# kaiidams/voice100

Hardware: AMD Instinct MI355X
Metric: audio frames/sec (fwd+bwd) asr_en_base, B=32x1024-frame mel (higher is better)
Workload: dtype bf16

## Files before the change

include/voice100_hip.h:

```cpp
#ifndef VOICE100_HIP_H
#define VOICE100_HIP_H

#ifdef __cplusplus
extern "C" {
#endif


int v100_dw_num_groups(int B, int C);
int v100_dwconv(const float* x, const float* x2, const float* w, const float* in_a, const float* in_b,
                const float* in_c, int in_mode, float* y, const float* aux, const float* out_a,
                const float* out_b, int out_mode, float* stats, int G, int B, int C, int Tin, int Tout,
                int K, int stride, int pad, int flip, int upsample, int force_generic, void* stream);

int v100_dwconv_wgrad(const float* g, const float* g2, const float* ga, const float* gb, const float* gc,
                      int g_mode, const float* x, const float* xa, const float* xb, int x_mode,
                      float* partial, float* dw, int G, int B, int C, int Tin, int Tout, int K, int stride,
                      int pad, int force_generic, void* stream);

int v100_dwconv_bwd(const float* g, const float* g2, const float* w, const float* ga, const float* gb,
                    const float* gc, const float* xpre, const float* xa, const float* xb, float* dxin,
                    float* stats, float* wpartial, float* dw, int G, int B, int C, int Tin, int Tout, int K,
                    int stride, int pad, int force_split, void* stream);

int v100_pw_num_parts(int B, int T);
int v100_pw_gemm(const float* A, const void* A_bf16, const float* X, const float* X2, const float* xa,
                 const float* xb, const float* xc, int x_mode, float* Y, const float* bias, const float* ea,
                 const float* eb, const float* R, int epi_mode, float* stats, int B, int M, int K, int T,
                 int use_bf16, void* stream);
int v100_pw_gemm_dropmask_supported(int B, int M, int K, int T, int use_bf16);
int v100_pw_gemm_dropmask(const float* A, const void* A_bf16, const float* X, float* Y, const void* keep, float p, int B, int M, int K,
                          int T, int use_bf16, void* stream);

int v100_pw_wgrad_splits(int B, int M, int K);
int v100_pw_wgrad(const float* G, const float* G2, const float* ga, const float* gb, const float* gc, int g_mode,
                  const float* X, const float* xa, const float* xb, int x_mode, float* partial, float* dW,
                  int S, int B, int M, int K, int T, int use_bf16, void* stream);

int v100_weight_prep(const float* w, int rows, int cols, void* w_bf16, float* wt, void* wt_bf16, void* stream);
int v100_weight_prep_f16(const float* w, int rows, int cols, void* w16, void* stream);

int v100_bn_finalize_train(const float* stats, int parts, long long count, const float* gamma, const float* beta,
                           float* running_mean, float* running_var, long long* num_batches_tracked, float momentum,
                           float eps, float* scale, float* shift, float* save_mean, float* save_rstd, int C, void* stream);
int v100_bn_eval_coeffs(const float* gamma, const float* beta, const float* running_mean, const float* running_var,
                        float eps, float* scale, float* shift, int C, void* stream);
int v100_bn_bwd_finalize(const float* partial, int parts, long long count, const float* gamma, const float* mean,
                         const float* rstd, float* p, float* q, float* r, float* dgamma, float* dbeta, int C, void* stream);
int v100_bn_frozen_coeffs(const float* gamma, const float* beta, const float* running_mean, const float* running_var,
                          float eps, float* scale, float* shift, float* mean, float* rstd, int C, void* stream);
int v100_bn_bwd_finalize_frozen(const float* partial, int parts, long long count, const float* gamma, const float* mean,
                                const float* rstd, float* p, float* q, float* r, float* dgamma, float* dbeta, int C, void* stream);

int v100_chan_reduce2(const float* u, const float* v, float* partial, int G, int B, int C, int T, void* stream);
int v100_slab_sum0(const float* partial, int parts, float* out, int C, void* stream);
int v100_chan_affine2(const float* u, const float* v, const float* A, const float* Bc, const float* Cc, float* out,
                      int B, int C, int T, void* stream);
int v100_mul_scale(const float* u, const float* m, float s, float* out, long long n, void* stream);
int v100_dropout_fwd(const float* x, long long seed, float p, float* y, void* mask, long long n, void* stream);
int v100_dropout_bwd(const float* dy, const void* mask, float p, float* dx, long long n, void* stream);
int v100_transpose_last2(const float* in, float* out, int B, int R, int Cc, void* stream);
int v100_embedding_bct(const long long* idx, const float* table, float* out, int B, int V, int C, int T, void* stream);
int v100_embedding_bwd(const long long* idx, const float* g, float* dtable, int B, int V, int C, int T, void* stream);


int v100_augment_fused(const float* x, const int* len, const float* uniform, float* y, int B, int Tin, int Tout,
                       int F, int stretch_rate, float pitch_rate, float amp, int n_tmask, const int* tm_s,
                       const int* tm_e, const float* tm_a, int fm_on, int fm_s, int fm_e, float fm_a, int noise_on,
                       float noise_low, float noise_high, float noise_std, int mix, float log_offset, void* stream);
int v100_augment_fused_len(const float* x, const int* len_raw, int* len_out, int* half_out, const float* uniform, float* y,
                           int B, int Tin, int Tout, int F, int stretch_rate, float pitch_rate, float amp, int n_tmask,
                           const int* tm_s, const int* tm_e, const float* tm_a, int fm_on, int fm_s, int fm_e, float fm_a,
                           int noise_on, float noise_low, float noise_high, float noise_std, int mix, float log_offset,
                           void* stream);
int v100_augment_fused_len_t(const float* x, const int* len_raw, int* len_out, int* half_out, const float* uniform, float* y,
                             float* yt, int B, int Tin, int Tout, int F, int stretch_rate, float pitch_rate, float amp, int n_tmask,
                             const int* tm_s, const int* tm_e, const float* tm_a, int fm_on, int fm_s, int fm_e, float fm_a,
                             int noise_on, float noise_low, float noise_high, float noise_std, int mix, float log_offset,
                             void* stream);

int v100_shift_copy(const float* in, float* out, const float* bias, int B, int C, int Tin, int Tout, int in_ctot,
                    int in_coff, int out_ctot, int out_coff, int in_mul, int in_add, int out_mul, int out_add, int n,
                    int accumulate, void* stream);
int v100_stft_frames(const float* x, float* frames, int B, int N, int T, int hop, int win, int n_fft, void* stream);
int v100_power_spectrum(const float* spec, float* pw, int B, int F, int T, void* stream);
int v100_log_transpose(const float* in, float* out, int B, int C, int T, float offset, void* stream);
int v100_log_mel_fused(const float* x, float* out, const float* window, const float* tw256, const float* tw512, const int* mel_start,
                       const int* mel_count, const float* mel_w, int B, int N, int T, int hop, int n_fft, int n_mels, float log_offset,
                       void* stream);
int v100_log_mel_fused_len(const float* x, const int* lengths, float* out, int* out_len, const float* window, const float* tw256,
                           const float* tw512, const int* mel_start, const int* mel_count, const float* mel_w, int B, int N, int T,
                           int hop, int n_fft, int n_mels, float log_offset, float fill, void* stream);
int v100_world_unnormalize(const float* x, float* f0, float* logspc, float* codeap, const float* f0_mean, const float* f0_std,
                           const float* ls_mean, const float* ls_std, const float* ca_mean, const float* ca_std,
                           int B, int T, int S, int Cap, void* stream);
int v100_world_loss_parts(int B, int Tp);
int v100_world_loss(const float* pred, const float* f0, const float* hasf0, const float* logspc, const float* codeap,
                    const int* length, const float* f0_mean, const float* f0_std, const float* ls_mean, const float* ls_std,
                    const float* ca_mean, const float* ca_std, const float* w, float* partial, float* loss, float* unit,
                    int B, int Tp, int Tt, int S, int Cap, int l1, void* stream);
int v100_world_loss_bwd(const float* unit, const float* gout, float* dpred, int B, int Tp, int S, int Cap, void* stream);
int v100_exp_clip(const float* x, float* y, float offset, long long n, void* stream);

int v100_bct_to_cm(const float* in, float* out, int B, int C, int T, void* stream);
int v100_cm_to_btc(const float* in, float* out, int B, int C, int T, void* stream);

int v100_world_randn_host(float* host_out, long long n);
int v100_world_decode_aperiodicity(const float* coded, float* ap, long long rows, int nb, int fs, int fft_size, void* stream);
long long v100_world_synth_workspace_bytes(int B, int T, int fs, double frame_period_ms, int fft_size, int max_pulses);
int v100_world_synthesize(const float* f0, const float* sp, const float* ap, const float* coded_ap, int nb, const int* frames, const float* randn_table,
                          long long table_len, const float* tw256, const float* tw512, const float* dc_remover, float* y,
                          int* n_pulses, void* workspace, int B, int T, int fs, double frame_period_ms, int fft_size,
                          int max_pulses, void* stream);

int v100_im2col(const float* x, float* cols, int B, int Cin, int Tin, int Tout, int k, int stride, int pad, void* stream);
int v100_col2im(const float* dcols, float* dx, int B, int Cin, int Tin, int Tout, int k, int stride, int pad, void* stream);
int v100_pad_copy(const float* src, float* dst, int B, int C, int Tsrc, int src_step, int src_off, int n, int Tx, int lpad, void* stream);
int v100_pw_taps_supported(int B, int M, int cx, int ntap, int T, int Tx, int use_bf16);
int v100_pw_gemm_taps(const float* A, const void* A_bf16, const float* Xp, float* Y, const float* bias, const float* R,
                      int B, int M, int cx, int T, int Tx, int ntap, const int* shifts, int use_bf16, void* stream);
int v100_pw_wgrad_taps(const float* G, int Tg, int g_off, const float* Xp, float* partial, float* dW, int S, int B, int M,
                       int cx, int T, int Tx, int ntap, const int* shifts, int use_bf16, void* stream);
int v100_ln_num_parts(int B, int T);
int v100_slab_sum2(const float* partial, int parts, float* out0, float* out1, int C, void* stream);
int v100_ln_gelu_fwd(const float* y, const float* gamma, const float* beta, float eps, float* out, float* mean,
                     float* rstd, int B, int C, int T, void* stream);
int v100_ln_gelu_bwd(const float* dout, const float* y, const float* gamma, const float* beta, const float* mean,
                     const float* rstd, float* dy, float* partial, int B, int C, int T, void* stream);

long long v100_launch_count(void);
int v100_copy_probe(const void* src, void* dst, long long nbytes, void* stream);
int v100_timing_enable(int tag_mask);
int v100_timing_read(int tag, double* ms, long long* count, double* bytes);
int v100_rows_copy_probe(const void* src, void* dst, int B, int C, int row_bytes, void* stream);

int v100_pw_gemm_io(const void* A_bf16, const void* X, const void* X2, const float* xa, const float* xb, const float* xc,
                    int x_mode, void* Y, const float* ea, const float* eb, const void* R, int epi_mode, float* stats,
                    int B, int M, int K, int T, int io16, void* stream);
int v100_pw_wgrad_io(const void* G, const void* G2, const float* ga, const float* gb, const float* gc, int g_mode,
                     const void* X, const float* xa, const float* xb, int x_mode, float* partial, float* dW, int S, int B,
                     int M, int K, int T, int io16, void* stream);
int v100_pw_wgrad_group_supported(int B, int M, int K, int T, int S, int g_mode, int x_mode, int io16);
int v100_pw_wgrad_group_tiles(int M, int K, int x_mode);
int v100_pw_wgrad_group(int n, const void* const* ptrs, const int* dims, void* stream);
int v100_dw_mfma_supported(int K, int stride);
int v100_row_pitch16(int T, int B);
int v100_dwconv_fwd_train_io(const void* a1, const float* w, const float* in_a, const float* in_b, void* a2, float* stats,
                             int G, int B, int C, int T, int K, int io16, void* stream);
int v100_dwconv_bwd_io(const void* g, const void* g2, const float* w, const float* ga, const float* gb, const float* gc,
                       const void* xpre, const float* xa, const float* xb, void* dxin, float* stats, float* wpartial,
                       float* dw, int G, int B, int C, int T, int K, int io16, void* stream);
int v100_dwconv_bwd_da1_io(const void* g, const void* g2, const float* w, const float* ga, const float* gb, const float* gc,
                           const void* xpre, const float* xa, const float* xb, void* da1_out, float* stats, float* dw,
                           const float* bn1_gamma, const float* bn1_mean, const float* bn1_rstd, float* pqr, float* dgamma,
                           float* dbeta, int B, int C, int T, int K, void* stream);
int v100_dwconv_fwd_eval_io(const void* h1, const float* w, const float* out_a, const float* out_b, void* h2, int B, int C, int T,
                            int K, int flags, void* stream);
int v100_chan_reduce2_io(const void* u, const void* v, float* partial, int G, int B, int C, int T, int io16, void* stream);
int v100_chan_affine2_shadow(const void* u, const float* v, const float* A, const float* Cc, float* out, void* shadow,
                             int B, int C, int T, int u_bf16, void* stream);
int v100_chan_affine2_io(const void* u, const void* v, const float* A, const float* Bc, const float* Cc, void* out,
                         int B, int C, int T, int io16, void* stream);
int v100_ir_act16_supported(const int* shape);

int v100_adam_chunk_elems(void);
int v100_adam_step(const void* chunks, int nchunks, const void* params, const void* grads, const void* exp_avg,
                   const void* exp_avg_sq, double lr, double beta1, double beta2, double eps, double weight_decay, int step,
                   void* stream);

int v100_grad_norm_partials(const void* chunks, int nchunks, const void* grads, void* partials, int norm_type, void* stream);
int v100_adam_step_clip(const void* chunks, int nchunks, const void* params, const void* grads, const void* exp_avg,
                        const void* exp_avg_sq, double lr, double beta1, double beta2, double eps, double weight_decay, int step,
                        int clip_mode, double clip, const void* partials, int npartials, int norm_type, void* total_norm, void* stream);
int v100_grad_clip(const void* chunks, int nchunks, const void* grads, int clip_mode, double clip, const void* partials, int npartials,
                   int norm_type, void* total_norm, void* stream);

int v100_ctc_workspace_floats(int B, int T, int Lmax);
int v100_ctc_loss_mean(const float* logits, const long long* targets, const int* in_len, const int* tgt_len, float* workspace,
                       float* nll, float* loss, float* grad, int B, int T, int V, int Lmax, int blank, void* stream);
int v100_ctc_loss(const float* logits, const long long* targets, const int* in_len, const int* tgt_len, float* workspace,
                  float* nll, float* grad, int B, int T, int V, int Lmax, int blank, void* stream);
int v100_ctc_loss_mean_t(const float* logits, const long long* targets, const int* in_len, const int* tgt_len, float* workspace,
                         float* nll, float* loss, float* grad, int grad_bvt, int B, int T, int V, int Lmax, int blank, void* stream);

long long v100_ir_prep_bytes(const int* shape);
long long v100_ir_fwd_workspace_bytes(const int* shape);
long long v100_ir_eval_cache_bytes(const int* shape);
int v100_ir_eval_prep(const int* shape, const void* const* ptrs, void* stream);
int v100_ir_fwd_eval(const int* shape, const void* const* ptrs, void* stream);
int v100_ir_stack_fwd_eval(int n, const int* shapes, const void* const* ptrs, void* stream);
int v100_ir_prep_batched(const int* shapes, const void* const* w1s, const void* const* w3s, void* const* preps, int n, void* stream);
int v100_ir_fwd_train(const int* shape, const void* const* ptrs, void* stream);
long long v100_ir_bwd_workspace_bytes(const int* shape);
int v100_ir_bwd(const int* shape, const void* const* ptrs, void* stream);

long long v100_ir_stack_plan(const int* desc, long long* plan);
int v100_ir_stack_fwd_train(const int* desc, const void* const* params, const void* x, const void* x16, void* blob, void* stream);
int v100_ir_stack_bwd(const int* desc, const void* const* params, const void* x, const void* x16, const void* blob, const void* dy,
                      void* dx, void* grads, void* ws, void* stream);
int v100_ir_stack_wgrad_plan(const int* desc, int have_x16, int min_problem_tiles, int min_flush_tiles, long long* out);
int v100_ir_stack_wgrad_group_thresholds(int min_problem_tiles, int min_flush_tiles);

int v100_ctc_greedy_decode(const float* logits, const int* lens, long long* out, int* out_len, int B, int T, int V, int blank, void* stream);
int v100_ctc_best_path(const float* logp, const long long* labels, const int* in_len, const int* lab_len, void* back_ws, int* path,
                       float* score, int B, int T, int V, int Lmax, int max_move, void* stream);
long long v100_ctc_align_workspace_bytes(int B, int T, int Lmax);
int v100_ctc_align_block(void);
int v100_ctc_align(const float* logp, const long long* labels, const int* in_len, const int* lab_len, void* moves_ws, int* path,
                   long long* best_labels, int* align, float* score, int B, int T, int V, int Lmax, int max_move, void* stream);
long long v100_edit_distance_workspace_bytes(int B, int Th, int Tr);
int v100_edit_distance(const long long* hyp, const int* hyp_len, const long long* ref, const int* ref_len, void* ws, int* dist,
                       int* hyp_n, int* ref_n, long long* totals, int B, int Th, int Tr, int levels, long long sep, void* stream);
long long v100_ctc_beam_workspace_bytes(int B, int T, int V, int W);
int v100_ctc_beam_search(const float* logits, const int* lens, void* ws, long long* ids, int* ids_len, float* scores, int B, int T, int V,
                         int W, int nbest, int blank, void* stream);
int v100_ctc_beam_search_lm(const float* logits, const int* lens, void* ws, long long* ids, int* ids_len, float* scores,
                            const float* lm_logp, const int* lm_next, const float* lm_final, int S, int start_state, float alpha,
                            float beta, int use_eos, float* ctc_scores, float* lm_scores, int B, int T, int V, int W, int nbest,
                            int blank, void* stream);
int v100_align_expand(const long long* text, const double* align, const int* text_len, long long* out, int* out_len, int B, int Lmax,
                      int Tmax, int head, int tail, void* stream);


int v100_world_randn_host_f64(double* host_out, long long n);
long long v100_world_randn_bound(int kind, int T, int fs, int fft_size);
int v100_world_frames(int fs, int length, double frame_period_ms);
int v100_world_dio_bands(int fs, double f0_floor, double f0_ceil, double channels_in_octave, int* half_lengths, int max_bands);
long long v100_world_dio_workspace_bytes(int B, int max_len, int fs, double f0_floor, double f0_ceil, double channels_in_octave,
                                         double frame_period_ms);
int v100_world_dio(const float* x, const int* lengths, int B, int max_len, int pitch, int fs, double f0_floor, double f0_ceil,
                   double channels_in_octave, double frame_period_ms, double allowed_range, const double* lowcut,
                   const double* nuttall, double* f0, void* workspace, void* stream);
int v100_world_cheaptrick(const float* x, const int* lengths, const double* f0, int B, int max_len, int pitch, int fs,
                          double frame_period_ms, double q1, int fft_size, const double* randn_table, long long table_len,
                          const double* twiddle, double* sp, float* logsp, double log_offset, long long* offsets, void* stream);
long long v100_world_d4c_workspace_bytes(int B, int max_len, int fs, double frame_period_ms);
int v100_world_d4c(const float* x, const int* lengths, const double* f0, int B, int max_len, int pitch, int fs, double frame_period_ms,
                   double threshold, int fft_size, const double* randn_table, long long table_len, const double* twiddle,
                   const double* nuttall, int window_length, double* ap, double* coded, float* coded32, void* workspace, void* stream);

long long v100_lstm_weight_bytes(int H, int ndir, int use_bf16, int backward);
int v100_lstm_geometry(int H, int use_bf16, int backward, int* out);
long long v100_lstm_ws_bytes(int B, int H, int ndir, int backward);
int v100_lstm_sync_words(int B, int ndir);
int v100_lstm_persistent_ok(int B, int H, int ndir, int use_bf16, int backward);
int v100_lstm_weight_prep(const float* w_hh0, const float* w_hh1, int H, int ndir, int use_bf16, int backward, void* out,
                          void* stream);
int v100_lstm_fwd(const float* xproj, const void* w_prep, const float* b_hh0, const float* b_hh1, const int* lens, float* y,
                  float* h_n, float* c_n, float* act, float* cs, float* hprev, void* ws, unsigned* sync, int B, int T, int H,
                  int ndir, int use_bf16, int persistent, void* stream);
int v100_lstm_bwd(const float* dy, const float* dh_n, const float* dc_n, const void* w_prep, const int* lens, const float* act,
                  const float* cs, float* dgates, void* ws, unsigned* sync, int B, int T, int H, int ndir, int use_bf16,
                  int persistent, void* stream);

int v100_world_loss_v2(const float* pred, const float* f0, const float* logspc, const float* codeap, const int* length,
                       const float* f0_mean, const float* f0_std, const float* ls_mean, const float* ls_std,
                       const float* ca_mean, const float* ca_std, float* partial, float* loss, float* unit,
                       int B, int Tp, int Tt, int S, int Cap, int l1, void* stream);
int v100_world_loss_v2_bwd(const float* unit, const float* gout, float* dpred, int B, int Tp, int S, int Cap, void* stream);
int v100_align_loss_parts(int B, int L);
int v100_align_loss(const float* pred, const long long* align, const int* text_len, float* partial, float* loss, float* unit,
                    int B, int L, int W, void* stream);
int v100_align_loss_bwd(const float* unit, const float* gout, float* dpred, int B, int L, void* stream);
int v100_align_expand_v2(const long long* text, const double* align, const int* text_len, long long* out, int* out_len, int B,
                         int Lmax, int Tmax, int head, int tail, void* stream);
int v100_world_unnormalize_v2(const float* x, float* f0, float* logspc, float* codeap, const float* f0_mean, const float* f0_std,
                              const float* ls_mean, const float* ls_std, const float* ca_mean, const float* ca_std,
                              int B, int T, int S, int Cap, void* stream);

int v100_masked_ce_parts(int B, int L);
int v100_masked_ce(const float* logits, const long long* target, const int* target_len, float* partial, float* loss, float* unit,
                   int B, int V, int L, void* stream);
int v100_masked_ce_bwd(const float* unit, const float* gout, float* dlogits, int B, int V, int L, void* stream);

long long v100_resample_out_len(long long len, int o, int n);
int v100_resample_tile(void);
int v100_resample_sinc(const float* x, const int* lens, const float* taps, const int* starts, float* y, int* out_lens, int B,
                       int Nmax, int Mmax, int o, int n, int width, int L, void* stream);

int v100_world_stat_parts(int B, int T, int S);
int v100_world_stat_accum(const float* f0, const int* f0_len, const float* logspc, const float* codeap, double* partial,
                          double* moments, int B, int T, int S, int A, void* stream);

#ifdef __cplusplus
}
#endif
#endif
```

voice100_amd/csrc/adam.hip:

```cpp
#include "common.h"
#include <math.h>

struct AdamChunk { int tensor; int count; long long offset; };

__device__ __forceinline__ void adam_update(float& pv, float gv, float& mv, float& vv, float lr_over_bc1, float omb1, float beta2,
                                            float omb2, float eps, float weight_decay, float inv_sqrt_bc2) {
    gv = fmaf(weight_decay, pv, gv);
    mv = fmaf(omb1, gv - mv, mv);
    vv = fmaf(omb2, gv * gv, beta2 * vv);
    pv -= lr_over_bc1 * mv / (sqrtf(vv) * inv_sqrt_bc2 + eps);
}

__global__ __launch_bounds__(256) void adam_step_kernel(const AdamChunk* __restrict__ chunks, float* const* __restrict__ params,
                                                        const float* const* __restrict__ grads, float* const* __restrict__ exp_avg,
                                                        float* const* __restrict__ exp_avg_sq, float lr_over_bc1, float omb1,
                                                        float beta2, float omb2, float eps, float weight_decay, float inv_sqrt_bc2) {
    const AdamChunk ch = chunks[blockIdx.x];
    float* __restrict__ p = params[ch.tensor] + ch.offset;
    const float* __restrict__ g = grads[ch.tensor] + ch.offset;
    float* __restrict__ m = exp_avg[ch.tensor] + ch.offset;
    float* __restrict__ v = exp_avg_sq[ch.tensor] + ch.offset;
    auto upd = [&](float& pv, float gv, float& mv, float& vv) {
        adam_update(pv, gv, mv, vv, lr_over_bc1, omb1, beta2, omb2, eps, weight_decay, inv_sqrt_bc2);
    };
    const bool vec = ((((size_t)p | (size_t)g | (size_t)m | (size_t)v) & 15) == 0);
    if (vec) {
        const int n4 = ch.count >> 2;
        for (int i = threadIdx.x; i < n4; i += 256) {
            f32x4 pv = reinterpret_cast<f32x4*>(p)[i], mv = reinterpret_cast<f32x4*>(m)[i], vv = reinterpret_cast<f32x4*>(v)[i];
            const f32x4 gv = reinterpret_cast<const f32x4*>(g)[i];
#pragma unroll
            for (int e = 0; e < 4; ++e) {
                float a = pv[e], b = mv[e], c = vv[e];
                upd(a, gv[e], b, c);
                pv[e] = a; mv[e] = b; vv[e] = c;
            }
            reinterpret_cast<f32x4*>(p)[i] = pv; reinterpret_cast<f32x4*>(m)[i] = mv; reinterpret_cast<f32x4*>(v)[i] = vv;
        }
        for (int i = (n4 << 2) + threadIdx.x; i < ch.count; i += 256) upd(p[i], g[i], m[i], v[i]);
    } else {
        for (int i = threadIdx.x; i < ch.count; i += 256) upd(p[i], g[i], m[i], v[i]);
    }
}

extern "C" int v100_adam_chunk_elems() { return 16384; }

extern "C" int v100_adam_step(const void* chunks, int nchunks, const void* params, const void* grads, const void* exp_avg,
                              const void* exp_avg_sq, double lr, double beta1, double beta2, double eps, double weight_decay, int step,
                              void* stream) {
    if (!chunks || !params || !grads || !exp_avg || !exp_avg_sq) return V100_ERR_NULL;
    if (nchunks <= 0 || step < 1) return V100_ERR_SHAPE;
    const double bc1 = 1.0 - pow(beta1, (double)step), bc2 = 1.0 - pow(beta2, (double)step);
    V100_GGL(adam_step_kernel, dim3((unsigned)nchunks), dim3(256), 0, (hipStream_t)stream, (const AdamChunk*)chunks,
                       (float* const*)params, (const float* const*)grads, (float* const*)exp_avg, (float* const*)exp_avg_sq,
                       (float)(lr / bc1), (float)(1.0 - beta1), (float)beta2, (float)(1.0 - beta2), (float)eps, (float)weight_decay,
                       (float)(1.0 / sqrt(bc2)));
    return v100_launch_status();
}

#define V100_NORM_L2 2
#define V100_NORM_INF (-1)
#define V100_CLIP_NORM 1
#define V100_CLIP_VALUE 2

__device__ __forceinline__ float nan_maxf(float a, float b) { return (a > b || a != a) ? a : b; }
__device__ __forceinline__ double nan_max(double a, double b) { return (a > b || a != a) ? a : b; }

template <bool MAX>
__device__ __forceinline__ double block_reduce256(double v, double* lds) {
#pragma unroll
    for (int off = 32; off > 0; off >>= 1) {
        const double o = __shfl_xor(v, off, 64);
        v = MAX ? nan_max(v, o) : v + o;
    }
    if ((threadIdx.x & 63) == 0) lds[threadIdx.x >> 6] = v;
    __syncthreads();
    double r = lds[0];
#pragma unroll
    for (int w = 1; w < 4; ++w) r = MAX ? nan_max(r, lds[w]) : r + lds[w];
    return r;
}

__device__ __forceinline__ float clip_coef(const double* __restrict__ partials, int npartials, bool inf, float max_norm,
                                           float* __restrict__ total_out, double* lds) {
    double a = 0.0;
    for (int i = threadIdx.x; i < npartials; i += 256) a = inf ? nan_max(a, partials[i]) : a + partials[i];
    a = inf ? block_reduce256<true>(a, lds) : block_reduce256<false>(a, lds);
    const float total = inf ? (float)a : (float)sqrt(a);
    if (total_out && blockIdx.x == 0 && threadIdx.x == 0) *total_out = total;
    const float coef = (1.0f / (total + 1e-6f)) * max_norm;
    return coef > 1.f ? 1.f : coef;
}

__device__ __forceinline__ float clamp_value(float x, float c) {
    x = x < -c ? -c : x;
    return x > c ? c : x;
}

template <bool INF>
__global__ __launch_bounds__(256) void grad_norm_partials_kernel(const AdamChunk* __restrict__ chunks, const float* const* __restrict__ grads,
                                                                 double* __restrict__ partials) {
    __shared__ double lds[4];
    const AdamChunk ch = chunks[blockIdx.x];
    const float* __restrict__ g = grads[ch.tensor] + ch.offset;
    float acc = 0.f;
    auto add = [&](float x) { acc = INF ? nan_maxf(acc, fabsf(x)) : fmaf(x, x, acc); };
    int i0 = 0;
    if (((size_t)g & 15) == 0) {
        const int n4 = ch.count >> 2;
        for (int i = threadIdx.x; i < n4; i += 256) {
            const f32x4 gv = reinterpret_cast<const f32x4*>(g)[i];
#pragma unroll
            for (int e = 0; e < 4; ++e) add(gv[e]);
        }
        i0 = n4 << 2;
    }
    for (int i = i0 + threadIdx.x; i < ch.count; i += 256) add(g[i]);
    const double r = block_reduce256<INF>((double)acc, lds);
    if (threadIdx.x == 0) partials[blockIdx.x] = r;
}

template <int MODE>
__global__ __launch_bounds__(256) void adam_step_clip_kernel(const AdamChunk* __restrict__ chunks, float* const* __restrict__ params,
                                                             float* const* __restrict__ grads, float* const* __restrict__ exp_avg,
                                                             float* const* __restrict__ exp_avg_sq, float lr_over_bc1, float omb1,
                                                             float beta2, float omb2, float eps, float weight_decay, float inv_sqrt_bc2,
                                                             float clip, const double* __restrict__ partials, int npartials, int inf,
                                                             float* __restrict__ total_out) {
    __shared__ double lds[4];
    const float coef = MODE == V100_CLIP_NORM ? clip_coef(partials, npartials, inf != 0, clip, total_out, lds) : 1.f;
    const bool write_g = MODE == V100_CLIP_VALUE || coef != 1.f;
    const AdamChunk ch = chunks[blockIdx.x];
    float* __restrict__ p = params[ch.tensor] + ch.offset;
    float* __restrict__ g = grads[ch.tensor] + ch.offset;
    float* __restrict__ m = exp_avg[ch.tensor] + ch.offset;
    float* __restrict__ v = exp_avg_sq[ch.tensor] + ch.offset;
    auto cl = [&](float x) { return MODE == V100_CLIP_NORM ? x * coef : clamp_value(x, clip); };
    auto upd = [&](float& pv, float gv, float& mv, float& vv) {
        adam_update(pv, gv, mv, vv, lr_over_bc1, omb1, beta2, omb2, eps, weight_decay, inv_sqrt_bc2);
    };
    int i0 = 0;
    if (((((size_t)p | (size_t)g | (size_t)m | (size_t)v) & 15) == 0)) {
        const int n4 = ch.count >> 2;
        for (int i = threadIdx.x; i < n4; i += 256) {
            f32x4 pv = reinterpret_cast<f32x4*>(p)[i], mv = reinterpret_cast<f32x4*>(m)[i], vv = reinterpret_cast<f32x4*>(v)[i];
            f32x4 gv = reinterpret_cast<const f32x4*>(g)[i];
#pragma unroll
            for (int e = 0; e < 4; ++e) {
                gv[e] = cl(gv[e]);
                float a = pv[e], b = mv[e], c = vv[e];
                upd(a, gv[e], b, c);
                pv[e] = a; mv[e] = b; vv[e] = c;
            }
            if (write_g) reinterpret_cast<f32x4*>(g)[i] = gv;
            reinterpret_cast<f32x4*>(p)[i] = pv; reinterpret_cast<f32x4*>(m)[i] = mv; reinterpret_cast<f32x4*>(v)[i] = vv;
        }
        i0 = n4 << 2;
    }
    for (int i = i0 + threadIdx.x; i < ch.count; i += 256) {
        const float gv = cl(g[i]);
        if (write_g) g[i] = gv;
        upd(p[i], gv, m[i], v[i]);
    }
}

template <int MODE>
__global__ __launch_bounds__(256) void grad_clip_kernel(const AdamChunk* __restrict__ chunks, float* const* __restrict__ grads, float clip,
                                                        const double* __restrict__ partials, int npartials, int inf,
                                                        float* __restrict__ total_out) {
    __shared__ double lds[4];
    const float coef = MODE == V100_CLIP_NORM ? clip_coef(partials, npartials, inf != 0, clip, total_out, lds) : 1.f;
    if (MODE == V100_CLIP_NORM && coef == 1.f) return;
    const AdamChunk ch = chunks[blockIdx.x];
    float* __restrict__ g = grads[ch.tensor] + ch.offset;
    auto cl = [&](float x) { return MODE == V100_CLIP_NORM ? x * coef : clamp_value(x, clip); };
    int i0 = 0;
    if (((size_t)g & 15) == 0) {
        const int n4 = ch.count >> 2;
        for (int i = threadIdx.x; i < n4; i += 256) {
            f32x4 gv = reinterpret_cast<f32x4*>(g)[i];
#pragma unroll
            for (int e = 0; e < 4; ++e) gv[e] = cl(gv[e]);
            reinterpret_cast<f32x4*>(g)[i] = gv;
        }
        i0 = n4 << 2;
    }
    for (int i = i0 + threadIdx.x; i < ch.count; i += 256) g[i] = cl(g[i]);
}

extern "C" int v100_grad_norm_partials(const void* chunks, int nchunks, const void* grads, void* partials, int norm_type, void* stream) {
    if (!chunks || !grads || !partials) return V100_ERR_NULL;
    if (nchunks <= 0 || (norm_type != V100_NORM_L2 && norm_type != V100_NORM_INF)) return V100_ERR_SHAPE;
    if (norm_type == V100_NORM_INF)
        V100_GGL(grad_norm_partials_kernel<true>, dim3((unsigned)nchunks), dim3(256), 0, (hipStream_t)stream, (const AdamChunk*)chunks,
                 (const float* const*)grads, (double*)partials);
    else
        V100_GGL(grad_norm_partials_kernel<false>, dim3((unsigned)nchunks), dim3(256), 0, (hipStream_t)stream, (const AdamChunk*)chunks,
                 (const float* const*)grads, (double*)partials);
    return v100_launch_status();
}

static int check_clip(int clip_mode, double clip, const void* partials, int npartials, int norm_type) {
    if (clip_mode == V100_CLIP_NORM) {
        if (!partials) return V100_ERR_NULL;
        if (npartials <= 0 || (norm_type != V100_NORM_L2 && norm_type != V100_NORM_INF)) return V100_ERR_SHAPE;
        return V100_OK;
    }
    return clip_mode == V100_CLIP_VALUE ? V100_OK : V100_ERR_SHAPE;
}

extern "C" int v100_adam_step_clip(const void* chunks, int nchunks, const void* params, const void* grads, const void* exp_avg,
                                   const void* exp_avg_sq, double lr, double beta1, double beta2, double eps, double weight_decay, int step,
                                   int clip_mode, double clip, const void* partials, int npartials, int norm_type, void* total_norm,
                                   void* stream) {
    if (!chunks || !params || !grads || !exp_avg || !exp_avg_sq) return V100_ERR_NULL;
    if (nchunks <= 0 || step < 1) return V100_ERR_SHAPE;
    if (int rc = check_clip(clip_mode, clip, partials, npartials, norm_type)) return rc;
    const double bc1 = 1.0 - pow(beta1, (double)step), bc2 = 1.0 - pow(beta2, (double)step);
    const int inf = norm_type == V100_NORM_INF;
#define V100_ADAM_CLIP_LAUNCH(MODE)                                                                                                       \
    V100_GGL(adam_step_clip_kernel<MODE>, dim3((unsigned)nchunks), dim3(256), 0, (hipStream_t)stream, (const AdamChunk*)chunks,         \
             (float* const*)params, (float* const*)grads, (float* const*)exp_avg, (float* const*)exp_avg_sq, (float)(lr / bc1),           \
             (float)(1.0 - beta1), (float)beta2, (float)(1.0 - beta2), (float)eps, (float)weight_decay, (float)(1.0 / sqrt(bc2)),         \
             (float)clip, (const double*)partials, npartials, inf, (float*)total_norm)
    if (clip_mode == V100_CLIP_NORM) V100_ADAM_CLIP_LAUNCH(V100_CLIP_NORM);
    else V100_ADAM_CLIP_LAUNCH(V100_CLIP_VALUE);
#undef V100_ADAM_CLIP_LAUNCH
    return v100_launch_status();
}

extern "C" int v100_grad_clip(const void* chunks, int nchunks, const void* grads, int clip_mode, double clip, const void* partials,
                              int npartials, int norm_type, void* total_norm, void* stream) {
    if (!chunks || !grads) return V100_ERR_NULL;
    if (nchunks <= 0) return V100_ERR_SHAPE;
    if (int rc = check_clip(clip_mode, clip, partials, npartials, norm_type)) return rc;
    const int inf = norm_type == V100_NORM_INF;
    if (clip_mode == V100_CLIP_NORM)
        V100_GGL(grad_clip_kernel<V100_CLIP_NORM>, dim3((unsigned)nchunks), dim3(256), 0, (hipStream_t)stream, (const AdamChunk*)chunks,
                 (float* const*)grads, (float)clip, (const double*)partials, npartials, inf, (float*)total_norm);
    else
        V100_GGL(grad_clip_kernel<V100_CLIP_VALUE>, dim3((unsigned)nchunks), dim3(256), 0, (hipStream_t)stream, (const AdamChunk*)chunks,
                 (float* const*)grads, (float)clip, (const double*)partials, npartials, inf, (float*)total_norm);
    return v100_launch_status();
}
```

voice100_amd/csrc/block.hip:

```cpp
#include "common.h"
#include "../../include/voice100_hip.h"
#include "depthwise_common.h"

namespace {
struct Carver {
    char* p; size_t used;
    explicit Carver(void* base) : p((char*)base), used(0) {}
    template <class T> T* take(size_t n) {
        used = (used + 255) & ~size_t(255);
        T* r = p ? (T*)(p + used) : nullptr;
        used += n * sizeof(T);
        return r;
    }
};
inline int conv_out(int t, int k, int s) { return (t + 2 * ((k - 1) / 2) - k) / s + 1; }
const float kMom = 0.1f, kEps = 1e-5f;
}
#define CK(call) do { rc = (call); if (rc) return rc; } while (0)

enum { IR_B, IR_CIN, IR_HID, IR_COUT, IR_T, IR_K, IR_STRIDE, IR_RES, IR_BF16, IR_PREPPED, IR_ACT16, IR_NSHAPE };
static inline int pitch16(int T, int B) { return v100_pitch16(T, B); }
extern "C" int v100_row_pitch16(int T, int B) { return v100_pitch16(T, B); }
enum { PW_IO_X = 1, PW_IO_X2 = 2, PW_IO_Y = 4, PW_IO_R = 8, PW_IO_F16 = 16, WG_IO_G = 1, WG_IO_G2 = 2, WG_IO_X = 4 };

extern "C" int v100_ir_act16_supported(const int* sh) {
    if (!sh || sh[IR_BF16] != 1 || sh[IR_STRIDE] != 1) return 0;
    if (!v100_dw_mfma_supported(sh[IR_K], sh[IR_STRIDE])) return 0;
    const long B = sh[IR_B], hid = sh[IR_HID], cin = sh[IR_CIN], cout = sh[IR_COUT], P = pitch16(sh[IR_T], sh[IR_B]);
    if (hid % 2 || cin % 2 || cout % 2) return 0;
    if (B * hid * P * 4 >= 0x7fffff00L || (hid + 128) * P * 4 >= 0x7fffff00L || (hid + 128) * (cin > cout ? cin : cout) * 2 >= 0x7fffff00L) return 0;
    return 1;
}

struct IrPrep { void *w1bf, *w1tbf, *w3bf, *w3tbf; float *w1t, *w3t; };
static size_t ir_prep_carve(const int* sh, void* base, IrPrep& w) {
    const int cin = sh[IR_CIN], hid = sh[IR_HID], cout = sh[IR_COUT];
    Carver c(base);
    if (sh[IR_BF16]) {
        w.w1bf = c.take<u16>((size_t)hid * cin); w.w1tbf = c.take<u16>((size_t)hid * cin);
        w.w3bf = c.take<u16>((size_t)cout * hid); w.w3tbf = c.take<u16>((size_t)cout * hid);
        w.w1t = nullptr; w.w3t = nullptr;
    } else {
        w.w1bf = w.w1tbf = w.w3bf = w.w3tbf = nullptr;
        w.w1t = c.take<float>((size_t)hid * cin); w.w3t = c.take<float>((size_t)cout * hid);
    }
    return c.used + 256;
}
extern "C" long long v100_ir_prep_bytes(const int* shape) {
    IrPrep w;
    return (long long)ir_prep_carve(shape, nullptr, w);
}

static size_t ir_fwd_carve(const int* sh, void* base, float** stats) {
    const int B = sh[IR_B], hid = sh[IR_HID], cout = sh[IR_COUT], T = sh[IR_T];
    const int T2 = conv_out(T, sh[IR_K], sh[IR_STRIDE]);
    Carver c(base);
    size_t n = (size_t)v100_pw_num_parts(B, T) * hid * 2;
    const size_t n2 = (size_t)v100_dw_num_groups(B, hid) * hid * 2;
    const size_t n3 = (size_t)v100_pw_num_parts(B, T2) * cout * 2;
    if (n2 > n) n = n2;
    if (n3 > n) n = n3;
    *stats = c.take<float>(n);
    return c.used + 256;
}

extern "C" long long v100_ir_fwd_workspace_bytes(const int* shape) {
    float* s;
    return (long long)ir_fwd_carve(shape, nullptr, &s);
}

extern "C" int v100_ir_fwd_train(const int* sh, const void* const* P, void* stream) {
    if (!sh || !P) return V100_ERR_NULL;
    const int B = sh[IR_B], cin = sh[IR_CIN], hid = sh[IR_HID], cout = sh[IR_COUT], T = sh[IR_T], K = sh[IR_K], S = sh[IR_STRIDE];
    const int res = sh[IR_RES], bf = sh[IR_BF16];
    if (bf != 0 && bf != 1) return V100_ERR_SHAPE;
    const int pad = (K - 1) / 2, T2 = conv_out(T, K, S);
    const float* x = (const float*)P[0];
    const float* w1 = (const float*)P[1]; const float* wd = (const float*)P[7]; const float* w3 = (const float*)P[13];
    float* a1 = (float*)P[19]; float* a2 = (float*)P[20]; float* a3 = (float*)P[21]; float* y = (float*)P[22];
    float* coef = (float*)P[23];
    const int mc = hid > cout ? hid : cout;
    float *s1 = coef, *t1 = coef + mc, *m1 = coef + 2 * mc, *r1 = coef + 3 * mc, *s2 = coef + 4 * mc, *t2 = coef + 5 * mc,
          *m2 = coef + 6 * mc, *r2 = coef + 7 * mc, *s3 = coef + 8 * mc, *t3 = coef + 9 * mc, *m3 = coef + 10 * mc, *r3 = coef + 11 * mc;
    float* st;
    ir_fwd_carve(sh, const_cast<void*>(P[24]), &st);
    IrPrep pw;
    ir_prep_carve(sh, const_cast<void*>(P[25]), pw);
    void *w1bf = pw.w1bf, *w3bf = pw.w3bf;
    int rc;
    if (!(sh[IR_PREPPED] & 1)) {
        CK(v100_weight_prep(w1, hid, cin, pw.w1bf, pw.w1t, pw.w1tbf, stream));
        CK(v100_weight_prep(w3, cout, hid, pw.w3bf, pw.w3t, pw.w3tbf, stream));
    }
    const int parts1 = v100_pw_num_parts(B, T), parts3 = v100_pw_num_parts(B, T2), G = v100_dw_num_groups(B, hid);
    const bool frozen = (sh[IR_PREPPED] & 8) != 0;
    if (frozen && sh[IR_ACT16]) return V100_ERR_SHAPE;
    auto finalize = [&](const float* stats, int parts, long long count, int j, float* s_, float* t_, float* m_, float* r_, int C) -> int {
        if (frozen)
            return v100_bn_frozen_coeffs((const float*)P[j], (const float*)P[j + 1], (const float*)P[j + 2], (const float*)P[j + 3], kEps, s_, t_, m_, r_, C, stream);
        return v100_bn_finalize_train(stats, parts, count, (const float*)P[j], (const float*)P[j + 1], (float*)P[j + 2], (float*)P[j + 3],
                                      (long long*)P[j + 4], kMom, kEps, s_, t_, m_, r_, C, stream);
    };
    if (sh[IR_ACT16]) {
        if (!v100_ir_act16_supported(sh)) return V100_ERR_SHAPE;
        const void* x16 = (sh[IR_ACT16] >= 4 && (sh[IR_PREPPED] & 2)) ? P[26] : nullptr;
        void* y16 = (sh[IR_ACT16] >= 4 && (sh[IR_PREPPED] & 2)) ? const_cast<void*>(P[27]) : nullptr;
        if (x16) CK(v100_pw_gemm_io(w1bf, x16, nullptr, nullptr, nullptr, nullptr, 0, a1, nullptr, nullptr, nullptr, 1, st, B, hid, cin, T, PW_IO_X | PW_IO_Y, stream));
        else CK(v100_pw_gemm_io(w1bf, x, nullptr, nullptr, nullptr, nullptr, 0, a1, nullptr, nullptr, nullptr, 1, st, B, hid, cin, T, PW_IO_Y, stream));
        if (G == 1) {
            const DwFin fin{1, (double)B * T2, (const float*)P[8], (const float*)P[9], nullptr, s2, t2, nullptr, m2, r2,
                            (float*)P[10], (float*)P[11], (long long*)P[12], kMom, kEps};
            const DwPre pre{{1, (double)B * T, (const float*)P[2], (const float*)P[3], nullptr, s1, t1, nullptr, m1, r1,
                             (float*)P[4], (float*)P[5], (long long*)P[6], kMom, kEps}, st, parts1};
            CK(dw_fwd_train_io_fin(a1, wd, s1, t1, a2, st, G, B, hid, T, K, DW_IO_X | DW_IO_Y, fin, pre, stream));
        } else {
            CK(v100_bn_finalize_train(st, parts1, (long long)B * T, (const float*)P[2], (const float*)P[3], (float*)P[4], (float*)P[5], (long long*)P[6],
                                      kMom, kEps, s1, t1, m1, r1, hid, stream));
            CK(v100_dwconv_fwd_train_io(a1, wd, s1, t1, a2, st, G, B, hid, T, K, DW_IO_X | DW_IO_Y, stream));
            CK(v100_bn_finalize_train(st, G, (long long)B * T2, (const float*)P[8], (const float*)P[9], (float*)P[10], (float*)P[11], (long long*)P[12],
                                      kMom, kEps, s2, t2, m2, r2, hid, stream));
        }
        const bool a316 = sh[IR_ACT16] >= 3;
        CK(v100_pw_gemm_io(w3bf, a2, nullptr, s2, t2, nullptr, 1, a3, nullptr, nullptr, nullptr, 1, st, B, cout, hid, T2, PW_IO_X | (a316 ? PW_IO_Y : 0), stream));
        const DwPre pre{{1, (double)B * T2, (const float*)P[14], (const float*)P[15], nullptr, s3, t3, nullptr, m3, r3,
                         (float*)P[16], (float*)P[17], (long long*)P[18], kMom, kEps}, st, parts3};
        const bool r16 = sh[IR_ACT16] >= 5 && x16 && a316;
        const bool noy = sh[IR_ACT16] >= 5 && y16 && a316 && (sh[IR_PREPPED] & 4);
        CK(chan_affine2_fin(a3, res ? (r16 ? x16 : (const void*)x) : nullptr, noy ? nullptr : y, y16, B, cout, T2, a316 ? 1 : 0, pre, stream, r16 ? 1 : 0));
        return V100_OK;
    }
    CK(v100_pw_gemm(w1, w1bf, x, nullptr, nullptr, nullptr, nullptr, 0, a1, nullptr, nullptr, nullptr, nullptr, 1, st, B, hid, cin, T, bf, stream));
    CK(finalize(st, parts1, (long long)B * T, 2, s1, t1, m1, r1, hid));
    CK(v100_dwconv(a1, nullptr, wd, s1, t1, nullptr, 1, a2, nullptr, nullptr, nullptr, 0, st, G, B, hid, T, T2, K, S, pad, 0, 1, 0, stream));
    CK(finalize(st, G, (long long)B * T2, 8, s2, t2, m2, r2, hid));
    CK(v100_pw_gemm(w3, w3bf, a2, nullptr, s2, t2, nullptr, 1, a3, nullptr, nullptr, nullptr, nullptr, 1, st, B, cout, hid, T2, bf, stream));
    if (!frozen && bf == 1 && (sh[IR_PREPPED] & 2) && P[27]) {
        const DwPre pre{{1, (double)B * T2, (const float*)P[14], (const float*)P[15], nullptr, s3, t3, nullptr, m3, r3,
                         (float*)P[16], (float*)P[17], (long long*)P[18], kMom, kEps}, st, parts3};
        CK(chan_affine2_fin(a3, res ? x : nullptr, y, const_cast<void*>(P[27]), B, cout, T2, 0, pre, stream, 0));
        return V100_OK;
    }
    CK(finalize(st, parts3, (long long)B * T2, 14, s3, t3, m3, r3, cout));
    if (bf == 1 && (sh[IR_PREPPED] & 2) && P[27]) CK(v100_chan_affine2_shadow(a3, res ? x : nullptr, s3, t3, y, const_cast<void*>(P[27]), B, cout, T2, 0, stream));
    else CK(v100_chan_affine2(a3, res ? x : nullptr, s3, nullptr, t3, y, B, cout, T2, stream));
    return V100_OK;
}

struct IrBwdWs {
    float *part, *da3, *dz2, *dz1, *slab, *pqr;
};
static size_t ir_bwd_carve(const int* sh, void* base, IrBwdWs& w) {
    const int B = sh[IR_B], cin = sh[IR_CIN], hid = sh[IR_HID], cout = sh[IR_COUT], T = sh[IR_T], K = sh[IR_K];
    const int T2 = conv_out(T, K, sh[IR_STRIDE]);
    Carver c(base);
    size_t n = (size_t)v100_dw_num_groups(B, cout) * cout * 2;
    size_t m = (size_t)v100_pw_num_parts(B, T2) * hid * 2; if (m > n) n = m;
    m = (size_t)v100_dw_num_groups(B, hid) * hid * 2; if (m > n) n = m;
    w.part = c.take<float>(n);
    w.da3 = sh[IR_ACT16] >= 3 ? (float*)c.take<u16>((size_t)B * cout * pitch16(T2, B)) : c.take<float>((size_t)B * cout * T2);
    if (sh[IR_ACT16] >= 2) {
        w.dz2 = (float*)c.take<u16>((size_t)B * hid * pitch16(T2, B));
        w.dz1 = (float*)c.take<u16>((size_t)B * hid * pitch16(T, B));
    } else {
        w.dz2 = c.take<float>((size_t)B * hid * T2);
        w.dz1 = c.take<float>((size_t)B * hid * T);
    }
    n = (size_t)v100_pw_wgrad_splits(B, cout, hid) * cout * hid;
    m = (size_t)v100_pw_wgrad_splits(B, hid, cin) * hid * cin; if (m > n) n = m;
    m = (size_t)v100_dw_num_groups(B, hid) * hid * K; if (m > n) n = m;
    w.slab = c.take<float>(n);
    w.pqr = c.take<float>((size_t)6 * (hid > cout ? hid : cout));
    return c.used + 256;
}

static size_t ir_defer_da3_bytes(const int* sh) {
    const size_t n = (size_t)sh[IR_B] * sh[IR_COUT] * pitch16(conv_out(sh[IR_T], sh[IR_K], sh[IR_STRIDE]), sh[IR_B]) * 2;
    return (n + 255) & ~size_t(255);
}
static size_t ir_defer_bytes(const int* sh) {
    const size_t n = (size_t)sh[IR_B] * sh[IR_HID] * pitch16(sh[IR_T], sh[IR_B]) * 2;
    return ir_defer_da3_bytes(sh) + ((n + 255) & ~size_t(255));
}
static int ir_wgrad_defer_tiles(const int* sh) {
    return v100_pw_wgrad_group_tiles(sh[IR_COUT], sh[IR_HID], 1) + v100_pw_wgrad_group_tiles(sh[IR_HID], sh[IR_CIN], 0);
}
static bool ir_wgrad_defer_ok(const int* sh, bool have_x16, int min_tiles) {
    const int B = sh[IR_B], cin = sh[IR_CIN], hid = sh[IR_HID], cout = sh[IR_COUT], T = sh[IR_T], K = sh[IR_K];
    if (sh[IR_ACT16] < 4 || !(sh[IR_PREPPED] & 2) || (sh[IR_PREPPED] & 8) || !have_x16 || sh[IR_STRIDE] != 1) return false;
    if (!v100_ir_act16_supported(sh) || v100_dw_num_groups(B, hid) != 1 || !dw_bwd_da1_supported(B, hid, T, K, 1)) return false;
    const int io = WG_IO_G | WG_IO_X;
    return v100_pw_wgrad_group_supported(B, cout, hid, T, v100_pw_wgrad_splits(B, cout, hid), 0, 1, io) &&
           v100_pw_wgrad_group_supported(B, hid, cin, T, v100_pw_wgrad_splits(B, hid, cin), 0, 0, io) &&
           v100_pw_wgrad_group_tiles(cout, hid, 1) >= min_tiles && v100_pw_wgrad_group_tiles(hid, cin, 0) >= min_tiles;
}

extern "C" long long v100_ir_bwd_workspace_bytes(const int* shape) {
    IrBwdWs w;
    return (long long)ir_bwd_carve(shape, nullptr, w);
}

extern "C" int v100_ir_bwd(const int* sh, const void* const* P, void* stream) {
    if (!sh || !P) return V100_ERR_NULL;
    const int B = sh[IR_B], cin = sh[IR_CIN], hid = sh[IR_HID], cout = sh[IR_COUT], T = sh[IR_T], K = sh[IR_K], S = sh[IR_STRIDE];
    const int res = sh[IR_RES], bf = sh[IR_BF16];
    const int pad = (K - 1) / 2, T2 = conv_out(T, K, S);
    const float *x = (const float*)P[0], *a1 = (const float*)P[1], *a2 = (const float*)P[2], *a3 = (const float*)P[3];
    const float *w1 = (const float*)P[4], *wd = (const float*)P[5], *w3 = (const float*)P[6];
    const float *g1 = (const float*)P[7], *g2 = (const float*)P[8], *g3 = (const float*)P[9];
    const float* coef = (const float*)P[10];
    const int mc = hid > cout ? hid : cout;
    const float *s1 = coef, *t1 = coef + mc, *m1 = coef + 2 * mc, *r1 = coef + 3 * mc, *s2 = coef + 4 * mc, *t2 = coef + 5 * mc,
                *m2 = coef + 6 * mc, *r2 = coef + 7 * mc, *m3 = coef + 10 * mc, *r3 = coef + 11 * mc;
    const float* dy = (const float*)P[11];
    float* dx = (float*)P[12];
    const int dy16 = (sh[IR_PREPPED] & 16) ? 1 : 0, dx16 = (sh[IR_PREPPED] & 32) ? 1 : 0;
    IrBwdWs w;
    ir_bwd_carve(sh, const_cast<void*>(P[22]), w);
    const bool defer = (sh[IR_PREPPED] & 64) != 0;
    if (defer) {
        if (!P[25]) return V100_ERR_NULL;
        if (sh[IR_ACT16] < 4) return V100_ERR_SHAPE;
        w.da3 = (float*)P[25];
        w.dz1 = (float*)((char*)const_cast<void*>(P[25]) + ir_defer_da3_bytes(sh));
    }
    float *pp = w.pqr, *qq = w.pqr + mc, *rr = w.pqr + 2 * mc;
    int rc;
    IrPrep pw;
    ir_prep_carve(sh, const_cast<void*>(P[23]), pw);
    (void)w1; (void)w3;
    const bool frozen = (sh[IR_PREPPED] & 8) != 0;
    if (frozen && sh[IR_ACT16]) return V100_ERR_SHAPE;
    auto bwd_finalize = frozen ? v100_bn_bwd_finalize_frozen : v100_bn_bwd_finalize;
    const int Gr = v100_dw_num_groups(B, cout);
    const bool a316 = sh[IR_ACT16] >= 3;
    bool da3_done = false;
    if (a316) {
        const DwFin fin{2, (double)B * T2, g3, m3, r3, pp, qq, rr, (float*)P[20], (float*)P[21], nullptr, nullptr, nullptr, 0.f, 0.f};
        if (chan_bn3_bwd(dy, a3, w.part, w.da3, B, cout, T2, fin, stream, dy16)) {
            if ((rc = v100_launch_status()) != V100_OK) return rc;
            da3_done = true;
        } else if (dy16) return V100_ERR_SHAPE;
        else CK(chan_reduce2_io_fin(dy, a3, w.part, B, cout, T2, fin, stream));
    } else {
        if (dy16) return V100_ERR_SHAPE;
        CK(v100_chan_reduce2(dy, a3, w.part, Gr, B, cout, T2, stream));
        CK(bwd_finalize(w.part, Gr, (long long)B * T2, g3, m3, r3, pp, qq, rr, (float*)P[20], (float*)P[21], cout, stream));
    }
    if (da3_done) {}
    else if (a316) CK(v100_chan_affine2_io(dy, a3, pp, qq, rr, w.da3, B, cout, T2, 6, stream));
    else CK(v100_chan_affine2(dy, a3, pp, qq, rr, w.da3, B, cout, T2, stream));
    if (sh[IR_ACT16]) {
        if (!v100_ir_act16_supported(sh)) return V100_ERR_SHAPE;
        const bool g16 = sh[IR_ACT16] >= 2;
        if (!defer)
            CK(v100_pw_wgrad_io(w.da3, nullptr, nullptr, nullptr, nullptr, 0, a2, s2, t2, 1, w.slab, (float*)P[19], v100_pw_wgrad_splits(B, cout, hid),
                                B, cout, hid, T2, WG_IO_X | (a316 ? WG_IO_G : 0), stream));
        const int parts16 = v100_pw_num_parts(B, T2);
        CK(v100_pw_gemm_io(pw.w3tbf, w.da3, nullptr, nullptr, nullptr, nullptr, 0, w.dz2, s2, t2, a2, 4, w.part, B, hid, cout, T2,
                           PW_IO_R | (g16 ? PW_IO_Y : 0) | (a316 ? PW_IO_X : 0), stream));
        const int G16 = v100_dw_num_groups(B, hid);
        bool da1 = false;
        if (G16 == 1) {
            float *pp2 = w.pqr + 3 * mc, *qq2 = w.pqr + 4 * mc, *rr2 = w.pqr + 5 * mc;
            const DwFin fin{2, (double)B * T, g1, m1, r1, pp2, qq2, rr2, (float*)P[14], (float*)P[15], nullptr, nullptr, nullptr, 0.f, 0.f};
            const DwPre pre{{2, (double)B * T2, g2, m2, r2, pp, qq, rr, (float*)P[17], (float*)P[18], nullptr, nullptr, nullptr, 0.f, 0.f},
                            w.part, parts16};
            da1 = g16 && !frozen && dw_bwd_da1_supported(B, hid, T, K, G16);
            CK(dw_bwd_io_fin(w.dz2, a2, wd, pp, qq, rr, a1, s1, t1, w.dz1, w.part, w.slab, (float*)P[16], G16, B, hid, T, K,
                             g16 ? (DW_IO_X | DW_IO_X2 | DW_IO_AUX | DW_IO_Y) : (DW_IO_X2 | DW_IO_AUX), fin, pre, stream, da1 ? 1 : 0));
            pp = pp2; qq = qq2; rr = rr2;
        } else {
            CK(v100_bn_bwd_finalize(w.part, parts16, (long long)B * T2, g2, m2, r2, pp, qq, rr, (float*)P[17], (float*)P[18], hid, stream));
            CK(v100_dwconv_bwd_io(w.dz2, a2, wd, pp, qq, rr, a1, s1, t1, w.dz1, w.part, w.slab, (float*)P[16], G16, B, hid, T, K,
                                  g16 ? (DW_IO_X | DW_IO_X2 | DW_IO_AUX | DW_IO_Y) : (DW_IO_X2 | DW_IO_AUX), stream));
            CK(v100_bn_bwd_finalize(w.part, G16, (long long)B * T, g1, m1, r1, pp, qq, rr, (float*)P[14], (float*)P[15], hid, stream));
        }
        const void* x16 = (sh[IR_ACT16] >= 4 && (sh[IR_PREPPED] & 2)) ? P[24] : nullptr;
        if (defer && !(da1 && x16)) return V100_ERR_SHAPE;
        if (da1) {
            if (!defer)
                CK(v100_pw_wgrad_io(w.dz1, nullptr, nullptr, nullptr, nullptr, 0, x16 ? x16 : (const void*)x, nullptr, nullptr, 0, w.slab, (float*)P[13],
                                    v100_pw_wgrad_splits(B, hid, cin), B, hid, cin, T, WG_IO_G | (x16 ? WG_IO_X : 0), stream));
            if (dx)
                CK(v100_pw_gemm_io(pw.w1tbf, w.dz1, nullptr, nullptr, nullptr, nullptr, 0, dx, nullptr, nullptr, res ? dy : nullptr, res ? 5 : 0, nullptr,
                                   B, cin, hid, T, PW_IO_X | ((dy16 && res) ? PW_IO_R : 0) | (dx16 ? PW_IO_Y : 0), stream));
            return V100_OK;
        }
        if (dy16 || dx16) return V100_ERR_SHAPE;
        CK(v100_pw_wgrad_io(w.dz1, a1, pp, qq, rr, 2, x16 ? x16 : (const void*)x, nullptr, nullptr, 0, w.slab, (float*)P[13], v100_pw_wgrad_splits(B, hid, cin),
                            B, hid, cin, T, WG_IO_G2 | (g16 ? WG_IO_G : 0) | (x16 ? WG_IO_X : 0), stream));
        if (dx)
            CK(v100_pw_gemm_io(pw.w1tbf, w.dz1, a1, pp, qq, rr, 2, dx, nullptr, nullptr, res ? dy : nullptr, res ? 5 : 0, nullptr,
                               B, cin, hid, T, PW_IO_X2 | (g16 ? PW_IO_X : 0), stream));
        return V100_OK;
    }
    if (dy16 || dx16) return V100_ERR_SHAPE;
    CK(v100_pw_wgrad(w.da3, nullptr, nullptr, nullptr, nullptr, 0, a2, s2, t2, 1, w.slab, (float*)P[19], v100_pw_wgrad_splits(B, cout, hid),
                     B, cout, hid, T2, bf, stream));
    const int parts = v100_pw_num_parts(B, T2);
    CK(v100_pw_gemm(pw.w3t, pw.w3tbf, w.da3, nullptr, nullptr, nullptr, nullptr, 0, w.dz2, nullptr, s2, t2, a2, 4, w.part, B, hid, cout, T2, bf, stream));
    CK(bwd_finalize(w.part, parts, (long long)B * T2, g2, m2, r2, pp, qq, rr, (float*)P[17], (float*)P[18], hid, stream));
    const int G = v100_dw_num_groups(B, hid);
    CK(v100_dwconv_bwd(w.dz2, a2, wd, pp, qq, rr, a1, s1, t1, w.dz1, w.part, w.slab, (float*)P[16], G, B, hid, T, T2, K, S, pad, 0, stream));
    CK(bwd_finalize(w.part, G, (long long)B * T, g1, m1, r1, pp, qq, rr, (float*)P[14], (float*)P[15], hid, stream));
    CK(v100_pw_wgrad(w.dz1, a1, pp, qq, rr, 2, x, nullptr, nullptr, 0, w.slab, (float*)P[13], v100_pw_wgrad_splits(B, hid, cin),
                     B, hid, cin, T, bf, stream));
    if (dx)
        CK(v100_pw_gemm(pw.w1t, pw.w1tbf, w.dz1, a1, pp, qq, rr, 2, dx, nullptr, nullptr, nullptr, res ? dy : nullptr, res ? 5 : 0, nullptr,
                        B, cin, hid, T, bf, stream));
    return V100_OK;
}

struct IrEvalCache { void *w1bf, *w3bf; float *s1, *t1, *s2, *t2, *s3, *t3; };
static size_t ir_eval_carve(const int* sh, void* base, IrEvalCache& w) {
    const int cin = sh[IR_CIN], hid = sh[IR_HID], cout = sh[IR_COUT];
    Carver c(base);
    w.w1bf = w.w3bf = nullptr;
    if (sh[IR_BF16]) { w.w1bf = c.take<u16>((size_t)hid * cin); w.w3bf = c.take<u16>((size_t)cout * hid); }
    w.s1 = c.take<float>(hid); w.t1 = c.take<float>(hid); w.s2 = c.take<float>(hid); w.t2 = c.take<float>(hid);
    w.s3 = c.take<float>(cout); w.t3 = c.take<float>(cout);
    return c.used + 256;
}
extern "C" long long v100_ir_eval_cache_bytes(const int* shape) {
    IrEvalCache w;
    return (long long)ir_eval_carve(shape, nullptr, w);
}
extern "C" int v100_ir_eval_prep(const int* sh, const void* const* P, void* stream) {
    if (!sh || !P) return V100_ERR_NULL;
    const int cin = sh[IR_CIN], hid = sh[IR_HID], cout = sh[IR_COUT];
    IrEvalCache c;
    ir_eval_carve(sh, const_cast<void*>(P[14]), c);
    int rc;
    if (sh[IR_BF16] == 2) {
        CK(v100_weight_prep_f16((const float*)P[0], hid, cin, c.w1bf, stream));
        CK(v100_weight_prep_f16((const float*)P[9], cout, hid, c.w3bf, stream));
    } else if (sh[IR_BF16]) {
        CK(v100_weight_prep((const float*)P[0], hid, cin, c.w1bf, nullptr, nullptr, stream));
        CK(v100_weight_prep((const float*)P[9], cout, hid, c.w3bf, nullptr, nullptr, stream));
    }
    CK(v100_bn_eval_coeffs((const float*)P[1], (const float*)P[2], (const float*)P[3], (const float*)P[4], kEps, c.s1, c.t1, hid, stream));
    CK(v100_bn_eval_coeffs((const float*)P[5], (const float*)P[6], (const float*)P[7], (const float*)P[8], kEps, c.s2, c.t2, hid, stream));
    CK(v100_bn_eval_coeffs((const float*)P[10], (const float*)P[11], (const float*)P[12], (const float*)P[13], kEps, c.s3, c.t3, cout, stream));
    return V100_OK;
}
extern "C" int v100_ir_fwd_eval(const int* sh, const void* const* P, void* stream) {
    if (!sh || !P) return V100_ERR_NULL;
    const int B = sh[IR_B], cin = sh[IR_CIN], hid = sh[IR_HID], cout = sh[IR_COUT], T = sh[IR_T], K = sh[IR_K], S = sh[IR_STRIDE];
    const int res = sh[IR_RES], bf = sh[IR_BF16];
    const int pad = (K - 1) / 2, T2 = conv_out(T, K, S);
    const float* x = (const float*)P[0];
    IrEvalCache c;
    ir_eval_carve(sh, const_cast<void*>(P[4]), c);
    float *h1 = (float*)P[5], *h2 = (float*)P[6], *y = (float*)P[7];
    int rc;
    if (sh[IR_ACT16] == 2) {
        int shb[IR_NSHAPE];
        for (int i = 0; i < IR_NSHAPE; ++i) shb[i] = sh[i];
        shb[IR_BF16] = 1;
        if ((bf != 1 && bf != 2) || S != 1 || T > 768 || !v100_ir_act16_supported(shb)) return V100_ERR_SHAPE;
        const long long N = (long long)B * pitch16(T, B);
        if (N > 0x7fffff00LL) return V100_ERR_SHAPE;
        const int f16 = bf == 2 ? PW_IO_F16 : 0;
        CK(v100_pw_gemm_io(c.w1bf, x, nullptr, nullptr, nullptr, nullptr, 0, h1, c.s1, c.t1, nullptr, 2, nullptr, 1, hid, cin, (int)N, PW_IO_Y | f16, stream));
        CK(dw_fwd_eval_io(h1, (const float*)P[2], c.s2, c.t2, h2, B, hid, T, K, stream, 1, bf == 2));
        CK(v100_pw_gemm_io(c.w3bf, h2, nullptr, nullptr, nullptr, nullptr, 0, y, c.s3, c.t3, res ? x : nullptr, 3, nullptr, 1, cout, hid, (int)N, PW_IO_X | f16, stream));
        return V100_OK;
    }
    if (sh[IR_ACT16]) {
        if (bf != 1 || !v100_ir_act16_supported(sh)) return V100_ERR_SHAPE;
        CK(v100_pw_gemm_io(c.w1bf, x, nullptr, nullptr, nullptr, nullptr, 0, h1, c.s1, c.t1, nullptr, 2, nullptr, B, hid, cin, T, PW_IO_Y, stream));
        CK(dw_fwd_eval_io(h1, (const float*)P[2], c.s2, c.t2, h2, B, hid, T, K, stream));
        CK(v100_pw_gemm_io(c.w3bf, h2, nullptr, nullptr, nullptr, nullptr, 0, y, c.s3, c.t3, res ? x : nullptr, 3, nullptr, B, cout, hid, T2, PW_IO_X, stream));
        return V100_OK;
    }
    CK(v100_pw_gemm((const float*)P[1], c.w1bf, x, nullptr, nullptr, nullptr, nullptr, 0, h1, nullptr, c.s1, c.t1, nullptr, 2, nullptr, B, hid, cin, T, bf, stream));
    CK(v100_dwconv(h1, nullptr, (const float*)P[2], nullptr, nullptr, nullptr, 0, h2, nullptr, c.s2, c.t2, 1, nullptr, v100_dw_num_groups(B, hid),
                   B, hid, T, T2, K, S, pad, 0, 1, 0, stream));
    CK(v100_pw_gemm((const float*)P[3], c.w3bf, h2, nullptr, nullptr, nullptr, nullptr, 0, y, nullptr, c.s3, c.t3, res ? x : nullptr, 3, nullptr, B, cout, hid, T2, bf, stream));
    return V100_OK;
}

extern "C" int v100_ir_stack_fwd_eval(int n, const int* shapes, const void* const* ptrs, void* stream) {
    if (!shapes || !ptrs) return V100_ERR_NULL;
    if (n < 0) return V100_ERR_SHAPE;
    for (int i = 0; i < n; ++i) {
        const int rc = v100_ir_fwd_eval(shapes + (size_t)i * IR_NSHAPE, ptrs + (size_t)i * 8, stream);
        if (rc != V100_OK) return rc;
    }
    return V100_OK;
}

struct PrepBatch {
    enum { MAXN = 32 };
    const float* w[2 * MAXN]; u16* wbf[2 * MAXN]; float* wt[2 * MAXN]; u16* wtbf[2 * MAXN];
    int rows[2 * MAXN], cols[2 * MAXN];
};
__global__ __launch_bounds__(256) void weight_prep_batched_kernel(PrepBatch t) {
    __shared__ float tile[64][65];
    const int e = blockIdx.y;
    const float* __restrict__ w = t.w[e];
    const int rows = t.rows[e], cols = t.cols[e];
    const int tr = (rows + 63) >> 6, tc = (cols + 63) >> 6;
    const int tx = threadIdx.x & 63, ty = threadIdx.x >> 6;
    const bool fast = !(rows & 63) && !(cols & 63) && t.wt[e] == nullptr && t.wbf[e] != nullptr && t.wtbf[e] != nullptr;
    for (int tl = blockIdx.x; fast && tl < tr * tc; tl += gridDim.x) {
        const int r0 = (tl / tc) << 6, c0 = (tl % tc) << 6;
        __syncthreads();
#pragma unroll
        for (int q = 0; q < 4; ++q) {
            const int id = threadIdx.x + 256 * q;
            const int i = id >> 4, c4 = (id & 15) << 2;
            const f32x4 v = *reinterpret_cast<const f32x4*>(w + (size_t)(r0 + i) * cols + c0 + c4);
            uint2 o; o.x = pack_bf16(v[0], v[1]); o.y = pack_bf16(v[2], v[3]);
            *reinterpret_cast<uint2*>(t.wbf[e] + (size_t)(r0 + i) * cols + c0 + c4) = o;
            tile[i][c4] = v[0]; tile[i][c4 + 1] = v[1]; tile[i][c4 + 2] = v[2]; tile[i][c4 + 3] = v[3];
        }
        __syncthreads();
#pragma unroll
        for (int q = 0; q < 4; ++q) {
            const int id = threadIdx.x + 256 * q;
            const int c = id >> 4, r4 = (id & 15) << 2;
            uint2 o; o.x = pack_bf16(tile[r4][c], tile[r4 + 1][c]); o.y = pack_bf16(tile[r4 + 2][c], tile[r4 + 3][c]);
            *reinterpret_cast<uint2*>(t.wtbf[e] + (size_t)(c0 + c) * rows + r0 + r4) = o;
        }
    }
    for (int tl = blockIdx.x; !fast && tl < tr * tc; tl += gridDim.x) {
        const int r0 = (tl / tc) << 6, c0 = (tl % tc) << 6;
        __syncthreads();
#pragma unroll 4
        for (int i = ty; i < 64; i += 4) {
            const int r = r0 + i, c = c0 + tx;
            float v = 0.f;
            if (r < rows && c < cols) {
                v = w[(size_t)r * cols + c];
                if (t.wbf[e]) t.wbf[e][(size_t)r * cols + c] = f2bf(v);
            }
            tile[i][tx] = v;
        }
        __syncthreads();
#pragma unroll 4
        for (int i = ty; i < 64; i += 4) {
            const int c = c0 + i, r = r0 + tx;
            if (c < cols && r < rows) {
                const float v = tile[tx][i];
                if (t.wt[e]) t.wt[e][(size_t)c * rows + r] = v;
                if (t.wtbf[e]) t.wtbf[e][(size_t)c * rows + r] = f2bf(v);
            }
        }
    }
}
extern "C" int v100_ir_prep_batched(const int* shapes, const void* const* w1s, const void* const* w3s, void* const* preps, int n,
                                    void* stream) {
    if (!shapes || !w1s || !w3s || !preps) return V100_ERR_NULL;
    if (n <= 0 || n > PrepBatch::MAXN) return V100_ERR_SHAPE;
    PrepBatch t;
    long maxn = 0;
    for (int i = 0; i < n; ++i) {
        const int* sh = shapes + (size_t)i * IR_NSHAPE;
        if (!w1s[i] || !w3s[i] || !preps[i]) return V100_ERR_NULL;
        IrPrep pw;
        ir_prep_carve(sh, preps[i], pw);
        t.w[2 * i] = (const float*)w1s[i]; t.rows[2 * i] = sh[IR_HID]; t.cols[2 * i] = sh[IR_CIN];
        t.wbf[2 * i] = (u16*)pw.w1bf; t.wt[2 * i] = pw.w1t; t.wtbf[2 * i] = (u16*)pw.w1tbf;
        t.w[2 * i + 1] = (const float*)w3s[i]; t.rows[2 * i + 1] = sh[IR_COUT]; t.cols[2 * i + 1] = sh[IR_HID];
        t.wbf[2 * i + 1] = (u16*)pw.w3bf; t.wt[2 * i + 1] = pw.w3t; t.wtbf[2 * i + 1] = (u16*)pw.w3tbf;
        const long a = (long)sh[IR_HID] * sh[IR_CIN], b = (long)sh[IR_COUT] * sh[IR_HID];
        if (a > maxn) maxn = a;
        if (b > maxn) maxn = b;
        if (a <= 0 || b <= 0) return V100_ERR_SHAPE;
    }
    long gx = (maxn + 4095) / 4096;
    if (gx > 256) gx = 256;
    if (gx < 1) gx = 1;
    V100_GGL(weight_prep_batched_kernel, dim3((unsigned)gx, 2 * n), dim3(256), 0, (hipStream_t)stream, t);
    return v100_launch_status();
}

enum { ST_N, ST_B, ST_T, ST_BF16, ST_LEVEL, ST_SHADOW, ST_HDR };
namespace {
struct StackBlock { int sh[IR_NSHAPE]; long long a1, a2, a3, y, y16, coef, prep; int Tout; size_t grad_floats; long long defer_off; };
inline size_t al256(size_t v) { return (v + 255) & ~size_t(255); }
int wg_min_problem_tiles = 32, wg_min_flush_tiles = 192;
int stack_layout(const int* desc, StackBlock* blk, size_t& blob_bytes, size_t& bwd_ws, size_t& grad_floats, size_t& fwd_ws_off,
                 int min_tiles = wg_min_problem_tiles) {
    const int n = desc[ST_N], B = desc[ST_B], bf = desc[ST_BF16], level = desc[ST_LEVEL];
    if (n <= 0 || n > 32 || B <= 0 || desc[ST_T] <= 0 || (bf != 0 && bf != 1)) return 0;
    int T = desc[ST_T];
    size_t off = 0, fwd_ws = 0, bws = 0, dxmax = 0;
    grad_floats = 0;
    const bool shadows = bf == 1 && level >= 4;
    for (int i = 0; i < n; ++i) {
        const int* d = desc + ST_HDR + 6 * i;
        StackBlock& b = blk[i];
        const int cin = d[0], hid = d[1], cout = d[2], k = d[3], s = d[4], res = d[5];
        if (cin <= 0 || hid <= 0 || cout <= 0 || k <= 0 || s <= 0) return 0;
        int* sh = b.sh;
        sh[IR_B] = B; sh[IR_CIN] = cin; sh[IR_HID] = hid; sh[IR_COUT] = cout; sh[IR_T] = T; sh[IR_K] = k; sh[IR_STRIDE] = s;
        sh[IR_RES] = res; sh[IR_BF16] = bf; sh[IR_PREPPED] = 1 | (shadows ? 2 : 0); sh[IR_ACT16] = 0;
        if (bf == 1 && level && v100_ir_act16_supported(sh)) sh[IR_ACT16] = level;
        const int T2 = conv_out(T, k, s);
        if (T2 <= 0) return 0;
        b.Tout = T2;
        const int lv = sh[IR_ACT16];
        const size_t P = pitch16(T, B), P2 = pitch16(T2, B);
        b.a1 = (long long)off; off = al256(off + (lv ? (size_t)B * hid * P * 2 : (size_t)B * hid * T * 4));
        b.a2 = (long long)off; off = al256(off + (lv ? (size_t)B * hid * P * 2 : (size_t)B * hid * T2 * 4));
        b.a3 = (long long)off; off = al256(off + (lv >= 3 ? (size_t)B * cout * P * 2 : (size_t)B * cout * T2 * 4));
        b.y = (long long)off; off = al256(off + (size_t)B * cout * T2 * 4);
        b.y16 = -1;
        if (shadows && (i + 1 < n || desc[ST_SHADOW])) { b.y16 = (long long)off; off = al256(off + (size_t)B * cout * P2 * 2); }
        if (i > 0 && lv >= 5 && shadows && blk[i - 1].y16 >= 0 && blk[i - 1].sh[IR_ACT16] >= 5) blk[i - 1].sh[IR_PREPPED] |= 4;
        b.coef = (long long)off; off = al256(off + (size_t)12 * (hid > cout ? hid : cout) * 4);
        b.prep = (long long)off; off = al256(off + (size_t)v100_ir_prep_bytes(sh));
        const size_t fw = (size_t)v100_ir_fwd_workspace_bytes(sh), bw = (size_t)v100_ir_bwd_workspace_bytes(sh);
        if (fw > fwd_ws) fwd_ws = fw;
        if (bw > bws) bws = bw;
        const size_t dxb = (size_t)B * cin * T * 4;
        if (dxb > dxmax) dxmax = dxb;
        b.grad_floats = (size_t)hid * cin + 2 * (size_t)hid + (size_t)hid * k + 2 * (size_t)hid + (size_t)cout * hid + 2 * (size_t)cout;
        grad_floats += b.grad_floats;
        T = T2;
    }
    fwd_ws_off = off;
    blob_bytes = al256(off + fwd_ws) + 256;
    bwd_ws = al256(bws) + 2 * al256(dxmax) + 256;
    for (int i = 0; i < n; ++i) {
        blk[i].defer_off = -1;
        if (ir_wgrad_defer_ok(blk[i].sh, i == 0 || blk[i - 1].y16 >= 0, min_tiles)) {
            blk[i].defer_off = (long long)bwd_ws;
            bwd_ws += ir_defer_bytes(blk[i].sh);
        }
    }
    return 1;
}

void stack_flush_plan(const StackBlock* blk, int n, bool have_x16, int min_flush, bool* defer, int* flush) {
    int tiles = 0, count = 0;
    for (int i = n - 1; i >= 0; --i) {
        defer[i] = blk[i].defer_off >= 0 && (i > 0 || have_x16);
        flush[i] = 0;
        if (defer[i]) { tiles += ir_wgrad_defer_tiles(blk[i].sh); count += 2; }
        if (!count) continue;
        const bool next = i > 0 && blk[i - 1].defer_off >= 0 && (i > 1 || have_x16);
        const bool fits = next && count + 2 <= 16 && tiles + ir_wgrad_defer_tiles(blk[i - 1].sh) <= 256;
        if (i == 0 || count + 2 > 16 || (tiles >= min_flush && !fits)) {
            flush[i] = tiles >= min_flush ? tiles : -tiles;
            tiles = count = 0;
        }
    }
}
}

extern "C" int v100_ir_stack_wgrad_group_thresholds(int min_problem_tiles, int min_flush_tiles) {
    if (min_problem_tiles < 1 || min_flush_tiles < 1) return V100_ERR_SHAPE;
    wg_min_problem_tiles = min_problem_tiles;
    wg_min_flush_tiles = min_flush_tiles;
    return V100_OK;
}

extern "C" int v100_ir_stack_wgrad_plan(const int* desc, int have_x16, int min_problem_tiles, int min_flush_tiles, long long* out) {
    if (!desc || !out) return V100_ERR_NULL;
    if (min_problem_tiles < 1 || min_flush_tiles < 1) return V100_ERR_SHAPE;
    StackBlock blk[32];
    size_t blob, bws, gf, fwo;
    if (!stack_layout(desc, blk, blob, bws, gf, fwo, min_problem_tiles)) return V100_ERR_SHAPE;
    const int n = desc[ST_N];
    bool defer[32]; int flush[32];
    stack_flush_plan(blk, n, have_x16 != 0, min_flush_tiles, defer, flush);
    size_t shared = bws;
    for (int i = 0; i < n; ++i) {
        out[3 * i] = defer[i]; out[3 * i + 1] = blk[i].defer_off; out[3 * i + 2] = flush[i];
        if (blk[i].defer_off >= 0 && (size_t)blk[i].defer_off < shared) shared = (size_t)blk[i].defer_off;
    }
    out[3 * n] = (long long)bws; out[3 * n + 1] = (long long)shared;
    return V100_OK;
}

extern "C" long long v100_ir_stack_plan(const int* desc, long long* plan) {
    if (!desc || !plan) return -1;
    StackBlock blk[32];
    size_t blob, bws, gf, fwo;
    if (!stack_layout(desc, blk, blob, bws, gf, fwo)) return -1;
    const int n = desc[ST_N];
    for (int i = 0; i < n; ++i) {
        long long* o = plan + 8 * i;
        o[0] = blk[i].a1; o[1] = blk[i].a2; o[2] = blk[i].a3; o[3] = blk[i].y; o[4] = blk[i].y16; o[5] = blk[i].coef; o[6] = blk[i].prep;
        o[7] = blk[i].Tout;
    }
    long long* t = plan + 8 * n;
    t[0] = (long long)blob; t[1] = (long long)bws; t[2] = (long long)gf; t[3] = (long long)fwo; t[4] = 0; t[5] = 0;
    return (long long)blob;
}

extern "C" int v100_ir_stack_fwd_train(const int* desc, const void* const* params, const void* x, const void* x16, void* blob,
                                       void* stream) {
    if (!desc || !params || !x || !blob) return V100_ERR_NULL;
    StackBlock blk[32];
    size_t blob_bytes, bws, gf, fwo;
    if (!stack_layout(desc, blk, blob_bytes, bws, gf, fwo)) return V100_ERR_SHAPE;
    const int n = desc[ST_N];
    char* base = (char*)blob;
    int rc;
    {
        int shapes[32 * IR_NSHAPE];
        const void* w1s[32]; const void* w3s[32]; void* preps[32];
        for (int i = 0; i < n; ++i) {
            for (int j = 0; j < IR_NSHAPE; ++j) shapes[i * IR_NSHAPE + j] = blk[i].sh[j];
            w1s[i] = params[18 * i + 0]; w3s[i] = params[18 * i + 12]; preps[i] = base + blk[i].prep;
        }
        CK(v100_ir_prep_batched(shapes, w1s, w3s, preps, n, stream));
    }
    const void* xin = x;
    const void* xin16 = x16;
    for (int i = 0; i < n; ++i) {
        const StackBlock& b = blk[i];
        const void* P[28];
        P[0] = xin;
        for (int j = 0; j < 18; ++j) P[1 + j] = params[18 * i + j];
        P[19] = base + b.a1; P[20] = base + b.a2; P[21] = base + b.a3; P[22] = base + b.y; P[23] = base + b.coef;
        P[24] = base + fwo; P[25] = base + b.prep;
        P[26] = xin16; P[27] = b.y16 >= 0 ? base + b.y16 : nullptr;
        CK(v100_ir_fwd_train(b.sh, P, stream));
        xin = base + b.y;
        xin16 = b.y16 >= 0 ? base + b.y16 : nullptr;
    }
    return V100_OK;
}

extern "C" int v100_ir_stack_bwd(const int* desc, const void* const* params, const void* x, const void* x16, const void* blob,
                                 const void* dy, void* dx, void* grads, void* ws, void* stream) {
    if (!desc || !params || !x || !blob || !dy || !grads || !ws) return V100_ERR_NULL;
    StackBlock blk[32];
    size_t blob_bytes, bws, gf, fwo;
    if (!stack_layout(desc, blk, blob_bytes, bws, gf, fwo)) return V100_ERR_SHAPE;
    const int n = desc[ST_N];
    const char* base = (const char*)blob;
    size_t wsmax = 0, dxmax = 0;
    for (int i = 0; i < n; ++i) {
        const size_t bw = (size_t)v100_ir_bwd_workspace_bytes(blk[i].sh);
        if (bw > wsmax) wsmax = bw;
        const size_t dxb = (size_t)blk[i].sh[IR_B] * blk[i].sh[IR_CIN] * blk[i].sh[IR_T] * 4;
        if (dxb > dxmax) dxmax = dxb;
    }
    char* w0 = (char*)ws;
    char* pp[2] = {w0 + al256(wsmax), w0 + al256(wsmax) + al256(dxmax)};
    size_t goff = gf;
    const void* dyi = dy;
    int rc;
    static const bool grad16_on = [] { const char* e = getenv("V100_IR_GRAD16"); return !(e && e[0] == '0'); }();
    auto grad16_ok = [&](int i) {
        const int* sh = blk[i].sh;
        return grad16_on && desc[ST_LEVEL] >= 5 && sh[IR_ACT16] >= 3 && sh[IR_STRIDE] == 1 && sh[IR_T] >= 8 &&
               chan_bn3_bwd_fits(sh[IR_B], sh[IR_T]) && v100_ir_act16_supported(sh) &&
               dw_bwd_da1_supported(sh[IR_B], sh[IR_HID], sh[IR_T], sh[IR_K], v100_dw_num_groups(sh[IR_B], sh[IR_HID])) && sh[IR_ACT16] >= 2;
    };
    bool defer[32]; int flush[32];
    stack_flush_plan(blk, n, x16 != nullptr, wg_min_flush_tiles, defer, flush);
    const void* gp[5 * 16]; int gd[8 * 16]; int gblk[16]; int ng = 0;
    auto flush_pending = [&](bool grouped) -> int {
        int rc = V100_OK;
        if (grouped) rc = v100_pw_wgrad_group(ng, gp, gd, stream);
        else
            for (int j = 0; j < ng && rc == V100_OK; ++j) {
                IrBwdWs w;
                ir_bwd_carve(blk[gblk[j]].sh, w0, w);
                const int* d = gd + 8 * j;
                rc = v100_pw_wgrad_io(gp[5 * j], nullptr, nullptr, nullptr, nullptr, d[5], gp[5 * j + 1], (const float*)gp[5 * j + 2],
                                      (const float*)gp[5 * j + 3], d[6], w.slab, (float*)const_cast<void*>(gp[5 * j + 4]), d[4], d[0], d[1], d[2], d[3],
                                      d[7], stream);
            }
        ng = 0;
        return rc;
    };
    bool dy_is16 = false;
    for (int i = n - 1; i >= 0; --i) {
        StackBlock b = blk[i];
        if (defer[i]) b.sh[IR_PREPPED] |= 64;
        const bool dx_is16 = i > 0 && grad16_ok(i) && grad16_ok(i - 1);
        if (dy_is16 && !grad16_ok(i)) return V100_ERR_SHAPE;
        b.sh[IR_PREPPED] |= (dy_is16 ? 16 : 0) | (dx_is16 ? 32 : 0);
        goff -= b.grad_floats;
        float* g = (float*)grads + goff;
        const int cin = b.sh[IR_CIN], hid = b.sh[IR_HID], cout = b.sh[IR_COUT], k = b.sh[IR_K];
        void* dxi = i > 0 ? (void*)pp[i & 1] : dx;
        const void* P[26];
        P[25] = defer[i] ? w0 + b.defer_off : nullptr;
        P[0] = i > 0 ? (const void*)(base + blk[i - 1].y) : x;
        P[1] = base + b.a1; P[2] = base + b.a2; P[3] = base + b.a3;
        P[4] = params[18 * i + 0]; P[5] = params[18 * i + 6]; P[6] = params[18 * i + 12];
        P[7] = params[18 * i + 1]; P[8] = params[18 * i + 7]; P[9] = params[18 * i + 13];
        P[10] = base + b.coef; P[11] = dyi; P[12] = dxi;
        float* q = g;
        P[13] = q; q += (size_t)hid * cin; P[14] = q; q += hid; P[15] = q; q += hid;
        P[16] = q; q += (size_t)hid * k; P[17] = q; q += hid; P[18] = q; q += hid;
        P[19] = q; q += (size_t)cout * hid; P[20] = q; q += cout; P[21] = q;
        P[22] = w0; P[23] = base + b.prep;
        P[24] = i > 0 ? (blk[i - 1].y16 >= 0 ? (const void*)(base + blk[i - 1].y16) : nullptr) : x16;
        CK(v100_ir_bwd(b.sh, P, stream));
        if (defer[i]) {
            const int B = b.sh[IR_B], T = b.sh[IR_T], mc = hid > cout ? hid : cout;
            const float* coef = (const float*)(base + b.coef);
            const char* own = w0 + b.defer_off;
            const void* pr[2][5] = {{own, P[2], coef + 4 * mc, coef + 5 * mc, P[19]}, {own + ir_defer_da3_bytes(b.sh), P[24], nullptr, nullptr, P[13]}};
            const int dm[2][8] = {{B, cout, hid, T, v100_pw_wgrad_splits(B, cout, hid), 0, 1, WG_IO_G | WG_IO_X},
                                  {B, hid, cin, T, v100_pw_wgrad_splits(B, hid, cin), 0, 0, WG_IO_G | WG_IO_X}};
            for (int j = 0; j < 2; ++j, ++ng) {
                for (int e = 0; e < 5; ++e) gp[5 * ng + e] = pr[j][e];
                for (int e = 0; e < 8; ++e) gd[8 * ng + e] = dm[j][e];
                gblk[ng] = i;
            }
        }
        if (flush[i]) CK(flush_pending(flush[i] > 0));
        dyi = dxi;
        dy_is16 = dx_is16;
    }
    return V100_OK;
}
```

voice100_amd/functional.py:

```python
import ctypes
import functools
import weakref
import os
from typing import Optional

import torch

from . import _native as N


@functools.lru_cache(maxsize=None)
def pitch16(T: int, B: int) -> int:
    return int(N.helper("v100_row_pitch16", int(T), int(B)))

CHECK_IDS = os.environ.get("VOICE100_CHECK_IDS", "0") not in ("", "0")


def _check_ids(idx: torch.Tensor, n: int, what: str) -> None:
    if CHECK_IDS and idx.numel():
        lo, hi = int(idx.min()), int(idx.max())
        if lo < 0 or hi >= n:
            raise IndexError(f"{what}: index out of range [0, {n}) (min {lo}, max {hi})")

BN_EPS = 1e-5
BN_MOMENTUM = 0.1

_PRECISION = "fp32"
_ACT16 = int(os.environ.get("VOICE100_ACT16", "5"))


def set_activation_storage(level: int) -> None:
    global _ACT16
    if level not in (0, 1, 2, 3, 4, 5):
        raise ValueError("activation storage level must be 0 ... 5")
    _ACT16 = level


def get_activation_storage() -> int:
    return _ACT16


def set_matmul_precision(p: str) -> None:
    global _PRECISION
    if p not in ("fp32", "bf16", "fp16"):
        raise ValueError("precision must be 'fp32', 'bf16' or 'fp16'")
    _PRECISION = p


def _fmt(precision: Optional[str]) -> int:
    precision = precision or _PRECISION
    try:
        return {"fp32": 0, "bf16": 1, "fp16": 2}[precision]
    except KeyError:
        raise ValueError(f"unknown precision {precision!r}") from None


def _no_fp16_training(fmt: int, what: str):
    if fmt == 2:
        raise RuntimeError(f"{what}: 'fp16' is an inference precision (no gradient kernels); train with 'bf16' or 'fp32'")


def get_matmul_precision() -> str:
    return _PRECISION


def _f32(*shape, like):
    return torch.empty(shape, dtype=torch.float32, device=like.device)


def _check(x: torch.Tensor, name: str):
    if not x.is_cuda:
        raise RuntimeError(f"{name}: voice100_amd runs on the GPU only (got a {x.device} tensor); "
                           "there is no CPU fallback -- see oracle/ for the CPU checker")
    if x.dtype != torch.float32:
        raise RuntimeError(f"{name}: expected float32, got {x.dtype}")


def conv_out_len(t: int, k: int, stride: int) -> int:
    pad = (k - 1) // 2
    return (t + 2 * pad - k) // stride + 1


class _Weights:

    def __init__(self, w2d: torch.Tensor, fmt, transposed: bool):
        fmt = int(fmt)
        self.w = w2d
        m, k = w2d.shape
        self.w_bf = self.wt = self.wt_bf = None
        if fmt == 2:
            _no_fp16_training(2 if transposed else 0, "backward GEMM")
            self.w_bf = torch.empty((m, k), dtype=torch.float16, device=w2d.device)
            N.call("v100_weight_prep_f16", w2d, m, k, self.w_bf)
            return
        if fmt:
            self.w_bf = torch.empty((m, k), dtype=torch.bfloat16, device=w2d.device)
        if transposed:
            if fmt:
                self.wt_bf = torch.empty((k, m), dtype=torch.bfloat16, device=w2d.device)
            else:
                self.wt = _f32(k, m, like=w2d)
        if self.w_bf is not None or self.wt is not None or self.wt_bf is not None:
            N.call("v100_weight_prep", w2d, m, k, self.w_bf, self.wt, self.wt_bf)


_DERIVED = {}


def _derived(w: torch.Tensor, tag, build):
    key = (id(w), tag)
    ent = _DERIVED.get(key)
    if ent is not None and ent[0]() is w and ent[1] == w._version and ent[2] == w.data_ptr():
        return ent[3]
    val = build()
    try:
        ref = weakref.ref(w, lambda _r, k=key: _DERIVED.pop(k, None))
    except TypeError:
        return val
    _DERIVED[key] = (ref, w._version, w.data_ptr(), val)
    return val


def clear_derived_cache() -> None:
    _DERIVED.clear()


def _weights_of(w: torch.Tensor, rows: int, cols: int, fmt, transposed: bool) -> "_Weights":
    return _derived(w, ("w", rows, cols, int(fmt), bool(transposed)), lambda: _Weights(w.detach().reshape(rows, cols), fmt, transposed))


def _touched(tensors) -> None:
    torch.autograd.graph.increment_version(tensors)


def _pw_gemm(a_f32, a_bf, x, y, m, k, t, b, bf16, x2=None, xa=None, xb=None, xc=None, x_mode=0, bias=None,
             ea=None, eb=None, r=None, epi=0, stats=None):
    N.call("v100_pw_gemm", a_f32, a_bf, x, x2, xa, xb, xc, x_mode, y, bias, ea, eb, r, epi, stats, b, m, k, t, int(bf16))


def _bn_train(stats, parts, count, bn_w, bn_b, rm, rv, nbt, c, like):
    scale, shift, mean, rstd = (_f32(c, like=like) for _ in range(4))
    N.call("v100_bn_finalize_train", stats, parts, count, bn_w, bn_b, rm, rv, nbt, BN_MOMENTUM, BN_EPS, scale, shift, mean, rstd, c)
    _touched((rm, rv, nbt))
    return scale, shift, mean, rstd


def _bn_eval(bn_w, bn_b, rm, rv, c, like):
    scale, shift = _f32(c, like=like), _f32(c, like=like)
    N.call("v100_bn_eval_coeffs", bn_w, bn_b, rm, rv, BN_EPS, scale, shift, c)
    return scale, shift


def _bn_bwd(partial, parts, count, gamma, mean, rstd, c, like):
    p, q, r, dg, db = (_f32(c, like=like) for _ in range(5))
    N.call("v100_bn_bwd_finalize", partial, parts, count, gamma, mean, rstd, p, q, r, dg, db, c)
    return p, q, r, dg, db


def _ptr_table(items):
    arr = (ctypes.c_void_p * len(items))()
    for i, t in enumerate(items):
        arr[i] = None if t is None else t.data_ptr()
    return arr


class InvertedResidualTrainFn(torch.autograd.Function):

    @staticmethod
    def forward(ctx, x, w1, g1, b1, wd, g2, b2, w3, g3, b3, rm1, rv1, nbt1, rm2, rv2, nbt2, rm3, rv3, nbt3,
                kernel_size, stride, use_residual, precision, prep=None, x16=None, want_shadow=False, frozen=False):
        _check(x, "InvertedResidual")
        x = x.contiguous()
        B, cin, T = x.shape
        hid, cout = w1.shape[0], w3.shape[0]
        k = int(kernel_size)
        T2 = conv_out_len(T, k, stride)
        bf16 = _fmt(precision)
        _no_fp16_training(bf16, "InvertedResidual (training mode)")
        shadows = bf16 == 1 and _ACT16 >= 4 and not frozen
        shape = (ctypes.c_int * 11)(B, cin, hid, cout, T, k, int(stride), int(bool(use_residual)), int(bf16),
                                    int(prep is not None) | (2 if shadows else 0) | (8 if frozen else 0), 0)
        if bf16 == 1 and _ACT16 and not frozen and N.helper("v100_ir_act16_supported", shape):
            shape[10] = _ACT16
            pitch = pitch16(T, B)
            a1 = torch.empty((B, hid, pitch), dtype=torch.bfloat16, device=x.device)
            a2 = torch.empty((B, hid, pitch), dtype=torch.bfloat16, device=x.device)
            a3 = torch.empty((B, cout, pitch), dtype=torch.bfloat16, device=x.device) if _ACT16 >= 3 else _f32(B, cout, T2, like=x)
        else:
            a1 = _f32(B, hid, T, like=x)
            a2 = _f32(B, hid, T2, like=x)
            a3 = _f32(B, cout, T2, like=x)
        y = _f32(B, cout, T2, like=x)
        y16 = torch.empty((B, cout, pitch16(T2, B)), dtype=torch.bfloat16, device=x.device) if (shadows and want_shadow) else None
        if not (shadows and shape[10] >= 4):
            x16 = None
        coef = _f32(12, max(hid, cout), like=x)
        ws = torch.empty(N.helper("v100_ir_fwd_workspace_bytes", shape), dtype=torch.uint8, device=x.device)
        if prep is None:
            prep = torch.empty(N.helper("v100_ir_prep_bytes", shape), dtype=torch.uint8, device=x.device)
        tensors = (x, w1, g1, b1, rm1, rv1, nbt1, wd, g2, b2, rm2, rv2, nbt2, w3, g3, b3, rm3, rv3, nbt3, a1, a2, a3, y, coef, ws, prep)
        if shadows:
            tensors = tensors + (x16, y16)
        for t in tensors[:19]:
            if not t.is_contiguous() or not t.is_cuda:
                raise RuntimeError("InvertedResidual: parameters and buffers must be contiguous CUDA tensors")
        N.call("v100_ir_fwd_train", shape, _ptr_table(tensors))
        if not frozen:
            _touched((rm1, rv1, nbt1, rm2, rv2, nbt2, rm3, rv3, nbt3))
        ctx.save_for_backward(x, a1, a2, a3, w1, wd, w3, g1, g2, g3, coef, prep, x16 if x16 is not None else coef)
        ctx.has_x16 = x16 is not None
        ctx.shape = shape
        if y16 is not None:
            ctx.mark_non_differentiable(y16)
        ctx.set_materialize_grads(False)
        ctx.y_shape = y.shape
        return y, y16

    @staticmethod
    def backward(ctx, dy, _dy16=None):
        x, a1, a2, a3, w1, wd, w3, g1, g2, g3, coef, prep, x16 = ctx.saved_tensors
        if not ctx.has_x16:
            x16 = None
        shape = ctx.shape
        if dy is None:
            dy = torch.zeros(ctx.y_shape, dtype=torch.float32, device=x.device)
        dy = dy.contiguous()
        hid, cin = w1.shape[0], w1.shape[1]
        cout, k = w3.shape[0], wd.shape[2]
        sizes = (hid * cin, hid, hid, hid * k, hid, hid, cout * hid, cout, cout)
        flat = _f32(sum(sizes), like=x)
        parts, off = [], 0
        for n in sizes:
            parts.append(flat[off:off + n])
            off += n
        dx = torch.empty_like(x) if ctx.needs_input_grad[0] else None
        ws = torch.empty(N.helper("v100_ir_bwd_workspace_bytes", shape), dtype=torch.uint8, device=x.device)
        extra = (x16,) if (shape[9] & 2) else ()
        N.call("v100_ir_bwd", shape, _ptr_table((x, a1, a2, a3, w1, wd, w3, g1, g2, g3, coef, dy, dx) + tuple(parts) + (ws, prep) + extra))
        dW1, dg1, db1, dWd, dg2, db2, dW3, dg3, db3 = parts
        return (dx, dW1.view_as(w1), dg1, db1, dWd.view_as(wd), dg2, db2, dW3.view_as(w3), dg3, db3) + (None,) * 17


def _block_tensors(blk):
    mods = blk.__dict__["_modules"]["conv"].__dict__["_modules"]
    pw, dw, pl, bn3 = mods["0"].__dict__["_modules"], mods["1"].__dict__["_modules"], mods["2"], mods["3"]
    c1, bn1, cd, bn2 = pw["0"], pw["1"], dw["0"], dw["1"]
    p1, b1, p2, b2, p3, b3 = bn1._parameters, bn1._buffers, bn2._parameters, bn2._buffers, bn3._parameters, bn3._buffers
    return (c1._parameters["weight"], p1["weight"], p1["bias"], b1["running_mean"], b1["running_var"], b1["num_batches_tracked"],
            cd._parameters["weight"], p2["weight"], p2["bias"], b2["running_mean"], b2["running_var"], b2["num_batches_tracked"],
            pl._parameters["weight"], p3["weight"], p3["bias"], b3["running_mean"], b3["running_var"], b3["num_batches_tracked"])


_STACK_PLANS = {}
_GRAD_ARENAS = []


def register_grad_arena(a) -> None:
    import weakref
    unregister_grad_arena(a)
    _GRAD_ARENAS.insert(0, weakref.ref(a))


def unregister_grad_arena(a) -> None:
    _GRAD_ARENAS[:] = [r for r in _GRAD_ARENAS if r() is not None and r() is not a]


def _grad_arena_for(weights, numel):
    if any(w.grad is not None for w in weights):
        return None
    for r in _GRAD_ARENAS:
        a = r()
        if a is None or not a._hooks:
            continue
        if weights[0] not in a._view:
            continue
        buf = a.grad_arena(weights)
        if buf is not None and buf.numel() != numel:
            a._claimed.discard(a._view[weights[0]][0])
            buf = None
        return buf
    return None
_STACK_SEGMENT = None


def set_stack_segment(n: Optional[int]) -> None:
    global _STACK_SEGMENT
    if n is not None and n < 1:
        raise ValueError("segment must be >= 1 or None")
    _STACK_SEGMENT = n


def set_wgrad_group_thresholds(min_problem_tiles: int = 32, min_flush_tiles: int = 192) -> None:
    N.call("v100_ir_stack_wgrad_group_thresholds", int(min_problem_tiles), int(min_flush_tiles))
    _STACK_PLANS.clear()


def _stack_plan(cfgs, B, T, bf16, level, last_shadow):
    key = (cfgs, B, T, bf16, level, last_shadow)
    ent = _STACK_PLANS.get(key)
    if ent is None:
        n = len(cfgs)
        desc = (ctypes.c_int * (6 + 6 * n))(n, B, T, bf16, level, int(last_shadow), *[v for c in cfgs for v in c])
        plan = (ctypes.c_longlong * (8 * n + 6))()
        if N.helper("v100_ir_stack_plan", desc, plan) < 0:
            raise RuntimeError("InvertedResidual stack: invalid shape")
        if len(_STACK_PLANS) > 256:
            _STACK_PLANS.clear()
        ent = _STACK_PLANS[key] = (desc, [tuple(plan[8 * i:8 * i + 8]) for i in range(n)], tuple(plan[8 * n:8 * n + 6]))
    return ent


class IRStackTrainFn(torch.autograd.Function):

    @staticmethod
    def forward(ctx, x, x16, meta, *weights):
        cfgs, precision, last_shadow, params = meta
        _check(x, "InvertedResidual stack")
        x = x.contiguous()
        B, cin, T = x.shape
        n = len(cfgs)
        if len(params) != 18 * n or len(weights) != 9 * n or cfgs[0][0] != cin:
            raise RuntimeError("InvertedResidual stack: parameter list / input width do not match the block configuration")
        bf16 = _fmt(precision)
        _no_fp16_training(bf16, "InvertedResidual (training mode)")
        level = _ACT16 if bf16 == 1 else 0
        desc, blocks, totals = _stack_plan(cfgs, B, T, bf16, level, bool(last_shadow))
        if not (bf16 == 1 and level >= 4):
            x16 = None
        blob = torch.empty(totals[0], dtype=torch.uint8, device=x.device)
        ptab = (ctypes.c_void_p * (18 * n))(*[t.data_ptr() for t in params])
        N.call("v100_ir_stack_fwd_train", desc, ptab, x, x16, blob)
        _touched([params[18 * i + j] for i in range(n) for j in (3, 4, 5, 9, 10, 11, 15, 16, 17)])
        o = blocks[-1]
        cout, T2 = cfgs[-1][2], o[7]
        y = blob[o[3]:o[3] + 4 * B * cout * T2].view(torch.float32).view(B, cout, T2)
        y16 = None
        if o[4] >= 0:
            P2 = pitch16(T2, B)
            y16 = blob[o[4]:o[4] + 2 * B * cout * P2].view(torch.bfloat16).view(B, cout, P2)
            ctx.mark_non_differentiable(y16)
        ctx.set_materialize_grads(False)
        ctx.blob, ctx.x, ctx.x16, ctx.params, ctx.desc, ctx.totals, ctx.cfgs = blob, x, x16, params, desc, totals, cfgs
        ctx.ptab = ptab
        ctx.y_shape = y.shape
        return y, y16

    @staticmethod
    def backward(ctx, dy, _dy16=None):
        x, params, cfgs, totals = ctx.x, ctx.params, ctx.cfgs, ctx.totals
        if ctx.blob is None:
            raise RuntimeError("InvertedResidual stack: backward ran already for this forward (its activations are freed as soon as "
                               "they are consumed; retain_graph / a second backward needs a second forward)")
        n = len(cfgs)
        if dy is None:
            dy = torch.zeros(ctx.y_shape, dtype=torch.float32, device=x.device)
        dy = dy.contiguous()
        weights = [params[18 * b + j] for b in range(n) for j in (0, 1, 2, 6, 7, 8, 12, 13, 14)]
        grads = _grad_arena_for(weights, totals[2]) if _GRAD_ARENAS else None
        if grads is None:
            grads = _f32(totals[2], like=x)
        ws = torch.empty(totals[1], dtype=torch.uint8, device=x.device)
        dx = torch.empty_like(x) if ctx.needs_input_grad[0] else None
        N.call("v100_ir_stack_bwd", ctx.desc, ctx.ptab, x, ctx.x16, ctx.blob, dy, dx, grads, ws)
        ctx.blob = None
        out, off = [], 0
        for i, (cin, hid, cout, k, _, _) in enumerate(cfgs):
            p = params[18 * i:18 * i + 18]
            for j, numel in ((0, hid * cin), (1, hid), (2, hid), (6, hid * k), (7, hid), (8, hid), (12, cout * hid), (13, cout), (14, cout)):
                out.append(grads[off:off + numel].view_as(p[j]))
                off += numel
        return (dx, None, None) + tuple(out)


def _stack_segments(blocks, segment):
    ent = blocks[0].__dict__.get("_v100_stack_meta")
    if ent is None or len(ent[0]) != len(blocks) or any(a is not b for a, b in zip(ent[0], blocks)):
        ent = blocks[0].__dict__["_v100_stack_meta"] = (tuple(blocks), {})
    segs = ent[1].get(segment)
    if segs is None:
        segs = []
        for s in range(0, len(blocks), segment):
            seg = blocks[s:s + segment]
            cfgs = tuple((b.conv[0][0].in_channels, b.conv[0][0].out_channels, b.conv[2].out_channels, int(b.kernel_size), int(b.stride),
                          int(bool(b.use_residual))) for b in seg)
            params = tuple(t for b in seg for t in _block_tensors(b))
            for t in params:
                if not t.is_cuda or not t.is_contiguous():
                    raise RuntimeError("InvertedResidual: parameters and buffers must be contiguous CUDA tensors (no CPU fallback)")
            segs.append((cfgs, params, seg))
        ent[1][segment] = segs
    return segs


def _stack_eligible(blocks) -> bool:
    import torch.nn.modules.module as _m
    if _m._global_forward_hooks or _m._global_forward_pre_hooks:
        return False
    for b in blocks:
        if not b.training or b._forward_hooks or b._forward_pre_hooks:
            return False
    return True


def ir_stack_train(blocks, x, precision: Optional[str] = None, segment: Optional[int] = None):
    blocks = list(blocks)
    if not _stack_eligible(blocks):
        for b in blocks:
            x = b(x)
        return x
    if segment is None:
        segment = _STACK_SEGMENT
    if segment is None:
        import torch.distributed as dist
        segment = 3 if (dist.is_available() and dist.is_initialized() and dist.get_world_size() > 1) else len(blocks)
    precision = precision or _PRECISION
    segs = _stack_segments(blocks, segment)
    for i, (cfgs, params, seg) in enumerate(segs):
        current = tuple(t for b in seg for t in _block_tensors(b))
        if any(a is not c for a, c in zip(params, current)):
            for t in current:
                if not t.is_cuda or not t.is_contiguous():
                    raise RuntimeError("InvertedResidual: parameters and buffers must be contiguous CUDA tensors (no CPU fallback)")
            params = current
            segs[i] = (cfgs, params, seg)
        sh = getattr(x, "_v100_shadow", None)
        x16 = sh[0] if (sh is not None and sh[1] == x._version and sh[0].shape[:2] == x.shape[:2]
                        and sh[0].shape[2] == pitch16(x.shape[2], x.shape[0])) else None
        last = i + 1 == len(segs)
        weights = [params[18 * b + j] for b in range(len(cfgs)) for j in (0, 1, 2, 6, 7, 8, 12, 13, 14)]
        y, y16 = IRStackTrainFn.apply(x, x16, (cfgs, precision, not last, params), *weights)
        if y16 is not None:
            y._v100_shadow = (y16, y._version)
        x = y
    return x


def prepare_block_weights(blocks, precision: Optional[str] = None) -> None:
    bf16 = _fmt(precision)
    _no_fp16_training(bf16, "InvertedResidual (training mode)")
    todo, total = [], 0
    for blk in blocks:
        w1, w3 = blk.conv[0][0].weight, blk.conv[2].weight
        if not w1.is_cuda:
            raise RuntimeError("InvertedResidual: parameters must be CUDA tensors (no CPU fallback)")
        hid, cin = w1.shape[0], w1.shape[1]
        cout = w3.shape[0]
        shape = (0, cin, hid, cout, 0, 0, 1, 0, int(bf16), 1, 0)
        nbytes = N.helper("v100_ir_prep_bytes", (ctypes.c_int * 11)(*shape))
        todo.append((blk, shape, w1, w3, total, nbytes))
        total += (nbytes + 255) // 256 * 256
    if not todo:
        return
    pool = torch.empty(total, dtype=torch.uint8, device=todo[0][2].device)
    bufs = [pool[off:off + nbytes] for _, _, _, _, off, nbytes in todo]
    for i in range(0, len(todo), 32):
        chunk = todo[i:i + 32]
        shapes = (ctypes.c_int * (11 * len(chunk)))(*[v for c in chunk for v in c[1]])
        N.call("v100_ir_prep_batched", shapes, _ptr_table([c[2] for c in chunk]), _ptr_table([c[3] for c in chunk]),
               _ptr_table(bufs[i:i + 32]), len(chunk))
    for (blk, _, _, _, _, _), buf in zip(todo, bufs):
        blk._prep_buf = buf
        blk._prep_fresh = bf16


def prepared_weights_of(blk, precision: Optional[str] = None):
    bf16 = _fmt(precision)
    fresh = getattr(blk, "_prep_fresh", None)
    if fresh is not None and fresh == bf16:
        buf, blk._prep_fresh, blk._prep_buf = blk._prep_buf, None, None
        return buf
    return None


def inverted_residual_eval_cached(blk, x, precision: Optional[str] = None):
    _check(x, "InvertedResidual")
    x = x.contiguous()
    pw, dw, pl, bn3 = blk.conv[0], blk.conv[1], blk.conv[2], blk.conv[3]
    bn1, bn2 = pw[1], dw[1]
    w1, wd, w3 = pw[0].weight, dw[0].weight, pl.weight
    bf16 = _fmt(precision)
    B, cin, T = x.shape
    hid, cout, k = w1.shape[0], w3.shape[0], int(blk.kernel_size)
    T2 = conv_out_len(T, k, blk.stride)
    shape = (ctypes.c_int * 11)(B, cin, hid, cout, T, k, int(blk.stride), int(bool(blk.use_residual)), int(bf16), 0, 0)
    params = (w1, bn1.weight, bn1.bias, bn1.running_mean, bn1.running_var, bn2.weight, bn2.bias, bn2.running_mean, bn2.running_var,
              w3, bn3.weight, bn3.bias, bn3.running_mean, bn3.running_var)
    key = (bf16,) + tuple((t.data_ptr(), t._version) for t in params) + (wd.data_ptr(), wd._version)
    if getattr(blk, "_eval_key", None) != key:
        for t in params + (wd,):
            if not t.is_cuda or not t.is_contiguous():
                raise RuntimeError("InvertedResidual: parameters and buffers must be contiguous CUDA tensors (no CPU fallback)")
        cache = torch.empty(N.helper("v100_ir_eval_cache_bytes", shape), dtype=torch.uint8, device=x.device)
        N.call("v100_ir_eval_prep", shape, _ptr_table(tuple(t.detach() for t in params) + (cache,)))
        blk._eval_cache, blk._eval_key = cache, key
    y = _f32(B, cout, T2, like=x)
    if bf16 == 1 and _ACT16 and N.helper("v100_ir_act16_supported", shape):
        shape[10] = 1
        pitch = pitch16(T, B)
        h1 = torch.empty((B, hid, pitch), dtype=torch.bfloat16, device=x.device)
        h2 = torch.empty((B, hid, pitch), dtype=torch.bfloat16, device=x.device)
    else:
        h1, h2 = _f32(B, hid, T, like=x), _f32(B, hid, T2, like=x)
    N.call("v100_ir_fwd_eval", shape, _ptr_table((x, w1.detach(), wd.detach(), w3.detach(), blk._eval_cache, h1, h2, y)))
    return y


EVAL_CM = os.environ.get("VOICE100_EVAL_CM", "1") not in ("", "0")


def eval_cm_supported(blocks, T: int, precision: Optional[str] = None, batch: int = 1) -> bool:
    import torch.nn.modules.module as _m
    if not EVAL_CM or _fmt(precision) == 0 or T > 768 or T < 1:
        return False
    if batch > 65535 or batch * pitch16(T, batch) > 0x7fffff00:
        return False
    if _m._global_forward_hooks or _m._global_forward_pre_hooks:
        return False
    for b in blocks:
        if b.training or b.stride != 1 or b._forward_hooks or b._forward_pre_hooks:
            return False
        if not N.helper("v100_dw_mfma_supported", int(b.kernel_size), 1):
            return False
        w1 = b.conv[0][0].weight
        if not w1.is_cuda or (w1.shape[0] % 2) or (w1.shape[1] % 2) or (b.conv[2].weight.shape[0] % 2):
            return False
    return True


def bct_to_cm(x: torch.Tensor) -> torch.Tensor:
    _check(x, "bct_to_cm")
    x = x.contiguous()
    B, C, T = x.shape
    P = pitch16(T, B)
    y = _f32(C, B * P, like=x)
    N.call("v100_bct_to_cm", x, y, B, C, T)
    return y


def cm_to_btc(x: torch.Tensor, B: int, T: int) -> torch.Tensor:
    C = x.shape[0]
    y = _f32(B, T, C, like=x)
    N.call("v100_cm_to_btc", x, y, B, C, T)
    return y


def inverted_residual_eval_cm(blk, x: torch.Tensor, B: int, T: int, precision: Optional[str] = None) -> torch.Tensor:
    pw, dw, pl, bn3 = blk.conv[0], blk.conv[1], blk.conv[2], blk.conv[3]
    bn1, bn2 = pw[1], dw[1]
    w1, wd, w3 = pw[0].weight, dw[0].weight, pl.weight
    fmt = _fmt(precision)
    hid, cin, cout, k = w1.shape[0], w1.shape[1], w3.shape[0], int(blk.kernel_size)
    P = pitch16(T, B)
    if x.shape != (cin, B * P):
        raise RuntimeError("inverted_residual_eval_cm: x must be [cin, B * pitch(T)]")
    shape = (ctypes.c_int * 11)(B, cin, hid, cout, T, k, 1, int(bool(blk.use_residual)), int(fmt), 0, 0)
    params = (w1, bn1.weight, bn1.bias, bn1.running_mean, bn1.running_var, bn2.weight, bn2.bias, bn2.running_mean, bn2.running_var,
              w3, bn3.weight, bn3.bias, bn3.running_mean, bn3.running_var)
    key = (fmt,) + tuple((t.data_ptr(), t._version) for t in params) + (wd.data_ptr(), wd._version)
    if getattr(blk, "_eval_key", None) != key:
        for t in params + (wd,):
            if not t.is_cuda or not t.is_contiguous():
                raise RuntimeError("InvertedResidual: parameters and buffers must be contiguous CUDA tensors (no CPU fallback)")
        cache = torch.empty(N.helper("v100_ir_eval_cache_bytes", shape), dtype=torch.uint8, device=x.device)
        N.call("v100_ir_eval_prep", shape, _ptr_table(tuple(t.detach() for t in params) + (cache,)))
        blk._eval_cache, blk._eval_key = cache, key
    shape[10] = 2
    h = torch.empty((2, hid, B * P), dtype=torch.float16 if fmt == 2 else torch.bfloat16, device=x.device)
    y = _f32(cout, B * P, like=x)
    N.call("v100_ir_fwd_eval", shape, _ptr_table((x, w1.detach(), wd.detach(), w3.detach(), blk._eval_cache, h[0], h[1], y)))
    return y


class _EvalStackPlan:
    __slots__ = ("key", "n", "shapes", "ptrs", "caches", "hid_max", "cout_max", "cout_last", "keep")


_EVAL_STACK_PLANS: "weakref.WeakKeyDictionary" = weakref.WeakKeyDictionary()


def ir_stack_eval_cm(blocks, x: torch.Tensor, B: int, T: int, precision: Optional[str] = None) -> torch.Tensor:
    fmt = _fmt(precision)
    n = len(blocks)
    P = pitch16(T, B)
    tens = [_block_tensors(b) for b in blocks]
    key = (fmt, B, T, x.device.index, n) + tuple((id(t), t.data_ptr(), t._version) for bt in tens for t in bt)
    plan = _EVAL_STACK_PLANS.get(blocks[0])
    if plan is None or plan.key != key:
        plan = _EvalStackPlan()
        plan.key, plan.n = key, n
        plan.shapes = (ctypes.c_int * (11 * n))()
        plan.ptrs = (ctypes.c_void_p * (8 * n))()
        plan.caches, plan.keep = [], []
        plan.hid_max = plan.cout_max = 0
        cin_prev = x.shape[0]
        for i, (blk, bt) in enumerate(zip(blocks, tens)):
            (w1, g1, b1, rm1, rv1, _n1, wd, g2, b2, rm2, rv2, _n2, w3, g3, b3, rm3, rv3, _n3) = bt
            hid, cin, cout, k = w1.shape[0], w1.shape[1], w3.shape[0], int(blk.kernel_size)
            if cin != cin_prev or int(blk.stride) != 1:
                raise RuntimeError("ir_stack_eval_cm: blocks must chain (cin == previous cout) at stride 1")
            cin_prev = cout
            params = (w1, g1, b1, rm1, rv1, g2, b2, rm2, rv2, w3, g3, b3, rm3, rv3)
            for t in params + (wd,):
                if not t.is_cuda or not t.is_contiguous():
                    raise RuntimeError("InvertedResidual: parameters and buffers must be contiguous CUDA tensors (no CPU fallback)")
            shape = (ctypes.c_int * 11)(B, cin, hid, cout, T, k, 1, int(bool(blk.use_residual)), int(fmt), 0, 0)
            cache = torch.empty(N.helper("v100_ir_eval_cache_bytes", shape), dtype=torch.uint8, device=x.device)
            N.call("v100_ir_eval_prep", shape, _ptr_table(tuple(t.detach() for t in params) + (cache,)))
            shape[10] = 2
            for j in range(11):
                plan.shapes[11 * i + j] = shape[j]
            plan.ptrs[8 * i + 1], plan.ptrs[8 * i + 2], plan.ptrs[8 * i + 3] = w1.data_ptr(), wd.data_ptr(), w3.data_ptr()
            plan.ptrs[8 * i + 4] = cache.data_ptr()
            plan.caches.append(cache)
            plan.keep.append(bt)
            plan.hid_max, plan.cout_max = max(plan.hid_max, hid), max(plan.cout_max, cout)
            plan.cout_last = cout
        _EVAL_STACK_PLANS[blocks[0]] = plan
    if x.shape != (plan.shapes[1], B * P):
        raise RuntimeError("ir_stack_eval_cm: x must be [cin, B * pitch(T)]")
    cols = B * P
    h = torch.empty((2, plan.hid_max, cols), dtype=torch.float16 if fmt == 2 else torch.bfloat16, device=x.device)
    out = _f32(plan.cout_last, cols, like=x)
    tmp = _f32(2, plan.cout_max, cols, like=x) if n > 1 else None
    h0, h1 = h.data_ptr(), h[1].data_ptr()
    cur = x.data_ptr()
    ptrs = plan.ptrs
    for i in range(n):
        y = out.data_ptr() if i == n - 1 else tmp[i & 1].data_ptr()
        ptrs[8 * i], ptrs[8 * i + 5], ptrs[8 * i + 6], ptrs[8 * i + 7] = cur, h0, h1, y
        cur = y
    N.call("v100_ir_stack_fwd_eval", n, plan.shapes, ptrs)
    return out


def pointwise_conv1d_cm(x: torch.Tensor, w: torch.Tensor, bias, precision: Optional[str] = None) -> torch.Tensor:
    cout, cin = w.shape[0], w.shape[1]
    n = x.shape[1]
    fmt = _fmt(precision)
    W = _weights_of(w, cout, cin, fmt, False)
    y = _f32(cout, n, like=x)
    _pw_gemm(W.w, W.w_bf, x, y, cout, cin, n, 1, fmt, bias=bias.detach() if bias is not None else None, epi=0)
    return y


def inverted_residual_eval(x, w1, g1, b1, rm1, rv1, wd, g2, b2, rm2, rv2, w3, g3, b3, rm3, rv3,
                           kernel_size, stride, use_residual, precision):
    _check(x, "InvertedResidual")
    x = x.contiguous()
    B, cin, T = x.shape
    hid, cout = w1.shape[0], w3.shape[0]
    k = int(kernel_size)
    pad = (k - 1) // 2
    T2 = conv_out_len(T, k, stride)
    bf16 = _fmt(precision)
    W1 = _Weights(w1.detach().reshape(hid, cin), bf16, False)
    W3 = _Weights(w3.detach().reshape(cout, hid), bf16, False)
    s1, t1 = _bn_eval(g1, b1, rm1, rv1, hid, x)
    s2, t2 = _bn_eval(g2, b2, rm2, rv2, hid, x)
    s3, t3 = _bn_eval(g3, b3, rm3, rv3, cout, x)
    h1 = _f32(B, hid, T, like=x)
    _pw_gemm(W1.w, W1.w_bf, x, h1, hid, cin, T, B, bf16, ea=s1, eb=t1, epi=2)
    h2 = _f32(B, hid, T2, like=x)
    G = N.helper("v100_dw_num_groups", B, hid)
    N.call("v100_dwconv", h1, None, wd.detach().reshape(hid, k).contiguous(), None, None, None, 0, h2, None, s2, t2, 1, None, G,
           B, hid, T, T2, k, stride, pad, 0, 1, 0)
    y = _f32(B, cout, T2, like=x)
    _pw_gemm(W3.w, W3.w_bf, h2, y, cout, hid, T2, B, bf16, ea=s3, eb=t3, r=x if use_residual else None, epi=3)
    return y


class PointwiseConvFn(torch.autograd.Function):

    @staticmethod
    def forward(ctx, x, w, bias, precision):
        _check(x, "pointwise_conv1d")
        x = x.contiguous()
        B, cin, T = x.shape
        cout = w.shape[0]
        bf16 = _fmt(precision)
        W = _weights_of(w, cout, cin, bf16, False)
        y = _f32(B, cout, T, like=x)
        _pw_gemm(W.w, W.w_bf, x, y, cout, cin, T, B, bf16, bias=bias.detach() if bias is not None else None, epi=0)
        ctx.save_for_backward(x, w)
        ctx.has_bias = bias is not None
        ctx.bf16 = bf16
        return y

    @staticmethod
    def backward(ctx, dy):
        x, w = ctx.saved_tensors
        dy = dy.contiguous()
        B, cin, T = x.shape
        cout = w.shape[0]
        bf16 = ctx.bf16
        _no_fp16_training(bf16, "backward")
        W = _weights_of(w, cout, cin, bf16, True)
        S = N.helper("v100_pw_wgrad_splits", B, cout, cin)
        partial = _f32(S, cout, cin, like=x)
        dW = _f32(cout, cin, like=x)
        N.call("v100_pw_wgrad", dy, None, None, None, None, 0, x, None, None, 0, partial, dW, S, B, cout, cin, T, int(bf16))
        db = None
        if ctx.has_bias:
            G = N.helper("v100_dw_num_groups", B, cout)
            part = _f32(G, cout, 2, like=x)
            N.call("v100_chan_reduce2", dy, None, part, G, B, cout, T)
            db = _f32(cout, like=x)
            N.call("v100_slab_sum0", part, G, db, cout)
        dx = None
        if ctx.needs_input_grad[0]:
            dx = _f32(B, cin, T, like=x)
            _pw_gemm(W.wt, W.wt_bf, dy, dx, cin, cout, T, B, bf16, epi=0)
        return dx, dW.view_as(w), db, None


def pointwise_conv1d(x, w, bias=None, precision: Optional[str] = None):
    return PointwiseConvFn.apply(x, w, bias, precision or _PRECISION)


class TransposeLast2Fn(torch.autograd.Function):

    @staticmethod
    def forward(ctx, x):
        _check(x, "transpose_last2")
        x = x.contiguous()
        B, R, C = x.shape
        y = _f32(B, C, R, like=x)
        N.call("v100_transpose_last2", x, y, B, R, C)
        return y

    @staticmethod
    def backward(ctx, dy):
        if not dy.is_contiguous() and dy.transpose(1, 2).is_contiguous():
            return dy.transpose(1, 2)
        dy = dy.contiguous()
        B, C, R = dy.shape
        dx = _f32(B, R, C, like=dy)
        N.call("v100_transpose_last2", dy, dx, B, C, R)
        return dx


def tag_transposed(x: torch.Tensor, xt: torch.Tensor):
    x._v100_T = (xt, x._version)


def transpose_last2(x):
    tag = getattr(x, "_v100_T", None)
    if tag is not None and tag[1] == x._version and not x.requires_grad and tag[0].device == x.device \
            and tag[0].shape == (x.shape[0], x.shape[2], x.shape[1]):
        return tag[0]
    y = TransposeLast2Fn.apply(x)
    if y.requires_grad:
        y._v100_grad_T = True
    return y


class DropoutMaskFn(torch.autograd.Function):

    @staticmethod
    def forward(ctx, x, keep, scale):
        x = x.contiguous()
        y = torch.empty_like(x)
        N.call("v100_mul_scale", x, keep, float(scale), y, x.numel())
        ctx.save_for_backward(keep)
        ctx.scale = float(scale)
        return y

    @staticmethod
    def backward(ctx, dy):
        (keep,) = ctx.saved_tensors
        dy = dy.contiguous()
        dx = torch.empty_like(dy)
        N.call("v100_mul_scale", dy, keep, ctx.scale, dx, dy.numel())
        return dx, None, None


class DropoutFn(torch.autograd.Function):

    @staticmethod
    def forward(ctx, x, p, seed):
        _check(x, "dropout")
        x = x.contiguous()
        y = torch.empty_like(x)
        mask = torch.empty(x.numel(), dtype=torch.uint8, device=x.device)
        N.call("v100_dropout_fwd", x, int(seed), float(p), y, mask, x.numel())
        ctx.save_for_backward(mask)
        ctx.p = float(p)
        return y

    @staticmethod
    def backward(ctx, dy):
        (mask,) = ctx.saved_tensors
        dy = dy.contiguous()
        dx = torch.empty_like(dy)
        N.call("v100_dropout_bwd", dy, mask, ctx.p, dx, dy.numel())
        return dx, None, None


class DropoutPointwiseFn(torch.autograd.Function):

    @staticmethod
    def forward(ctx, x, w, bias, p, seed, precision):
        _check(x, "dropout_pointwise_conv1d")
        x = x.contiguous()
        B, cin, T = x.shape
        cout = w.shape[0]
        bf16 = _fmt(precision)
        xd = torch.empty_like(x)
        mask = torch.empty(x.numel(), dtype=torch.uint8, device=x.device)
        N.call("v100_dropout_fwd", x, int(seed), float(p), xd, mask, x.numel())
        W = _weights_of(w, cout, cin, bf16, False)
        y = _f32(B, cout, T, like=x)
        _pw_gemm(W.w, W.w_bf, xd, y, cout, cin, T, B, bf16, bias=bias.detach() if bias is not None else None, epi=0)
        ctx.save_for_backward(xd, w, mask)
        ctx.has_bias = bias is not None
        ctx.bf16 = bf16
        ctx.p = float(p)
        return y

    @staticmethod
    def backward(ctx, dy):
        xd, w, mask = ctx.saved_tensors
        dy = dy.contiguous()
        B, cin, T = xd.shape
        cout = w.shape[0]
        bf16 = ctx.bf16
        _no_fp16_training(bf16, "backward")
        W = _weights_of(w, cout, cin, bf16, True)
        S = N.helper("v100_pw_wgrad_splits", B, cout, cin)
        partial = _f32(S, cout, cin, like=xd)
        dW = _f32(cout, cin, like=xd)
        N.call("v100_pw_wgrad", dy, None, None, None, None, 0, xd, None, None, 0, partial, dW, S, B, cout, cin, T, int(bf16))
        db = None
        if ctx.has_bias:
            G = N.helper("v100_dw_num_groups", B, cout)
            part = _f32(G, cout, 2, like=xd)
            N.call("v100_chan_reduce2", dy, None, part, G, B, cout, T)
            db = _f32(cout, like=xd)
            N.call("v100_slab_sum0", part, G, db, cout)
        dx = None
        if ctx.needs_input_grad[0]:
            dx = _f32(B, cin, T, like=xd)
            if N.helper("v100_pw_gemm_dropmask_supported", B, cin, cout, T, int(bf16)):
                N.call("v100_pw_gemm_dropmask", W.wt, W.wt_bf, dy, dx, mask, ctx.p, B, cin, cout, T, int(bf16))
            else:
                dz = _f32(B, cin, T, like=xd)
                _pw_gemm(W.wt, W.wt_bf, dy, dz, cin, cout, T, B, bf16, epi=0)
                N.call("v100_dropout_bwd", dz, mask, ctx.p, dx, dx.numel())
        return dx, dW.view_as(w), db, None, None, None


def dropout_pointwise_conv1d(x, w, bias, p: float, precision: Optional[str] = None):
    seed = int(torch.randint(0, 2 ** 62, (1,), dtype=torch.int64).item())
    return DropoutPointwiseFn.apply(x, w, bias, float(p), seed, precision or _PRECISION)


def dropout(x, p: float, training: bool, keep: Optional[torch.Tensor] = None):
    if not training or p == 0.0:
        return x
    if p >= 1.0:
        return x * 0.0
    if keep is not None:
        return DropoutMaskFn.apply(x, keep, 1.0 / (1.0 - p))
    seed = int(torch.randint(0, 2 ** 62, (1,), dtype=torch.int64).item())
    return DropoutFn.apply(x, p, seed)


class EmbeddingBCTFn(torch.autograd.Function):

    @staticmethod
    def forward(ctx, idx, table):
        if not idx.is_cuda:
            raise RuntimeError("embedding: voice100_amd runs on the GPU only")
        idx = idx.contiguous().to(torch.int64)
        B, T = idx.shape
        V, C = table.shape
        _check_ids(idx, V, "embedding")
        out = _f32(B, C, T, like=table)
        N.call("v100_embedding_bct", idx, table.detach().contiguous(), out, B, V, C, T)
        ctx.save_for_backward(idx)
        ctx.vc = (V, C)
        return out

    @staticmethod
    def backward(ctx, dy):
        (idx,) = ctx.saved_tensors
        V, C = ctx.vc
        dy = dy.contiguous()
        B, _, T = dy.shape
        dtable = _f32(V, C, like=dy)
        N.call("v100_embedding_bwd", idx, dy, dtable, B, V, C, T)
        return None, dtable


def embedding_bct(idx, table):
    return EmbeddingBCTFn.apply(idx, table)


def _pad_rows(x, lpad: int, tx: int, step: int = 1, off: int = 0, n: Optional[int] = None):
    B, C, T = x.shape
    n = T if n is None else n
    flat = torch.empty(B * C * tx + 64, dtype=torch.float32, device=x.device)
    xp = flat[:B * C * tx].view(B, C, tx)
    N.call("v100_pad_copy", x, xp, B, C, T, step, off, n, tx, lpad)
    return xp


USE_TAP_GEMM = True


def _taps_ok(b, m, cx, ntap, t, tx, fmt) -> bool:
    return USE_TAP_GEMM and bool(N.helper("v100_pw_taps_supported", b, m, cx, ntap, t, tx, int(fmt)))


def _gemm_taps(W, xp, y, bias, r, m, cx, t, shifts, fmt):
    B, _, tx = xp.shape
    N.call("v100_pw_gemm_taps", W.w, W.w_bf, xp, y, bias, r, B, m, cx, t, tx, len(shifts), (ctypes.c_int * len(shifts))(*shifts), int(fmt))


def _wgrad_taps(g, tg, g_off, xp, m, cx, t, shifts, fmt):
    B, _, tx = xp.shape
    kk = len(shifts) * cx
    S = N.helper("v100_pw_wgrad_splits", B, m, kk)
    partial, dW = _f32(S, m, kk, like=xp), _f32(m, kk, like=xp)
    N.call("v100_pw_wgrad_taps", g, tg, g_off, xp, partial, dW, S, B, m, cx, t, tx, len(shifts), (ctypes.c_int * len(shifts))(*shifts), int(fmt))
    return dW


class ConvTranspose1dK5S2Fn(torch.autograd.Function):

    @staticmethod
    def _stack(x):
        B, cin, L = x.shape
        xe = _f32(B, 3 * cin, L, like=x)
        xo = _f32(B, 2 * cin, L, like=x)
        for tap, d in enumerate((1, 0, -1)):
            N.call("v100_shift_copy", x, xe, None, B, cin, L, L, cin, 0, 3 * cin, tap * cin, 1, d, 1, 0, L, 0)
        for tap, d in enumerate((1, 0)):
            N.call("v100_shift_copy", x, xo, None, B, cin, L, L, cin, 0, 2 * cin, tap * cin, 1, d, 1, 0, L, 0)
        return xe, xo

    @staticmethod
    def _mats(w):
        wt = w.detach().permute(1, 2, 0)
        ae = wt[:, [0, 2, 4], :].reshape(w.shape[1], -1).contiguous()
        ao = wt[:, [1, 3], :].reshape(w.shape[1], -1).contiguous()
        return ae, ao

    @staticmethod
    def forward(ctx, x, w, bias, precision):
        _check(x, "conv_transpose1d")
        if w.shape[2] != 5:
            raise RuntimeError("conv_transpose1d: only kernel_size=5, stride=2, padding=2 is built (tts.py:22)")
        x = x.contiguous()
        B, cin, L = x.shape
        cout = w.shape[1]
        bf16 = _fmt(precision)
        def _phase_weights():
            ae, ao = ConvTranspose1dK5S2Fn._mats(w)
            return _Weights(ae, bf16, False), _Weights(ao, bf16, False)
        We, Wo = _derived(w, ("convt_fwd", int(bf16)), _phase_weights)
        ye, yo = _f32(B, cout, L, like=x), _f32(B, cout, L, like=x)
        tx = (L + 2 + 3) // 4 * 4
        ctx.taps = _taps_ok(B, cout, cin, 3, L, tx, bf16) and (bf16 == 2 or _taps_ok(B, cin, cout, 3, L, tx, bf16))
        if ctx.taps:
            xp = _pad_rows(x, 1, tx)
            _gemm_taps(We, xp, ye, None, None, cout, cin, L, (2, 1, 0), bf16)
            _gemm_taps(Wo, xp, yo, None, None, cout, cin, L, (2, 1), bf16)
        else:
            xe, xo = ConvTranspose1dK5S2Fn._stack(x)
            _pw_gemm(We.w, We.w_bf, xe, ye, cout, 3 * cin, L, B, bf16)
            _pw_gemm(Wo.w, Wo.w_bf, xo, yo, cout, 2 * cin, L, B, bf16)
        T = 2 * L - 1
        y = _f32(B, cout, T, like=x)
        b = bias.detach() if bias is not None else None
        N.call("v100_shift_copy", ye, y, b, B, cout, L, T, cout, 0, cout, 0, 1, 0, 2, 0, L, 0)
        if L > 1:
            N.call("v100_shift_copy", yo, y, b, B, cout, L, T, cout, 0, cout, 0, 1, 0, 2, 1, L - 1, 0)
        ctx.save_for_backward(x, w)
        ctx.has_bias = bias is not None
        ctx.bf16 = bf16
        return y

    @staticmethod
    def backward(ctx, dy):
        x, w = ctx.saved_tensors
        dy = dy.contiguous()
        B, cin, L = x.shape
        cout = w.shape[1]
        T = 2 * L - 1
        bf16 = ctx.bf16
        _no_fp16_training(bf16, "backward")
        if ctx.taps:
            return ConvTranspose1dK5S2Fn._backward_taps(ctx, x, w, dy)
        dye, dyo = _f32(B, cout, L, like=x), torch.zeros((B, cout, L), dtype=torch.float32, device=x.device)
        N.call("v100_shift_copy", dy, dye, None, B, cout, T, L, cout, 0, cout, 0, 2, 0, 1, 0, L, 0)
        if L > 1:
            N.call("v100_shift_copy", dy, dyo, None, B, cout, T, L, cout, 0, cout, 0, 2, 1, 1, 0, L - 1, 0)
        xe, xo = ConvTranspose1dK5S2Fn._stack(x)
        ae, ao = ConvTranspose1dK5S2Fn._mats(w)
        We, Wo = _Weights(ae, bf16, True), _Weights(ao, bf16, True)
        dae, dao = _f32(cout, 3 * cin, like=x), _f32(cout, 2 * cin, like=x)
        for g, xs, out, kk in ((dye, xe, dae, 3 * cin), (dyo, xo, dao, 2 * cin)):
            S = N.helper("v100_pw_wgrad_splits", B, cout, kk)
            partial = _f32(S, cout, kk, like=x)
            N.call("v100_pw_wgrad", g, None, None, None, None, 0, xs, None, None, 0, partial, out, S, B, cout, kk, L, int(bf16))
        dw = torch.empty_like(w)
        dw[:, :, [0, 2, 4]] = dae.view(cout, 3, cin).permute(2, 0, 1)
        dw[:, :, [1, 3]] = dao.view(cout, 2, cin).permute(2, 0, 1)
        db = None
        if ctx.has_bias:
            G = N.helper("v100_dw_num_groups", B, cout)
            part = _f32(G, cout, 2, like=x)
            N.call("v100_chan_reduce2", dy, None, part, G, B, cout, T)
            db = _f32(cout, like=x)
            N.call("v100_slab_sum0", part, G, db, cout)
        dx = None
        if ctx.needs_input_grad[0]:
            dxe, dxo = _f32(B, 3 * cin, L, like=x), _f32(B, 2 * cin, L, like=x)
            _pw_gemm(We.wt, We.wt_bf, dye, dxe, 3 * cin, cout, L, B, bf16)
            _pw_gemm(Wo.wt, Wo.wt_bf, dyo, dxo, 2 * cin, cout, L, B, bf16)
            dx = torch.zeros_like(x)
            for tap, d in enumerate((1, 0, -1)):
                N.call("v100_shift_copy", dxe, dx, None, B, cin, L, L, 3 * cin, tap * cin, cin, 0, 1, -d, 1, 0, L, 1)
            for tap, d in enumerate((1, 0)):
                N.call("v100_shift_copy", dxo, dx, None, B, cin, L, L, 2 * cin, tap * cin, cin, 0, 1, -d, 1, 0, L, 1)
        return dx, dw, db, None


def _convt_backward_taps(ctx, x, w, dy):
    B, cin, L = x.shape
    cout = w.shape[1]
    T = 2 * L - 1
    bf16 = ctx.bf16
    tx = (L + 2 + 3) // 4 * 4
    xp = _pad_rows(x, 1, tx)
    dyep = _pad_rows(dy, 1, tx, step=2, off=0, n=L)
    dyop = _pad_rows(dy, 1, tx, step=2, off=1 if L > 1 else 0, n=L - 1)
    dae = _wgrad_taps(dyep, tx, 1, xp, cout, cin, L, (2, 1, 0), bf16)
    dao = _wgrad_taps(dyop, tx, 1, xp, cout, cin, L, (2, 1), bf16)
    dw = torch.empty_like(w)
    dw[:, :, [0, 2, 4]] = dae.view(cout, 3, cin).permute(2, 0, 1)
    dw[:, :, [1, 3]] = dao.view(cout, 2, cin).permute(2, 0, 1)
    db = None
    if ctx.has_bias:
        G = N.helper("v100_dw_num_groups", B, cout)
        part = _f32(G, cout, 2, like=x)
        N.call("v100_chan_reduce2", dy, None, part, G, B, cout, T)
        db = _f32(cout, like=x)
        N.call("v100_slab_sum0", part, G, db, cout)
    dx = None
    if ctx.needs_input_grad[0]:
        wd = w.detach()
        a1 = wd[:, :, [0, 2, 4]].permute(0, 2, 1).reshape(cin, 3 * cout).contiguous()
        a2 = wd[:, :, [1, 3]].permute(0, 2, 1).reshape(cin, 2 * cout).contiguous()
        W1, W2 = _Weights(a1, bf16, False), _Weights(a2, bf16, False)
        dx1, dx = _f32(B, cin, L, like=x), _f32(B, cin, L, like=x)
        _gemm_taps(W1, dyep, dx1, None, None, cin, cout, L, (0, 1, 2), bf16)
        _gemm_taps(W2, dyop, dx, None, dx1, cin, cout, L, (0, 1), bf16)
    return dx, dw, db, None


ConvTranspose1dK5S2Fn._backward_taps = staticmethod(_convt_backward_taps)


def conv_transpose1d_k5s2(x, w, bias=None, precision: Optional[str] = None):
    return ConvTranspose1dK5S2Fn.apply(x, w, bias, precision or _PRECISION)


class Conv1dDenseFn(torch.autograd.Function):

    @staticmethod
    def forward(ctx, x, w, bias, stride, padding, precision):
        _check(x, "conv1d_dense")
        x = x.contiguous()
        B, cin, T = x.shape
        cout, cin_w, k = w.shape
        if cin_w != cin:
            raise RuntimeError(f"conv1d_dense: weight expects {cin_w} input channels, got {cin}")
        tout = (T + 2 * padding - k) // stride + 1
        if tout <= 0:
            raise RuntimeError("conv1d_dense: input shorter than the kernel")
        bf16 = _fmt(precision)
        W = _derived(w, ("dense_fwd", int(bf16)),
                     lambda: _Weights(w.detach().permute(0, 2, 1).reshape(cout, k * cin).contiguous(), bf16, False))
        y = _f32(B, cout, tout, like=x)
        bias_d = bias.detach() if bias is not None else None
        tx = (T + k - 1 + 3) // 4 * 4
        taps = (stride == 1 and 2 * padding == k - 1 and k <= 8 and _taps_ok(B, cout, cin, k, T, tx, bf16)
                and (bf16 == 2 or _taps_ok(B, cin, cout, k, T, tx, bf16)))
        if taps:
            _gemm_taps(W, _pad_rows(x, padding, tx), y, bias_d, None, cout, cin, T, tuple(range(k)), bf16)
        else:
            cols = _f32(B, k * cin, tout, like=x)
            N.call("v100_im2col", x, cols, B, cin, T, tout, k, stride, padding)
            _pw_gemm(W.w, W.w_bf, cols, y, cout, k * cin, tout, B, bf16, bias=bias_d, epi=0)
        ctx.save_for_backward(x, w)
        ctx.cfg = (stride, padding, bias is not None, bf16, tout, taps)
        return y

    @staticmethod
    def backward(ctx, dy):
        x, w = ctx.saved_tensors
        stride, padding, has_bias, bf16, tout, taps = ctx.cfg
        _no_fp16_training(bf16, "backward")
        dy = dy.contiguous()
        B, cin, T = x.shape
        cout, _, k = w.shape
        kk = k * cin
        tx = (T + k - 1 + 3) // 4 * 4
        if taps:
            dW = _wgrad_taps(dy, T, 0, _pad_rows(x, padding, tx), cout, cin, T, tuple(range(k)), bf16)
        else:
            cols = _f32(B, kk, tout, like=x)
            N.call("v100_im2col", x, cols, B, cin, T, tout, k, stride, padding)
            S = N.helper("v100_pw_wgrad_splits", B, cout, kk)
            partial = _f32(S, cout, kk, like=x)
            dW = _f32(cout, kk, like=x)
            N.call("v100_pw_wgrad", dy, None, None, None, None, 0, cols, None, None, 0, partial, dW, S, B, cout, kk, tout, int(bf16))
        dw = dW.view(cout, k, cin).permute(0, 2, 1).contiguous()
        db = None
        if has_bias:
            G = N.helper("v100_dw_num_groups", B, cout)
            part = _f32(G, cout, 2, like=x)
            N.call("v100_chan_reduce2", dy, None, part, G, B, cout, tout)
            db = _f32(cout, like=x)
            N.call("v100_slab_sum0", part, G, db, cout)
        dx = None
        if ctx.needs_input_grad[0] and taps:
            a = w.detach().flip(2).permute(1, 2, 0).reshape(cin, k * cout).contiguous()
            dx = _f32(B, cin, T, like=x)
            _gemm_taps(_Weights(a, bf16, False), _pad_rows(dy, padding, tx), dx, None, None, cin, cout, T, tuple(range(k)), bf16)
        elif ctx.needs_input_grad[0]:
            w2d = w.detach().permute(0, 2, 1).reshape(cout, kk).contiguous()
            W = _Weights(w2d, bf16, True)
            dcols = cols
            _pw_gemm(W.wt, W.wt_bf, dy, dcols, kk, cout, tout, B, bf16, epi=0)
            dx = _f32(B, cin, T, like=x)
            N.call("v100_col2im", dcols, dx, B, cin, T, tout, k, stride, padding)
        return dx, dw, db, None, None, None


def conv1d_dense(x, w, bias=None, stride: int = 1, padding: int = 0, precision: Optional[str] = None):
    return Conv1dDenseFn.apply(x, w, bias, int(stride), int(padding), precision or _PRECISION)


class LayerNormGeluFn(torch.autograd.Function):

    @staticmethod
    def forward(ctx, y, gamma, beta, eps):
        _check(y, "layer_norm_gelu")
        y = y.contiguous()
        B, C, T = y.shape
        out = _f32(B, C, T, like=y)
        mean, rstd = _f32(B, T, like=y), _f32(B, T, like=y)
        g, b = gamma.detach().contiguous(), beta.detach().contiguous()
        N.call("v100_ln_gelu_fwd", y, g, b, float(eps), out, mean, rstd, B, C, T)
        ctx.save_for_backward(y, g, b, mean, rstd)
        return out

    @staticmethod
    def backward(ctx, dout):
        y, g, b, mean, rstd = ctx.saved_tensors
        dout = dout.contiguous()
        B, C, T = y.shape
        parts = N.helper("v100_ln_num_parts", B, T)
        partial = _f32(parts, C, 2, like=y)
        dy = _f32(B, C, T, like=y)
        N.call("v100_ln_gelu_bwd", dout, y, g, b, mean, rstd, dy, partial, B, C, T)
        dg, db = _f32(C, like=y), _f32(C, like=y)
        N.call("v100_slab_sum2", partial, parts, dg, db, C)
        return dy, dg, db, None


def layer_norm_gelu(y, gamma, beta, eps: float = 1e-5):
    return LayerNormGeluFn.apply(y, gamma, beta, eps)


def world_unnormalize_gate(x_bta, f0_mean, f0_std, ls_mean, ls_std, ca_mean, ca_std):
    _check(x_bta, "world_unnormalize")
    x_bta = x_bta.contiguous()
    B, T, A = x_bta.shape
    S, cap = ls_mean.shape[0], ca_mean.shape[0]
    assert A == 2 + S + cap
    f0 = _f32(B, T, like=x_bta)
    logspc = _f32(B, T, S, like=x_bta)
    codeap = _f32(B, T, cap, like=x_bta)
    N.call("v100_world_unnormalize", x_bta, f0, logspc, codeap, f0_mean, f0_std, ls_mean, ls_std, ca_mean, ca_std, B, T, S, cap)
    return f0, logspc, codeap



class WorldLossFn(torch.autograd.Function):

    @staticmethod
    def forward(ctx, pred, length, hasf0, f0, logspc, codeap, norm, weights, l1):
        _check(pred, "world_loss")
        pred = pred.contiguous()
        B, Tp, A = pred.shape
        S, cap = logspc.shape[2], codeap.shape[2]
        if A != 2 + S + cap:
            raise RuntimeError(f"world_loss: pred has {A} features, targets imply {2 + S + cap}")
        Tt = f0.shape[1]
        dev = pred.device
        f0, logspc, codeap = (t.to(device=dev, dtype=torch.float32).contiguous() for t in (f0, logspc, codeap))
        if logspc.shape[1] != Tt or codeap.shape[1] != Tt:
            raise RuntimeError("world_loss: targets must share one time axis")
        hasf0 = None if hasf0 is None else hasf0.to(device=dev, dtype=torch.float32).contiguous()
        length = length.to(device=dev, dtype=torch.int32).contiguous()
        nrm = [None] * 6 if norm is None else [t.detach().to(device=dev, dtype=torch.float32).contiguous() for t in norm]
        w = None if weights is None else weights.detach().to(device=dev, dtype=torch.float32).contiguous()
        partial = _f32(N.helper("v100_world_loss_parts", B, Tp), 4, like=pred)
        loss = _f32(4, like=pred)
        unit = torch.empty_like(pred)
        N.call("v100_world_loss", pred, f0, hasf0, logspc, codeap, length, *nrm, w, partial, loss, unit, B, Tp, Tt, S, cap, int(l1))
        ctx.save_for_backward(unit)
        ctx.dims = (B, Tp, S, cap)
        return loss

    @staticmethod
    def backward(ctx, gout):
        (unit,) = ctx.saved_tensors
        B, Tp, S, cap = ctx.dims
        dpred = torch.empty_like(unit)
        N.call("v100_world_loss_bwd", unit, gout.to(torch.float32).contiguous(), dpred, B, Tp, S, cap)
        return (dpred,) + (None,) * 8


def world_loss(pred_bta, length, hasf0, f0, logspc, codeap, norm=None, weights=None, loss: str = "mse"):
    if loss not in ("l1", "mse"):
        raise ValueError("Unknown loss type")
    return WorldLossFn.apply(pred_bta, length, hasf0, f0, logspc, codeap, norm, weights, loss == "l1")


def world_unnormalize_gate_v2(x_bta, f0_mean, f0_std, ls_mean, ls_std, ca_mean, ca_std):
    if x_bta.is_cuda and x_bta.dtype in (torch.float16, torch.bfloat16):
        x_bta = x_bta.float()
    _check(x_bta, "world_unnormalize_v2")
    x_bta = x_bta.contiguous()
    B, T, A = x_bta.shape
    S, cap = ls_mean.shape[0], ca_mean.shape[0]
    if A != 2 + S + 2 * cap:
        raise RuntimeError(f"world_unnormalize_v2: x has {A} features, the norm implies {2 + S + 2 * cap}")
    f0 = _f32(B, T, like=x_bta)
    logspc = _f32(B, T, S, like=x_bta)
    codeap = _f32(B, T, cap, like=x_bta)
    nv = [t.detach().float().contiguous() for t in (f0_mean, f0_std, ls_mean, ls_std, ca_mean, ca_std)]
    N.call("v100_world_unnormalize_v2", x_bta, f0, logspc, codeap, *nv, B, T, S, cap)
    return f0, logspc, codeap


class WorldLossV2Fn(torch.autograd.Function):

    @staticmethod
    def forward(ctx, pred, length, f0, logspc, codeap, norm, l1):
        _check(pred, "world_loss_v2")
        pred = pred.contiguous()
        B, Tp, A = pred.shape
        S, cap = logspc.shape[2], codeap.shape[2]
        if A != 2 + S + 2 * cap:
            raise RuntimeError(f"world_loss_v2: pred has {A} features, targets imply {2 + S + 2 * cap}")
        Tt = f0.shape[1]
        dev = pred.device
        f0, logspc, codeap = (t.to(device=dev, dtype=torch.float32).contiguous() for t in (f0, logspc, codeap))
        if logspc.shape[1] != Tt or codeap.shape[1] != Tt or f0.shape[0] != B or logspc.shape[0] != B or codeap.shape[0] != B:
            raise RuntimeError("world_loss_v2: targets must be [B, Tt(, C)] with one time axis")
        length = length.to(device=dev, dtype=torch.int32).contiguous()
        if length.shape != (B,):
            raise RuntimeError("world_loss_v2: length must be [B]")
        nrm = [t.detach().to(device=dev, dtype=torch.float32).contiguous() for t in norm]
        partial = _f32(N.helper("v100_world_loss_parts", B, Tp), 5, like=pred)
        loss = _f32(5, like=pred)
        unit = torch.empty_like(pred)
        N.call("v100_world_loss_v2", pred, f0, logspc, codeap, length, *nrm, partial, loss, unit, B, Tp, Tt, S, cap, int(l1))
        ctx.save_for_backward(unit)
        ctx.dims = (B, Tp, S, cap)
        return loss

    @staticmethod
    def backward(ctx, gout):
        (unit,) = ctx.saved_tensors
        B, Tp, S, cap = ctx.dims
        dpred = torch.empty_like(unit)
        N.call("v100_world_loss_v2_bwd", unit, gout.to(torch.float32).contiguous(), dpred, B, Tp, S, cap)
        return (dpred,) + (None,) * 6


def world_loss_v2(pred_bta, length, f0, logspc, codeap, norm, loss: str = "mse"):
    if loss not in ("l1", "mse"):
        raise ValueError("Unknown loss type")
    return WorldLossV2Fn.apply(pred_bta, length, f0, logspc, codeap, tuple(norm), loss == "l1")


class AlignLossFn(torch.autograd.Function):

    @staticmethod
    def forward(ctx, pred, align, text_len):
        _check(pred, "align_loss")
        pred = pred.contiguous()
        B, L, two = pred.shape
        if two != 2:
            raise RuntimeError("align_loss: pred must be [B, L, 2]")
        dev = pred.device
        align = align.to(device=dev, dtype=torch.int64).contiguous()
        W = align.shape[1]
        if align.shape[0] != B or W - 1 != 2 * L:
            raise RuntimeError(f"align_loss: align [B, 2L+1] = [{B}, {2 * L + 1}] expected, got {list(align.shape)}")
        text_len = text_len.to(device=dev, dtype=torch.int32).contiguous()
        partial = _f32(N.helper("v100_align_loss_parts", B, L), like=pred)
        loss = _f32(1, like=pred)
        unit = torch.empty_like(pred)
        N.call("v100_align_loss", pred, align, text_len, partial, loss, unit, B, L, W)
        ctx.save_for_backward(unit)
        return loss[0]

    @staticmethod
    def backward(ctx, gout):
        (unit,) = ctx.saved_tensors
        B, L, _ = unit.shape
        dpred = torch.empty_like(unit)
        N.call("v100_align_loss_bwd", unit, gout.to(torch.float32).reshape(1).contiguous(), dpred, B, L)
        return dpred, None, None


def align_loss(pred_bl2, align, text_len):
    return AlignLossFn.apply(pred_bl2, align, text_len)


class MaskedCrossEntropyFn(torch.autograd.Function):

    @staticmethod
    def forward(ctx, logits, target, target_len):
        _check(logits, "masked_cross_entropy")
        logits = logits.contiguous()
        B, V, L = logits.shape
        dev = logits.device
        target = target.to(device=dev, dtype=torch.int64).contiguous()
        target_len = target_len.to(device=dev, dtype=torch.int32).contiguous()
        if CHECK_IDS and target.numel():
            _check_ids(torch.where(target == -100, torch.zeros_like(target), target), V, "masked_cross_entropy targets")
        parts = N.helper("v100_masked_ce_parts", B, L)
        if parts < 0:
            raise RuntimeError(f"masked_cross_entropy: invalid shape {list(logits.shape)}")
        partial = _f32(parts, like=logits)
        loss = _f32(1, like=logits)
        unit = torch.empty_like(logits)
        N.call("v100_masked_ce", logits, target, target_len, partial, loss, unit, B, V, L)
        ctx.save_for_backward(unit)
        return loss[0]

    @staticmethod
    def backward(ctx, gout):
        (unit,) = ctx.saved_tensors
        B, V, L = unit.shape
        dlogits = torch.empty_like(unit)
        N.call("v100_masked_ce_bwd", unit, gout.to(torch.float32).reshape(1).contiguous(), dlogits, B, V, L)
        return dlogits, None, None


def _masked_cross_entropy_stock(logits_bvl, target, target_len):
    ce = torch.nn.functional.cross_entropy(logits_bvl, target, reduction="none")
    mask = (torch.arange(target.shape[1], device=target.device)[None, :] < target_len.to(target.device)[:, None]).to(ce.dtype)
    return torch.sum(ce * mask) / torch.sum(mask)


def masked_cross_entropy(logits_bvl, target, target_len):
    if logits_bvl.dim() != 3 or target.dim() != 2 or target_len.dim() != 1:
        raise RuntimeError("masked_cross_entropy: logits [B, V, L], target [B, L], target_len [B] expected")
    B, V, L = logits_bvl.shape
    if target.shape[0] != B or target.shape[1] != L or target_len.shape[0] != B:
        raise RuntimeError(f"masked_cross_entropy: logits {list(logits_bvl.shape)} need target [{B}, {L}] and target_len [{B}], got "
                           f"{list(target.shape)} and {list(target_len.shape)}")
    from ._base import tracing
    if not logits_bvl.is_cuda or tracing():
        return _masked_cross_entropy_stock(logits_bvl, target, target_len)
    return MaskedCrossEntropyFn.apply(logits_bvl, target, target_len)


class CTCLossFn(torch.autograd.Function):

    @staticmethod
    def forward(ctx, logits, targets, input_lengths, target_lengths, blank, grad_bvt=False):
        _check(logits, "ctc_loss")
        logits = logits.contiguous()
        B, T, V = logits.shape
        targets = targets.to(device=logits.device, dtype=torch.int64).contiguous()
        lmax = targets.shape[1]
        if lmax > 2047:
            raise RuntimeError(f"ctc_loss: padded target width {lmax} exceeds the kernel's 2047-token limit")
        _check_ids(targets, V, "ctc_loss targets")
        il = input_lengths.to(device=logits.device, dtype=torch.int32).contiguous()
        tl = target_lengths.to(device=logits.device, dtype=torch.int32).contiguous()
        nws = N.helper("v100_ctc_workspace_floats", B, T, lmax)
        if nws < 0:
            raise RuntimeError("ctc_loss: workspace too large")
        ws = _f32(nws, like=logits)
        nll = _f32(B, like=logits)
        loss = _f32(1, like=logits)
        grad = _f32(B, V, T, like=logits) if grad_bvt else torch.empty_like(logits)
        N.call("v100_ctc_loss_mean_t", logits, targets, il, tl, ws, nll, loss, grad, int(bool(grad_bvt)), B, T, V, lmax, int(blank))
        ctx.save_for_backward(grad)
        ctx.handed_out = False
        ctx.grad_bvt = bool(grad_bvt)
        return loss[0]

    @staticmethod
    def backward(ctx, gout):
        (grad,) = ctx.saved_tensors
        if ctx.handed_out:
            raise RuntimeError("ctc_loss: second backward after the unit-root-gradient shortcut handed out the saved gradient; "
                               "call backward() with an explicit gradient tensor (not functional.unit_grad) when retaining the graph")
        if ctx.grad_bvt:
            grad = grad.transpose(1, 2)
        if is_unit_grad(gout):
            ctx.handed_out = True
            return grad, None, None, None, None, None
        return grad * gout, None, None, None, None, None


_UNIT_GRADS = {}


def unit_grad(like: torch.Tensor) -> torch.Tensor:
    key = (like.device, like.dtype)
    one = _UNIT_GRADS.get(key)
    if one is None:
        one = _UNIT_GRADS[key] = torch.ones((), device=like.device, dtype=like.dtype)
    return one


def is_unit_grad(g: torch.Tensor) -> bool:
    one = _UNIT_GRADS.get((g.device, g.dtype))
    return one is not None and g.dim() == 0 and g.data_ptr() == one.data_ptr()


def tag_half_length(lengths: torch.Tensor, half: torch.Tensor) -> None:
    lengths._v100_half = (half, lengths._version)


def half_length(lengths: torch.Tensor):
    tag = getattr(lengths, "_v100_half", None)
    if tag is not None and tag[1] == lengths._version and tag[0].device == lengths.device:
        return tag[0] if tag[0].dtype == lengths.dtype else tag[0].to(lengths.dtype)
    return None


def ctc_loss(logits_btv, targets, input_lengths, target_lengths, blank: int = 0):
    grad_bvt = bool(getattr(logits_btv, "_v100_grad_T", False)) and logits_btv.requires_grad
    return CTCLossFn.apply(logits_btv, targets, input_lengths, target_lengths, blank, grad_bvt)


LSTM_PERSISTENT = os.environ.get("V100_LSTM_PERSISTENT", "1") not in ("", "0")


def _lstm_sync(sync: torch.Tensor, layer, what: str) -> None:
    code = int(sync[0].item())
    if code:
        raise RuntimeError(f"lstm layer {layer}: the {what} recurrence gave up waiting for a hand-off at step {code - 1} "
                           "(the outputs of this call are invalid)")


def _lstm_prep(w0, w1, H, ndir, fmt, backward, like):
    buf = torch.empty(int(N.helper("v100_lstm_weight_bytes", H, ndir, fmt, backward)), dtype=torch.uint8, device=like.device)
    N.call("v100_lstm_weight_prep", w0.detach(), None if w1 is None else w1.detach(), H, ndir, fmt, backward, buf)
    return buf


def _lstm_scratch(B, H, ndir, backward, like):
    ws = torch.empty(int(N.helper("v100_lstm_ws_bytes", B, H, ndir, backward)), dtype=torch.uint8, device=like.device)
    sync = torch.empty(int(N.helper("v100_lstm_sync_words", B, ndir)), dtype=torch.int32, device=like.device)
    return ws, sync


class LSTMLayerFn(torch.autograd.Function):

    @staticmethod
    def forward(ctx, x, lens, precision, persistent, layer, train, w_ih0, w_hh0, b_ih0, b_hh0, w_ih1, w_hh1, b_ih1, b_hh1):
        _check(x, "lstm")
        x = x.contiguous()
        B, C, T = x.shape
        H = w_hh0.shape[1]
        ndir = 1 if w_ih1 is None else 2
        fmt = _fmt(precision)
        if train:
            _no_fp16_training(fmt, "lstm")
        xproj = _f32(ndir, B, 4 * H, T, like=x)
        for d, (w_ih, b_ih) in enumerate(((w_ih0, b_ih0), (w_ih1, b_ih1))[:ndir]):
            W = _weights_of(w_ih, 4 * H, C, fmt, False)
            _pw_gemm(W.w, W.w_bf, x, xproj[d], 4 * H, C, T, B, fmt, bias=None if b_ih is None else b_ih.detach())
        wp = _lstm_prep(w_hh0, w_hh1, H, ndir, fmt, 0, x)
        ws, sync = _lstm_scratch(B, H, ndir, 0, x)
        y = _f32(B, ndir * H, T, like=x)
        hn = torch.zeros((ndir, B, H), dtype=torch.float32, device=x.device)
        cn = torch.zeros((ndir, B, H), dtype=torch.float32, device=x.device)
        act = cs = hprev = None
        if train:
            act, cs, hprev = _f32(ndir, T, B, 4 * H, like=x), _f32(ndir, T, B, H, like=x), _f32(ndir, B, H, T, like=x)
        bh = [None if b is None else b.detach() for b in (b_hh0, b_hh1)]
        N.call("v100_lstm_fwd", xproj, wp, bh[0], bh[1], lens, y, hn, cn, act, cs, hprev, ws, sync, B, T, H, ndir, fmt,
               int(bool(persistent)))
        _lstm_sync(sync, layer, "forward")
        if train:
            ctx.save_for_backward(x, lens, act, cs, hprev, w_ih0, w_hh0, w_ih1, w_hh1)
        ctx.meta = (fmt, bool(persistent), layer, b_ih0 is not None, ndir, H)
        return y, hn, cn

    @staticmethod
    def backward(ctx, dy, dhn, dcn):
        x, lens, act, cs, hprev, w_ih0, w_hh0, w_ih1, w_hh1 = ctx.saved_tensors
        fmt, persistent, layer, has_bias, ndir, H = ctx.meta
        B, C, T = x.shape
        H4 = 4 * H
        dy = dy.contiguous()
        dhn = None if dhn is None else dhn.contiguous()
        dcn = None if dcn is None else dcn.contiguous()
        wp = _lstm_prep(w_hh0, w_hh1, H, ndir, fmt, 1, x)
        ws, sync = _lstm_scratch(B, H, ndir, 1, x)
        dg = _f32(ndir, B, H4, T, like=x)
        N.call("v100_lstm_bwd", dy, dhn, dcn, wp, lens, act, cs, dg, ws, sync, B, T, H, ndir, fmt, int(persistent))
        _lstm_sync(sync, layer, "backward")
        grads = []
        for d, (w_ih, w_hh) in enumerate(((w_ih0, w_hh0), (w_ih1, w_hh1))[:ndir]):
            out = []
            for w, xin, cin in ((w_ih, x, C), (w_hh, hprev[d], H)):
                S = N.helper("v100_pw_wgrad_splits", B, H4, cin)
                partial = _f32(S, H4, cin, like=x)
                dW = _f32(H4, cin, like=x)
                N.call("v100_pw_wgrad", dg[d], None, None, None, None, 0, xin, None, None, 0, partial, dW, S, B, H4, cin, T, fmt)
                out.append(dW)
            db = dbh = None
            if has_bias:
                G = N.helper("v100_dw_num_groups", B, H4)
                part = _f32(G, H4, 2, like=x)
                N.call("v100_chan_reduce2", dg[d], None, part, G, B, H4, T)
                db = _f32(H4, like=x)
                N.call("v100_slab_sum0", part, G, db, H4)
                dbh = db.clone()
            grads += [out[0], out[1], db, dbh]
        if ndir == 1:
            grads += [None] * 4
        dx = None
        if ctx.needs_input_grad[0]:
            dx = _f32(B, C, T, like=x)
            r = None
            if ndir == 2:
                W1 = _weights_of(w_ih1, H4, C, fmt, True)
                r = _f32(B, C, T, like=x)
                _pw_gemm(W1.wt, W1.wt_bf, dg[1], r, C, H4, T, B, fmt, epi=0)
            W0 = _weights_of(w_ih0, H4, C, fmt, True)
            _pw_gemm(W0.wt, W0.wt_bf, dg[0], dx, C, H4, T, B, fmt, r=r, epi=5 if r is not None else 0)
        return (dx, None, None, None, None, None, *grads)


def lstm_layer(x, lens, params, precision: Optional[str] = None, persistent: Optional[bool] = None, layer: int = 0):
    p = list(params) + [None] * (8 - len(params))
    train = torch.is_grad_enabled() and any(t is not None and t.requires_grad for t in [x] + p)
    return LSTMLayerFn.apply(x, lens, precision or _PRECISION, LSTM_PERSISTENT if persistent is None else persistent, layer, train,
                             *p)
```

voice100_amd/optim.py:

```python
import math

import numpy as np
import torch

from . import _native as N


RING = 32


class FusedAdam(torch.optim.Optimizer):
    def __init__(self, params, lr=1e-3, betas=(0.9, 0.999), eps=1e-8, weight_decay=0.0):
        if lr < 0 or eps < 0 or weight_decay < 0 or not 0 <= betas[0] < 1 or not 0 <= betas[1] < 1:
            raise ValueError("invalid Adam hyper-parameters")
        super().__init__(params, dict(lr=lr, betas=betas, eps=eps, weight_decay=weight_decay))
        self._tables = None
        self._partials = None
        self.last_grad_norm = None

    def load_state_dict(self, state_dict):
        super().load_state_dict(state_dict)
        self._tables = None

    def add_param_group(self, param_group):
        super().add_param_group(param_group)
        self._tables = None

    def _build(self, group):
        ps = [p for p in group["params"] if p.requires_grad]
        if not ps:
            return None
        dev = ps[0].device
        for p in ps:
            if not p.is_cuda or p.dtype != torch.float32 or not p.is_contiguous() or p.device != dev:
                raise RuntimeError("FusedAdam: parameters must be contiguous float32 CUDA tensors on one device")
        n = sum(p.numel() for p in ps)
        flat_m = torch.zeros(n, dtype=torch.float32, device=dev)
        flat_v = torch.zeros(n, dtype=torch.float32, device=dev)
        off = 0
        m_ptrs, v_ptrs, p_ptrs = [], [], []
        for p in ps:
            k = p.numel()
            st = self.state[p]
            if "exp_avg" in st:
                flat_m[off:off + k].copy_(st["exp_avg"].reshape(-1))
                flat_v[off:off + k].copy_(st["exp_avg_sq"].reshape(-1))
            st["exp_avg"] = flat_m[off:off + k].view_as(p)
            st["exp_avg_sq"] = flat_v[off:off + k].view_as(p)
            st.setdefault("step", torch.tensor(0.0))
            m_ptrs.append(flat_m.data_ptr() + 4 * off)
            v_ptrs.append(flat_v.data_ptr() + 4 * off)
            p_ptrs.append(p.data_ptr())
            off += k
        chunks, nchunks = _chunk_table([p.numel() for p in ps], dev)
        t = {"params": ps, "chunks": chunks, "nchunks": nchunks, "p": _to_dev(np.array(p_ptrs, dtype=np.uint64), dev),
             "m": _to_dev(np.array(m_ptrs, dtype=np.uint64), dev), "v": _to_dev(np.array(v_ptrs, dtype=np.uint64), dev),
             "g": _PtrTable(len(ps), dev), "flat": (flat_m, flat_v), "step": 0, "p_ptrs": p_ptrs}
        t["step"] = int(max(float(self.state[p]["step"]) for p in ps))
        return t

    def _upload_grads(self, t):
        ps = t["params"]
        grads = [p.grad for p in ps]
        f32 = torch.float32
        try:
            bad = [i for i, g in enumerate(grads) if g.dtype is not f32 or not g.is_contiguous() or not g.is_cuda]
        except AttributeError:
            raise RuntimeError("FusedAdam: every parameter needs a gradient each step (the reference's models produce one)") from None
        for i in bad:
            grads[i] = ps[i].grad = grads[i].to(device=ps[i].device, dtype=f32).contiguous()
        if [p.data_ptr() for p in ps] != t["p_ptrs"]:
            raise RuntimeError("FusedAdam: a parameter's storage moved since the optimizer was built (re-create the optimizer)")
        t["g"].update([g.data_ptr() for g in grads])
        return grads

    @torch.no_grad()
    def step(self, closure=None, *, max_grad_norm=None, norm_type=2.0, grad_clip_value=None):
        if max_grad_norm is not None and grad_clip_value is not None:
            raise ValueError("FusedAdam.step: pass max_grad_norm or grad_clip_value, not both")
        loss = None
        if closure is not None:
            with torch.enable_grad():
                loss = closure()
        if self._tables is None:
            self._tables = [self._build(g) for g in self.param_groups]
            self._partials = None
        live = [(group, t) for group, t in zip(self.param_groups, self._tables) if t is not None]
        grads = [self._upload_grads(t) for _, t in live]
        self.last_grad_norm = None
        if max_grad_norm is not None and live:
            mode, clip, code = CLIP_NORM, float(max_grad_norm), _norm_code(norm_type)
            if self._partials is None:
                self._partials = torch.empty(sum(t["nchunks"] for _, t in live), dtype=torch.float64, device=live[0][1]["chunks"].device)
            base = self._partials.data_ptr()
            for _, t in live:
                N.call("v100_grad_norm_partials", t["chunks"], t["nchunks"], t["g"].dev, base, code)
                base += 8 * t["nchunks"]
            self.last_grad_norm = torch.empty((), dtype=torch.float32, device=self._partials.device)
            partials, npartials = self._partials, self._partials.numel()
        elif grad_clip_value is not None:
            mode, clip, code, partials, npartials = CLIP_VALUE, float(grad_clip_value), NORM_L2, None, 0
        else:
            mode = None
        for gi, (group, t) in enumerate(live):
            ps = t["params"]
            t["step"] += 1
            b1, b2 = group["betas"]
            if mode is None:
                N.call("v100_adam_step", t["chunks"], t["nchunks"], t["p"], t["g"].dev, t["m"], t["v"], float(group["lr"]), float(b1),
                       float(b2), float(group["eps"]), float(group["weight_decay"]), t["step"])
            else:
                N.call("v100_adam_step_clip", t["chunks"], t["nchunks"], t["p"], t["g"].dev, t["m"], t["v"], float(group["lr"]), float(b1),
                       float(b2), float(group["eps"]), float(group["weight_decay"]), t["step"], mode, clip, partials, npartials, code,
                       self.last_grad_norm if gi == 0 else None)
                torch.autograd.graph.increment_version(grads[gi])
            torch.autograd.graph.increment_version(ps)
            st = t.get("step_tensor")
            if st is None or any(self.state[p].get("step") is not st for p in ps[:1]):
                st = t["step_tensor"] = torch.tensor(float(t["step"]))
                for p in ps:
                    self.state[p]["step"] = st
            else:
                st.fill_(float(t["step"]))
        return loss


NORM_L2, NORM_INF = 2, -1
CLIP_NORM, CLIP_VALUE = 1, 2


def _norm_code(norm_type):
    nt = float(norm_type)
    if nt == 2.0:
        return NORM_L2
    if nt == math.inf:
        return NORM_INF
    raise ValueError(f"norm_type must be 2.0 or inf (the norms the HIP kernels compute), got {norm_type!r}")


def _to_dev(a, dev):
    return torch.from_numpy(np.ascontiguousarray(a).view(np.uint8).copy()).to(dev)


def _chunk_table(numels, dev):
    ce = N.helper("v100_adam_chunk_elems")
    rec = np.array([(ti, min(ce, k - o), o) for ti, k in enumerate(numels) for o in range(0, k, ce)],
                   dtype=np.dtype([("tensor", "<i4"), ("count", "<i4"), ("offset", "<i8")]))
    return _to_dev(rec, dev), len(rec)


class _PtrTable:

    def __init__(self, n, dev):
        self.dev = torch.empty(8 * n, dtype=torch.uint8, device=dev)
        self.ring = [torch.empty(8 * n, dtype=torch.uint8).pin_memory() for _ in range(RING)]
        self.events = [None] * RING
        self.pos = 0
        self.ptrs = None

    def update(self, ptrs):
        if ptrs == self.ptrs:
            return
        slot = self.pos % RING
        self.pos += 1
        host = self.ring[slot]
        if self.events[slot] is not None:
            self.events[slot].synchronize()
        host.numpy().view(np.uint64)[:] = ptrs
        self.dev.copy_(host, non_blocking=True)
        ev = torch.cuda.Event()
        ev.record()
        self.events[slot] = ev
        self.ptrs = ptrs


_clip_tables = {}


def _grad_tables(grads):
    dev = grads[0].device
    for g in grads:
        if not g.is_cuda or g.dtype != torch.float32 or not g.is_contiguous() or g.device != dev:
            raise RuntimeError("voice100_amd gradient clipping takes contiguous float32 CUDA gradients on one device")
    key = (dev, tuple(g.numel() for g in grads))
    t = _clip_tables.get(key)
    if t is None:
        if len(_clip_tables) >= 8:
            _clip_tables.clear()
        chunks, n = _chunk_table(key[1], dev)
        t = _clip_tables[key] = {"chunks": chunks, "nchunks": n, "g": _PtrTable(len(grads), dev),
                                 "partials": torch.empty(n, dtype=torch.float64, device=dev)}
    t["g"].update([g.data_ptr() for g in grads])
    return t


def _grads(parameters):
    if isinstance(parameters, torch.Tensor):
        parameters = [parameters]
    return [p.grad for p in parameters if p.grad is not None and p.grad.numel()]


@torch.no_grad()
def clip_grad_norm_(parameters, max_norm, norm_type=2.0, error_if_nonfinite=False):
    code = _norm_code(norm_type)
    grads = _grads(parameters)
    if not grads:
        return torch.tensor(0.0)
    t = _grad_tables(grads)
    N.call("v100_grad_norm_partials", t["chunks"], t["nchunks"], t["g"].dev, t["partials"], code)
    if error_if_nonfinite and not bool(torch.isfinite(t["partials"]).all()):
        raise RuntimeError(
            f"The total norm of order {float(norm_type)} for gradients from `parameters` is non-finite, so it cannot be clipped. To "
            "disable this error and scale the gradients by the non-finite norm anyway, set `error_if_nonfinite=False`")
    total = torch.empty((), dtype=torch.float32, device=grads[0].device)
    N.call("v100_grad_clip", t["chunks"], t["nchunks"], t["g"].dev, CLIP_NORM, float(max_norm), t["partials"], t["nchunks"], code, total)
    torch.autograd.graph.increment_version(grads)
    return total


@torch.no_grad()
def clip_grad_value_(parameters, clip_value):
    grads = _grads(parameters)
    if not grads:
        return
    t = _grad_tables(grads)
    N.call("v100_grad_clip", t["chunks"], t["nchunks"], t["g"].dev, CLIP_VALUE, float(clip_value), None, 0, NORM_L2, None)
    torch.autograd.graph.increment_version(grads)
```

Before: 10.67 million.

## Fuse bf16 weight and transposed-weight prep into the Adam optimizer step

The Adam kernel now also writes bf16 copies of selected pointwise weights, both row-major and transposed through an LDS tile, into a pool. The next forward and backward stack calls reuse these copies instead of converting the fp32 weights themselves. The aim is to drop the separate per-iteration weight-prep passes and their extra reads of fp32 weights. In exchange the optimizer kernel does more work, its chunk tables become tile-based, and keeping the prepared copies valid depends on version tracking between the optimizer and the modules.

New measurement: 10.64 million (median of 2 runs). Within noise of the previous version (-0.3%).

```diff
diff --git a/include/voice100_hip.h b/include/voice100_hip.h
--- a/include/voice100_hip.h
+++ b/include/voice100_hip.h
@@ -171,6 +171,16 @@
 int v100_adam_step_clip(const void* chunks, int nchunks, const void* params, const void* grads, const void* exp_avg,
                         const void* exp_avg_sq, double lr, double beta1, double beta2, double eps, double weight_decay, int step,
                         int clip_mode, double clip, const void* partials, int npartials, int norm_type, void* total_norm, void* stream);
+int v100_adam_prep_tile(void);
+int v100_adam_prep_max_tiles(void);
+int v100_adam_prep_fits(int rows, int cols, long long bf_off, long long tbf_off);
+int v100_adam_step_prep(const void* prep_chunks, int nchunks, const void* params, const void* grads, const void* exp_avg,
+                        const void* exp_avg_sq, double lr, double beta1, double beta2, double eps, double weight_decay, int step,
+                        const void* prep, void* pool, void* stream);
+int v100_adam_step_clip_prep(const void* prep_chunks, int nchunks, const void* params, const void* grads, const void* exp_avg,
+                             const void* exp_avg_sq, double lr, double beta1, double beta2, double eps, double weight_decay, int step,
+                             int clip_mode, double clip, const void* partials, int npartials, int norm_type, void* total_norm,
+                             const void* prep, void* pool, void* stream);
 int v100_grad_clip(const void* chunks, int nchunks, const void* grads, int clip_mode, double clip, const void* partials, int npartials,
                    int norm_type, void* total_norm, void* stream);
 
@@ -183,6 +193,7 @@
                          float* nll, float* loss, float* grad, int grad_bvt, int B, int T, int V, int Lmax, int blank, void* stream);
 
 long long v100_ir_prep_bytes(const int* shape);
+long long v100_ir_prep_offsets(const int* shape, long long* out);
 long long v100_ir_fwd_workspace_bytes(const int* shape);
 long long v100_ir_eval_cache_bytes(const int* shape);
 int v100_ir_eval_prep(const int* shape, const void* const* ptrs, void* stream);
@@ -197,6 +208,10 @@
 int v100_ir_stack_fwd_train(const int* desc, const void* const* params, const void* x, const void* x16, void* blob, void* stream);
 int v100_ir_stack_bwd(const int* desc, const void* const* params, const void* x, const void* x16, const void* blob, const void* dy,
                       void* dx, void* grads, void* ws, void* stream);
+int v100_ir_stack_fwd_train_prep(const int* desc, const void* const* params, const void* x, const void* x16, void* blob,
+                                 const void* const* preps, void* stream);
+int v100_ir_stack_bwd_prep(const int* desc, const void* const* params, const void* x, const void* x16, const void* blob, const void* dy,
+                           void* dx, void* grads, void* ws, const void* const* preps, void* stream);
 int v100_ir_stack_wgrad_plan(const int* desc, int have_x16, int min_problem_tiles, int min_flush_tiles, long long* out);
 int v100_ir_stack_wgrad_group_thresholds(int min_problem_tiles, int min_flush_tiles);
 
diff --git a/voice100_amd/csrc/adam.hip b/voice100_amd/csrc/adam.hip
--- a/voice100_amd/csrc/adam.hip
+++ b/voice100_amd/csrc/adam.hip
@@ -11,52 +11,7 @@
     pv -= lr_over_bc1 * mv / (sqrtf(vv) * inv_sqrt_bc2 + eps);
 }
 
-__global__ __launch_bounds__(256) void adam_step_kernel(const AdamChunk* __restrict__ chunks, float* const* __restrict__ params,
-                                                        const float* const* __restrict__ grads, float* const* __restrict__ exp_avg,
-                                                        float* const* __restrict__ exp_avg_sq, float lr_over_bc1, float omb1,
-                                                        float beta2, float omb2, float eps, float weight_decay, float inv_sqrt_bc2) {
-    const AdamChunk ch = chunks[blockIdx.x];
-    float* __restrict__ p = params[ch.tensor] + ch.offset;
-    const float* __restrict__ g = grads[ch.tensor] + ch.offset;
-    float* __restrict__ m = exp_avg[ch.tensor] + ch.offset;
-    float* __restrict__ v = exp_avg_sq[ch.tensor] + ch.offset;
-    auto upd = [&](float& pv, float gv, float& mv, float& vv) {
-        adam_update(pv, gv, mv, vv, lr_over_bc1, omb1, beta2, omb2, eps, weight_decay, inv_sqrt_bc2);
-    };
-    const bool vec = ((((size_t)p | (size_t)g | (size_t)m | (size_t)v) & 15) == 0);
-    if (vec) {
-        const int n4 = ch.count >> 2;
-        for (int i = threadIdx.x; i < n4; i += 256) {
-            f32x4 pv = reinterpret_cast<f32x4*>(p)[i], mv = reinterpret_cast<f32x4*>(m)[i], vv = reinterpret_cast<f32x4*>(v)[i];
-            const f32x4 gv = reinterpret_cast<const f32x4*>(g)[i];
-#pragma unroll
-            for (int e = 0; e < 4; ++e) {
-                float a = pv[e], b = mv[e], c = vv[e];
-                upd(a, gv[e], b, c);
-                pv[e] = a; mv[e] = b; vv[e] = c;
-            }
-            reinterpret_cast<f32x4*>(p)[i] = pv; reinterpret_cast<f32x4*>(m)[i] = mv; reinterpret_cast<f32x4*>(v)[i] = vv;
-        }
-        for (int i = (n4 << 2) + threadIdx.x; i < ch.count; i += 256) upd(p[i], g[i], m[i], v[i]);
-    } else {
-        for (int i = threadIdx.x; i < ch.count; i += 256) upd(p[i], g[i], m[i], v[i]);
-    }
-}
-
 extern "C" int v100_adam_chunk_elems() { return 16384; }
-
-extern "C" int v100_adam_step(const void* chunks, int nchunks, const void* params, const void* grads, const void* exp_avg,
-                              const void* exp_avg_sq, double lr, double beta1, double beta2, double eps, double weight_decay, int step,
-                              void* stream) {
-    if (!chunks || !params || !grads || !exp_avg || !exp_avg_sq) return V100_ERR_NULL;
-    if (nchunks <= 0 || step < 1) return V100_ERR_SHAPE;
-    const double bc1 = 1.0 - pow(beta1, (double)step), bc2 = 1.0 - pow(beta2, (double)step);
-    V100_GGL(adam_step_kernel, dim3((unsigned)nchunks), dim3(256), 0, (hipStream_t)stream, (const AdamChunk*)chunks,
-                       (float* const*)params, (const float* const*)grads, (float* const*)exp_avg, (float* const*)exp_avg_sq,
-                       (float)(lr / bc1), (float)(1.0 - beta1), (float)beta2, (float)(1.0 - beta2), (float)eps, (float)weight_decay,
-                       (float)(1.0 / sqrt(bc2)));
-    return v100_launch_status();
-}
 
 #define V100_NORM_L2 2
 #define V100_NORM_INF (-1)
@@ -120,24 +75,97 @@
     if (threadIdx.x == 0) partials[blockIdx.x] = r;
 }
 
-template <int MODE>
-__global__ __launch_bounds__(256) void adam_step_clip_kernel(const AdamChunk* __restrict__ chunks, float* const* __restrict__ params,
-                                                             float* const* __restrict__ grads, float* const* __restrict__ exp_avg,
-                                                             float* const* __restrict__ exp_avg_sq, float lr_over_bc1, float omb1,
-                                                             float beta2, float omb2, float eps, float weight_decay, float inv_sqrt_bc2,
-                                                             float clip, const double* __restrict__ partials, int npartials, int inf,
-                                                             float* __restrict__ total_out) {
+struct AdamPrepDst { long long bf_off, tbf_off; int rows, cols; };
+#define AP_TILE 64
+#define AP_PITCH 65
+#define AP_MAX_TILES 4
+
+extern "C" int v100_adam_prep_tile() { return AP_TILE; }
+extern "C" int v100_adam_prep_max_tiles() { return AP_MAX_TILES; }
+
+__device__ __forceinline__ unsigned bf_pair(float lo, float hi) { return (unsigned)f2bf(lo) | ((unsigned)f2bf(hi) << 16); }
+
+template <int MODE, bool PREP>
+__global__ __launch_bounds__(256) void adam_step_kernel(const AdamChunk* __restrict__ chunks, float* const* __restrict__ params,
+                                                        float* const* __restrict__ grads, float* const* __restrict__ exp_avg,
+                                                        float* const* __restrict__ exp_avg_sq, float lr_over_bc1, float omb1,
+                                                        float beta2, float omb2, float eps, float weight_decay, float inv_sqrt_bc2,
+                                                        float clip, const double* __restrict__ partials, int npartials, int inf,
+                                                        float* __restrict__ total_out, const AdamPrepDst* __restrict__ prep,
+                                                        char* __restrict__ pool) {
     __shared__ double lds[4];
+    __shared__ float tile[PREP ? AP_TILE * AP_PITCH : 1];
     const float coef = MODE == V100_CLIP_NORM ? clip_coef(partials, npartials, inf != 0, clip, total_out, lds) : 1.f;
-    const bool write_g = MODE == V100_CLIP_VALUE || coef != 1.f;
+    const bool write_g = MODE == V100_CLIP_VALUE || (MODE == V100_CLIP_NORM && coef != 1.f);
     const AdamChunk ch = chunks[blockIdx.x];
+    auto upd = [&](float& pv, float& gv, float& mv, float& vv) {
+        if (MODE == V100_CLIP_NORM) gv = gv * coef;
+        if (MODE == V100_CLIP_VALUE) gv = clamp_value(gv, clip);
+        adam_update(pv, gv, mv, vv, lr_over_bc1, omb1, beta2, omb2, eps, weight_decay, inv_sqrt_bc2);
+    };
+    AdamPrepDst d = {0, 0, 0, 0};
+    if (PREP) d = prep[ch.tensor];
+    if (PREP) {
+        if (d.rows > 0) {
+            float* __restrict__ p = params[ch.tensor];
+            float* __restrict__ g = grads[ch.tensor];
+            float* __restrict__ m = exp_avg[ch.tensor];
+            float* __restrict__ v = exp_avg_sq[ch.tensor];
+            u16* __restrict__ wbf = reinterpret_cast<u16*>(pool + d.bf_off);
+            u16* __restrict__ wtbf = reinterpret_cast<u16*>(pool + d.tbf_off);
+            const int rows = d.rows, cols = d.cols;
+            const int r0 = (int)(ch.offset / cols), cb = (int)(ch.offset % cols);
+            for (int s = 0; s < ch.count; ++s) {
+                const int c0 = cb + s * AP_TILE;
+                if (s) __syncthreads();
+#pragma unroll
+                for (int q = 0; q < 4; ++q) {
+                    const int id = threadIdx.x + 256 * q;
+                    const int i = ((id >> 7) << 3) | ((id >> 3) & 7), j = (((id >> 6) & 1) << 3) | (id & 7);
+                    const size_t o = (size_t)(r0 + i) * cols + c0 + 4 * j;
+                    f32x4 pv = *reinterpret_cast<const f32x4u*>(p + o), mv = *reinterpret_cast<const f32x4u*>(m + o);
+                    f32x4 vv = *reinterpret_cast<const f32x4u*>(v + o), gv = *reinterpret_cast<const f32x4u*>(g + o);
+#pragma unroll
+                    for (int e = 0; e < 4; ++e) {
+                        float a = pv[e], b = mv[e], c = vv[e], gg = gv[e];
+                        upd(a, gg, b, c);
+                        pv[e] = a; mv[e] = b; vv[e] = c; gv[e] = gg;
+                    }
+                    if (write_g) *reinterpret_cast<f32x4u*>(g + o) = gv;
+                    *reinterpret_cast<f32x4u*>(p + o) = pv; *reinterpret_cast<f32x4u*>(m + o) = mv; *reinterpret_cast<f32x4u*>(v + o) = vv;
+                    uint2 pk; pk.x = bf_pair(pv[0], pv[1]); pk.y = bf_pair(pv[2], pv[3]);
+                    *reinterpret_cast<uint2*>(wbf + o) = pk;
+#pragma unroll
+                    for (int e = 0; e < 4; ++e) tile[i * AP_PITCH + 4 * j + e] = pv[e];
+                }
+                __syncthreads();
+#pragma unroll
+                for (int q = 0; q < 2; ++q) {
+                    const int l = threadIdx.x & 63;
+                    const int c = 32 * q + 8 * (threadIdx.x >> 6) + ((l >> 2) & 7), k = (l & 3) | ((l >> 5) << 2);
+                    const float* __restrict__ t = tile + 8 * k * AP_PITCH + c;
+                    uint4 pk;
+                    pk.x = bf_pair(t[0], t[AP_PITCH]); pk.y = bf_pair(t[2 * AP_PITCH], t[3 * AP_PITCH]);
+                    pk.z = bf_pair(t[4 * AP_PITCH], t[5 * AP_PITCH]); pk.w = bf_pair(t[6 * AP_PITCH], t[7 * AP_PITCH]);
+                    *reinterpret_cast<uint4*>(wtbf + (size_t)(c0 + c) * rows + r0 + 8 * k) = pk;
+                }
+            }
+            return;
+        }
+    }
     float* __restrict__ p = params[ch.tensor] + ch.offset;
     float* __restrict__ g = grads[ch.tensor] + ch.offset;
     float* __restrict__ m = exp_avg[ch.tensor] + ch.offset;
     float* __restrict__ v = exp_avg_sq[ch.tensor] + ch.offset;
-    auto cl = [&](float x) { return MODE == V100_CLIP_NORM ? x * coef : clamp_value(x, clip); };
-    auto upd = [&](float& pv, float gv, float& mv, float& vv) {
-        adam_update(pv, gv, mv, vv, lr_over_bc1, omb1, beta2, omb2, eps, weight_decay, inv_sqrt_bc2);
+    const bool small = PREP && d.rows < 0;
+    u16* __restrict__ wbf = small ? reinterpret_cast<u16*>(pool + d.bf_off) + ch.offset : nullptr;
+    u16* __restrict__ wtbf = small ? reinterpret_cast<u16*>(pool + d.tbf_off) : nullptr;
+    const int srows = -d.rows, scols = d.cols;
+    auto copies = [&](int i, float pv) {
+        const u16 b = f2bf(pv);
+        const int idx = (int)ch.offset + i;
+        wbf[i] = b;
+        wtbf[(size_t)(idx % scols) * srows + idx / scols] = b;
     };
     int i0 = 0;
     if (((((size_t)p | (size_t)g | (size_t)m | (size_t)v) & 15) == 0)) {
@@ -147,20 +175,25 @@
             f32x4 gv = reinterpret_cast<const f32x4*>(g)[i];
 #pragma unroll
             for (int e = 0; e < 4; ++e) {
-                gv[e] = cl(gv[e]);
-                float a = pv[e], b = mv[e], c = vv[e];
-                upd(a, gv[e], b, c);
-                pv[e] = a; mv[e] = b; vv[e] = c;
+                float a = pv[e], b = mv[e], c = vv[e], gg = gv[e];
+                upd(a, gg, b, c);
+                pv[e] = a; mv[e] = b; vv[e] = c; gv[e] = gg;
             }
             if (write_g) reinterpret_cast<f32x4*>(g)[i] = gv;
             reinterpret_cast<f32x4*>(p)[i] = pv; reinterpret_cast<f32x4*>(m)[i] = mv; reinterpret_cast<f32x4*>(v)[i] = vv;
+            if (small) {
+#pragma unroll
+                for (int e = 0; e < 4; ++e) copies(4 * i + e, pv[e]);
+            }
         }
         i0 = n4 << 2;
     }
     for (int i = i0 + threadIdx.x; i < ch.count; i += 256) {
-        const float gv = cl(g[i]);
+        float gv = g[i], pv = p[i];
+        upd(pv, gv, m[i], v[i]);
+        p[i] = pv;
         if (write_g) g[i] = gv;
-        upd(p[i], gv, m[i], v[i]);
+        if (small) copies(i, pv);
     }
 }
 
@@ -209,6 +242,38 @@
     return clip_mode == V100_CLIP_VALUE ? V100_OK : V100_ERR_SHAPE;
 }
 
+static int adam_launch(const void* chunks, int nchunks, const void* params, const void* grads, const void* exp_avg, const void* exp_avg_sq,
+                       double lr, double beta1, double beta2, double eps, double weight_decay, int step, int clip_mode, double clip,
+                       const void* partials, int npartials, int norm_type, void* total_norm, const void* prep, void* pool, void* stream) {
+    const double bc1 = 1.0 - pow(beta1, (double)step), bc2 = 1.0 - pow(beta2, (double)step);
+    const int inf = norm_type == V100_NORM_INF;
+#define V100_ADAM_LAUNCH(MODE, PREP)                                                                                                      \
+    V100_GGL((adam_step_kernel<MODE, PREP>), dim3((unsigned)nchunks), dim3(256), 0, (hipStream_t)stream, (const AdamChunk*)chunks,        \
+             (float* const*)params, (float* const*)grads, (float* const*)exp_avg, (float* const*)exp_avg_sq, (float)(lr / bc1),           \
+             (float)(1.0 - beta1), (float)beta2, (float)(1.0 - beta2), (float)eps, (float)weight_decay, (float)(1.0 / sqrt(bc2)),         \
+             (float)clip, (const double*)partials, npartials, inf, (float*)total_norm, (const AdamPrepDst*)prep, (char*)pool)
+    if (prep) {
+        if (clip_mode == V100_CLIP_NORM) V100_ADAM_LAUNCH(V100_CLIP_NORM, true);
+        else if (clip_mode == V100_CLIP_VALUE) V100_ADAM_LAUNCH(V100_CLIP_VALUE, true);
+        else V100_ADAM_LAUNCH(0, true);
+    } else {
+        if (clip_mode == V100_CLIP_NORM) V100_ADAM_LAUNCH(V100_CLIP_NORM, false);
+        else if (clip_mode == V100_CLIP_VALUE) V100_ADAM_LAUNCH(V100_CLIP_VALUE, false);
+        else V100_ADAM_LAUNCH(0, false);
+    }
+#undef V100_ADAM_LAUNCH
+    return v100_launch_status();
+}
+
+extern "C" int v100_adam_step(const void* chunks, int nchunks, const void* params, const void* grads, const void* exp_avg,
+                              const void* exp_avg_sq, double lr, double beta1, double beta2, double eps, double weight_decay, int step,
+                              void* stream) {
+    if (!chunks || !params || !grads || !exp_avg || !exp_avg_sq) return V100_ERR_NULL;
+    if (nchunks <= 0 || step < 1) return V100_ERR_SHAPE;
+    return adam_launch(chunks, nchunks, params, grads, exp_avg, exp_avg_sq, lr, beta1, beta2, eps, weight_decay, step, 0, 0.0, nullptr, 0,
+                       V100_NORM_L2, nullptr, nullptr, nullptr, stream);
+}
+
 extern "C" int v100_adam_step_clip(const void* chunks, int nchunks, const void* params, const void* grads, const void* exp_avg,
                                    const void* exp_avg_sq, double lr, double beta1, double beta2, double eps, double weight_decay, int step,
                                    int clip_mode, double clip, const void* partials, int npartials, int norm_type, void* total_norm,
@@ -216,17 +281,34 @@
     if (!chunks || !params || !grads || !exp_avg || !exp_avg_sq) return V100_ERR_NULL;
     if (nchunks <= 0 || step < 1) return V100_ERR_SHAPE;
     if (int rc = check_clip(clip_mode, clip, partials, npartials, norm_type)) return rc;
-    const double bc1 = 1.0 - pow(beta1, (double)step), bc2 = 1.0 - pow(beta2, (double)step);
-    const int inf = norm_type == V100_NORM_INF;
-#define V100_ADAM_CLIP_LAUNCH(MODE)                                                                                                       \
-    V100_GGL(adam_step_clip_kernel<MODE>, dim3((unsigned)nchunks), dim3(256), 0, (hipStream_t)stream, (const AdamChunk*)chunks,         \
-             (float* const*)params, (float* const*)grads, (float* const*)exp_avg, (float* const*)exp_avg_sq, (float)(lr / bc1),           \
-             (float)(1.0 - beta1), (float)beta2, (float)(1.0 - beta2), (float)eps, (float)weight_decay, (float)(1.0 / sqrt(bc2)),         \
-             (float)clip, (const double*)partials, npartials, inf, (float*)total_norm)
-    if (clip_mode == V100_CLIP_NORM) V100_ADAM_CLIP_LAUNCH(V100_CLIP_NORM);
-    else V100_ADAM_CLIP_LAUNCH(V100_CLIP_VALUE);
-#undef V100_ADAM_CLIP_LAUNCH
-    return v100_launch_status();
+    return adam_launch(chunks, nchunks, params, grads, exp_avg, exp_avg_sq, lr, beta1, beta2, eps, weight_decay, step, clip_mode, clip,
+                       partials, npartials, norm_type, total_norm, nullptr, nullptr, stream);
+}
+
+extern "C" int v100_adam_prep_fits(int rows, int cols, long long bf_off, long long tbf_off) {
+    if (rows <= 0 || cols <= 0 || bf_off < 0 || tbf_off < 0 || bf_off % 16 || tbf_off % 16) return 0;
+    if (rows % AP_TILE == 0 && cols % AP_TILE == 0) return 1;
+    return (long long)rows * cols <= v100_adam_chunk_elems() ? 2 : 0;
+}
+
+extern "C" int v100_adam_step_prep(const void* prep_chunks, int nchunks, const void* params, const void* grads, const void* exp_avg,
+                                   const void* exp_avg_sq, double lr, double beta1, double beta2, double eps, double weight_decay,
+                                   int step, const void* prep, void* pool, void* stream) {
+    if (!prep_chunks || !params || !grads || !exp_avg || !exp_avg_sq || !prep || !pool) return V100_ERR_NULL;
+    if (nchunks <= 0 || step < 1 || ((size_t)pool & 15)) return V100_ERR_SHAPE;
+    return adam_launch(prep_chunks, nchunks, params, grads, exp_avg, exp_avg_sq, lr, beta1, beta2, eps, weight_decay, step, 0, 0.0,
+                       nullptr, 0, V100_NORM_L2, nullptr, prep, pool, stream);
+}
+
+extern "C" int v100_adam_step_clip_prep(const void* prep_chunks, int nchunks, const void* params, const void* grads, const void* exp_avg,
+                                        const void* exp_avg_sq, double lr, double beta1, double beta2, double eps, double weight_decay,
+                                        int step, int clip_mode, double clip, const void* partials, int npartials, int norm_type,
+                                        void* total_norm, const void* prep, void* pool, void* stream) {
+    if (!prep_chunks || !params || !grads || !exp_avg || !exp_avg_sq || !prep || !pool) return V100_ERR_NULL;
+    if (nchunks <= 0 || step < 1 || ((size_t)pool & 15)) return V100_ERR_SHAPE;
+    if (int rc = check_clip(clip_mode, clip, partials, npartials, norm_type)) return rc;
+    return adam_launch(prep_chunks, nchunks, params, grads, exp_avg, exp_avg_sq, lr, beta1, beta2, eps, weight_decay, step, clip_mode, clip,
+                       partials, npartials, norm_type, total_norm, prep, pool, stream);
 }
 
 extern "C" int v100_grad_clip(const void* chunks, int nchunks, const void* grads, int clip_mode, double clip, const void* partials,
diff --git a/voice100_amd/csrc/block.hip b/voice100_amd/csrc/block.hip
--- a/voice100_amd/csrc/block.hip
+++ b/voice100_amd/csrc/block.hip
@@ -49,6 +49,14 @@
 extern "C" long long v100_ir_prep_bytes(const int* shape) {
     IrPrep w;
     return (long long)ir_prep_carve(shape, nullptr, w);
+}
+extern "C" long long v100_ir_prep_offsets(const int* shape, long long* out) {
+    if (!shape || !out || shape[IR_BF16] != 1) return -1;
+    IrPrep w;
+    const size_t n = ir_prep_carve(shape, (void*)256, w);
+    out[0] = (char*)w.w1bf - (char*)256; out[1] = (char*)w.w1tbf - (char*)256;
+    out[2] = (char*)w.w3bf - (char*)256; out[3] = (char*)w.w3tbf - (char*)256;
+    return (long long)n;
 }
 
 static size_t ir_fwd_carve(const int* sh, void* base, float** stats) {
@@ -592,8 +600,8 @@
     return (long long)blob;
 }
 
-extern "C" int v100_ir_stack_fwd_train(const int* desc, const void* const* params, const void* x, const void* x16, void* blob,
-                                       void* stream) {
+extern "C" int v100_ir_stack_fwd_train_prep(const int* desc, const void* const* params, const void* x, const void* x16, void* blob,
+                                            const void* const* preps, void* stream) {
     if (!desc || !params || !x || !blob) return V100_ERR_NULL;
     StackBlock blk[32];
     size_t blob_bytes, bws, gf, fwo;
@@ -601,7 +609,10 @@
     const int n = desc[ST_N];
     char* base = (char*)blob;
     int rc;
-    {
+    if (preps) {
+        if (desc[ST_BF16] != 1) return V100_ERR_SHAPE;
+        for (int i = 0; i < n; ++i) if (!preps[i]) return V100_ERR_NULL;
+    } else {
         int shapes[32 * IR_NSHAPE];
         const void* w1s[32]; const void* w3s[32]; void* preps[32];
         for (int i = 0; i < n; ++i) {
@@ -618,7 +629,7 @@
         P[0] = xin;
         for (int j = 0; j < 18; ++j) P[1 + j] = params[18 * i + j];
         P[19] = base + b.a1; P[20] = base + b.a2; P[21] = base + b.a3; P[22] = base + b.y; P[23] = base + b.coef;
-        P[24] = base + fwo; P[25] = base + b.prep;
+        P[24] = base + fwo; P[25] = preps ? preps[i] : base + b.prep;
         P[26] = xin16; P[27] = b.y16 >= 0 ? base + b.y16 : nullptr;
         CK(v100_ir_fwd_train(b.sh, P, stream));
         xin = base + b.y;
@@ -627,9 +638,18 @@
     return V100_OK;
 }
 
-extern "C" int v100_ir_stack_bwd(const int* desc, const void* const* params, const void* x, const void* x16, const void* blob,
-                                 const void* dy, void* dx, void* grads, void* ws, void* stream) {
+extern "C" int v100_ir_stack_fwd_train(const int* desc, const void* const* params, const void* x, const void* x16, void* blob,
+                                       void* stream) {
+    return v100_ir_stack_fwd_train_prep(desc, params, x, x16, blob, nullptr, stream);
+}
+
+extern "C" int v100_ir_stack_bwd_prep(const int* desc, const void* const* params, const void* x, const void* x16, const void* blob,
+                                      const void* dy, void* dx, void* grads, void* ws, const void* const* preps, void* stream) {
     if (!desc || !params || !x || !blob || !dy || !grads || !ws) return V100_ERR_NULL;
+    if (preps) {
+        if (desc[ST_BF16] != 1 || desc[ST_N] <= 0 || desc[ST_N] > 32) return V100_ERR_SHAPE;
+        for (int i = 0; i < desc[ST_N]; ++i) if (!preps[i]) return V100_ERR_NULL;
+    }
     StackBlock blk[32];
     size_t blob_bytes, bws, gf, fwo;
     if (!stack_layout(desc, blk, blob_bytes, bws, gf, fwo)) return V100_ERR_SHAPE;
@@ -694,7 +714,7 @@
         P[13] = q; q += (size_t)hid * cin; P[14] = q; q += hid; P[15] = q; q += hid;
         P[16] = q; q += (size_t)hid * k; P[17] = q; q += hid; P[18] = q; q += hid;
         P[19] = q; q += (size_t)cout * hid; P[20] = q; q += cout; P[21] = q;
-        P[22] = w0; P[23] = base + b.prep;
+        P[22] = w0; P[23] = preps ? preps[i] : base + b.prep;
         P[24] = i > 0 ? (blk[i - 1].y16 >= 0 ? (const void*)(base + blk[i - 1].y16) : nullptr) : x16;
         CK(v100_ir_bwd(b.sh, P, stream));
         if (defer[i]) {
@@ -716,3 +736,9 @@
     }
     return V100_OK;
 }
+
+
+extern "C" int v100_ir_stack_bwd(const int* desc, const void* const* params, const void* x, const void* x16, const void* blob,
+                                 const void* dy, void* dx, void* grads, void* ws, void* stream) {
+    return v100_ir_stack_bwd_prep(desc, params, x, x16, blob, dy, dx, grads, ws, nullptr, stream);
+}
diff --git a/voice100_amd/functional.py b/voice100_amd/functional.py
--- a/voice100_amd/functional.py
+++ b/voice100_amd/functional.py
@@ -83,11 +83,17 @@
 
 class _Weights:
 
-    def __init__(self, w2d: torch.Tensor, fmt, transposed: bool):
+    def __init__(self, w2d: torch.Tensor, fmt, transposed: bool, adopted=None):
         fmt = int(fmt)
         self.w = w2d
         m, k = w2d.shape
         self.w_bf = self.wt = self.wt_bf = None
+        if adopted is not None:
+            buf, (ob, ot) = adopted
+            self.w_bf = buf[ob:ob + 2 * m * k].view(torch.bfloat16).view(m, k)
+            if transposed:
+                self.wt_bf = buf[ot:ot + 2 * m * k].view(torch.bfloat16).view(k, m)
+            return
         if fmt == 2:
             _no_fp16_training(2 if transposed else 0, "backward GEMM")
             self.w_bf = torch.empty((m, k), dtype=torch.float16, device=w2d.device)
@@ -123,14 +129,92 @@
 
 def clear_derived_cache() -> None:
     _DERIVED.clear()
+    for u in _PREP_UNITS.values():
+        u.ready = None
 
 
 def _weights_of(w: torch.Tensor, rows: int, cols: int, fmt, transposed: bool) -> "_Weights":
-    return _derived(w, ("w", rows, cols, int(fmt), bool(transposed)), lambda: _Weights(w.detach().reshape(rows, cols), fmt, transposed))
+    def build():
+        adopted = None
+        if int(fmt) == 1 and w.is_cuda and isinstance(w, torch.nn.Parameter):
+            u = _single_prep_unit(w, rows, cols)
+            buf = _adopt(u, (w,))
+            if buf is not None:
+                adopted = (buf, u.offs[0])
+        return _Weights(w.detach().reshape(rows, cols), fmt, transposed, adopted)
+    return _derived(w, ("w", rows, cols, int(fmt), bool(transposed)), build)
 
 
 def _touched(tensors) -> None:
     torch.autograd.graph.increment_version(tensors)
+
+
+class _PrepUnit:
+    __slots__ = ("refs", "dims", "offs", "nbytes", "kinds", "fits", "ready", "__weakref__")
+
+
+_PREP_UNITS = {}
+_PREP_GEN = [0]
+
+
+def _prep_unit_drop(key) -> None:
+    if _PREP_UNITS.pop(key, None) is not None:
+        _PREP_GEN[0] += 1
+
+
+def _prep_unit(weights, dims, offsets):
+    key = id(weights[0])
+    u = _PREP_UNITS.get(key)
+    if u is not None and u.dims == dims and len(u.refs) == len(weights) and all(r() is w for r, w in zip(u.refs, weights)):
+        return u
+    u = _PrepUnit()
+    u.refs = tuple(weakref.ref(w) for w in weights[1:])
+    u.refs = (weakref.ref(weights[0], lambda _r, k=key: _prep_unit_drop(k)),) + u.refs
+    u.dims = dims
+    u.offs, u.nbytes = offsets()
+    u.kinds = tuple(N.helper("v100_adam_prep_fits", r, c, ob, ot) for (r, c), (ob, ot) in zip(dims, u.offs))
+    u.fits = all(u.kinds)
+    u.ready = None
+    _PREP_UNITS[key] = u
+    _PREP_GEN[0] += 1
+    return u
+
+
+def _block_prep_unit(w1, w3):
+    key = id(w1)
+    u = _PREP_UNITS.get(key)
+    if u is not None:
+        r = u.refs
+        if len(r) == 2 and r[0]() is w1 and r[1]() is w3:
+            return u
+    hid, cin, cout = w1.shape[0], w1.shape[1], w3.shape[0]
+
+    def offsets():
+        out = (ctypes.c_longlong * 4)()
+        n = N.helper("v100_ir_prep_offsets", (ctypes.c_int * 11)(0, cin, hid, cout, 0, 0, 1, 0, 1, 1, 0), out)
+        if n <= 0:
+            raise RuntimeError("v100_ir_prep_offsets failed")
+        return ((out[0], out[1]), (out[2], out[3])), int(n)
+    return _prep_unit((w1, w3), ((hid, cin), (cout, hid)), offsets)
+
+
+def _single_prep_unit(w, rows, cols):
+    n = (2 * rows * cols + 255) // 256 * 256
+    return _prep_unit((w,), ((rows, cols),), lambda: (((0, n),), 2 * n))
+
+
+def _adopt(u, weights):
+    r = u.ready
+    if r is None:
+        return None
+    for w, ver, ptr in zip(weights, r[0], r[1]):
+        if w._version != ver or w.data_ptr() != ptr:
+            return None
+    return r[2]
+
+
+def prep_units():
+    return list(_PREP_UNITS.values())
 
 
 def _pw_gemm(a_f32, a_bf, x, y, m, k, t, b, bf16, x2=None, xa=None, xb=None, xc=None, x_mode=0, bias=None,
@@ -329,7 +413,22 @@
             x16 = None
         blob = torch.empty(totals[0], dtype=torch.uint8, device=x.device)
         ptab = (ctypes.c_void_p * (18 * n))(*[t.data_ptr() for t in params])
-        N.call("v100_ir_stack_fwd_train", desc, ptab, x, x16, blob)
+        preps = None
+        if bf16 == 1:
+            preps = []
+            for i in range(n):
+                w1, w3 = params[18 * i], params[18 * i + 12]
+                buf = _adopt(_block_prep_unit(w1, w3), (w1, w3))
+                if buf is None:
+                    preps = None
+                elif preps is not None:
+                    preps.append(buf)
+        if preps is None:
+            N.call("v100_ir_stack_fwd_train", desc, ptab, x, x16, blob)
+            ctx.preps = None
+        else:
+            ctx.preps = (preps, _ptr_table(preps))
+            N.call("v100_ir_stack_fwd_train_prep", desc, ptab, x, x16, blob, ctx.preps[1])
         _touched([params[18 * i + j] for i in range(n) for j in (3, 4, 5, 9, 10, 11, 15, 16, 17)])
         o = blocks[-1]
         cout, T2 = cfgs[-1][2], o[7]
@@ -361,7 +460,11 @@
             grads = _f32(totals[2], like=x)
         ws = torch.empty(totals[1], dtype=torch.uint8, device=x.device)
         dx = torch.empty_like(x) if ctx.needs_input_grad[0] else None
-        N.call("v100_ir_stack_bwd", ctx.desc, ctx.ptab, x, ctx.x16, ctx.blob, dy, dx, grads, ws)
+        if ctx.preps is None:
+            N.call("v100_ir_stack_bwd", ctx.desc, ctx.ptab, x, ctx.x16, ctx.blob, dy, dx, grads, ws)
+        else:
+            N.call("v100_ir_stack_bwd_prep", ctx.desc, ctx.ptab, x, ctx.x16, ctx.blob, dy, dx, grads, ws, ctx.preps[1])
+            ctx.preps = None
         ctx.blob = None
         out, off = [], 0
         for i, (cin, hid, cout, k, _, _) in enumerate(cfgs):
@@ -443,6 +546,11 @@
         w1, w3 = blk.conv[0][0].weight, blk.conv[2].weight
         if not w1.is_cuda:
             raise RuntimeError("InvertedResidual: parameters must be CUDA tensors (no CPU fallback)")
+        if bf16 == 1:
+            buf = _adopt(_block_prep_unit(w1, w3), (w1, w3))
+            if buf is not None:
+                blk._prep_buf, blk._prep_fresh = buf, bf16
+                continue
         hid, cin = w1.shape[0], w1.shape[1]
         cout = w3.shape[0]
         shape = (0, cin, hid, cout, 0, 0, 1, 0, int(bf16), 1, 0)
diff --git a/voice100_amd/optim.py b/voice100_amd/optim.py
--- a/voice100_amd/optim.py
+++ b/voice100_amd/optim.py
@@ -1,4 +1,5 @@
 import math
+import weakref
 
 import numpy as np
 import torch
@@ -7,13 +8,15 @@
 
 
 RING = 32
+SMALL_CHUNK = 1024
 
 
 class FusedAdam(torch.optim.Optimizer):
-    def __init__(self, params, lr=1e-3, betas=(0.9, 0.999), eps=1e-8, weight_decay=0.0):
+    def __init__(self, params, lr=1e-3, betas=(0.9, 0.999), eps=1e-8, weight_decay=0.0, prepare_weights=True):
         if lr < 0 or eps < 0 or weight_decay < 0 or not 0 <= betas[0] < 1 or not 0 <= betas[1] < 1:
             raise ValueError("invalid Adam hyper-parameters")
         super().__init__(params, dict(lr=lr, betas=betas, eps=eps, weight_decay=weight_decay))
+        self.prepare_weights = bool(prepare_weights)
         self._tables = None
         self._partials = None
         self.last_grad_norm = None
@@ -59,6 +62,35 @@
         t["step"] = int(max(float(self.state[p]["step"]) for p in ps))
         return t
 
+    def _prep(self, t):
+        from . import functional as F_
+        if not self.prepare_weights:
+            return None
+        if t.get("prep_gen") == F_._PREP_GEN[0]:
+            return t["prep"]
+        ps = t["params"]
+        index = {id(p): i for i, p in enumerate(ps)}
+        dst = np.zeros(len(ps), dtype=np.dtype([("bf", "<i8"), ("tbf", "<i8"), ("rows", "<i4"), ("cols", "<i4")]))
+        units, total = [], 0
+        for u in F_.prep_units():
+            ws = [r() for r in u.refs]
+            idx = [index.get(id(w)) if w is not None else None for w in ws]
+            if not u.fits or any(i is None or ps[i] is not w or dst[i]["rows"] for i, w in zip(idx, ws)):
+                continue
+            for i, w, (rows, cols), (ob, ot), kind in zip(idx, ws, u.dims, u.offs, u.kinds):
+                if w.numel() != rows * cols:
+                    raise RuntimeError("FusedAdam: a registered weight does not have the registered shape")
+                dst[i] = (total + ob, total + ot, rows if kind == 1 else -rows, cols)
+            units.append((weakref.ref(u), total, idx))
+            total += (u.nbytes + 255) // 256 * 256
+        prep = None
+        if units:
+            dev = ps[0].device
+            chunks, nchunks = _chunk_table([p.numel() for p in ps], dev, [(int(d["rows"]), int(d["cols"])) for d in dst])
+            prep = {"chunks": chunks, "nchunks": nchunks, "dst": _to_dev(dst, dev), "bytes": total, "units": units}
+        t["prep"], t["prep_gen"] = prep, F_._PREP_GEN[0]
+        return prep
+
     def _upload_grads(self, t):
         ps = t["params"]
         grads = [p.grad for p in ps]
@@ -106,15 +138,26 @@
             ps = t["params"]
             t["step"] += 1
             b1, b2 = group["betas"]
+            hyper = (float(group["lr"]), float(b1), float(b2), float(group["eps"]), float(group["weight_decay"]), t["step"])
+            prep = self._prep(t)
+            if prep is None:
+                chunks, nchunks, sfx, tail = t["chunks"], t["nchunks"], "", ()
+            else:
+                pool = torch.empty(prep["bytes"], dtype=torch.uint8, device=ps[0].device)
+                chunks, nchunks, sfx, tail = prep["chunks"], prep["nchunks"], "_prep", (prep["dst"], pool)
             if mode is None:
-                N.call("v100_adam_step", t["chunks"], t["nchunks"], t["p"], t["g"].dev, t["m"], t["v"], float(group["lr"]), float(b1),
-                       float(b2), float(group["eps"]), float(group["weight_decay"]), t["step"])
+                N.call("v100_adam_step" + sfx, chunks, nchunks, t["p"], t["g"].dev, t["m"], t["v"], *hyper, *tail)
             else:
-                N.call("v100_adam_step_clip", t["chunks"], t["nchunks"], t["p"], t["g"].dev, t["m"], t["v"], float(group["lr"]), float(b1),
-                       float(b2), float(group["eps"]), float(group["weight_decay"]), t["step"], mode, clip, partials, npartials, code,
-                       self.last_grad_norm if gi == 0 else None)
+                N.call("v100_adam_step_clip" + sfx, chunks, nchunks, t["p"], t["g"].dev, t["m"], t["v"], *hyper, mode, clip, partials,
+                       npartials, code, self.last_grad_norm if gi == 0 else None, *tail)
                 torch.autograd.graph.increment_version(grads[gi])
             torch.autograd.graph.increment_version(ps)
+            if prep is not None:
+                ptrs = t["p_ptrs"]
+                for uref, off, idx in prep["units"]:
+                    u = uref()
+                    if u is not None:
+                        u.ready = (tuple(ps[i]._version for i in idx), tuple(ptrs[i] for i in idx), pool[off:off + u.nbytes])
             st = t.get("step_tensor")
             if st is None or any(self.state[p].get("step") is not st for p in ps[:1]):
                 st = t["step_tensor"] = torch.tensor(float(t["step"]))
@@ -142,10 +185,22 @@
     return torch.from_numpy(np.ascontiguousarray(a).view(np.uint8).copy()).to(dev)
 
 
-def _chunk_table(numels, dev):
+def _chunk_table(numels, dev, tiled=None):
     ce = N.helper("v100_adam_chunk_elems")
-    rec = np.array([(ti, min(ce, k - o), o) for ti, k in enumerate(numels) for o in range(0, k, ce)],
-                   dtype=np.dtype([("tensor", "<i4"), ("count", "<i4"), ("offset", "<i8")]))
+    tile, side = N.helper("v100_adam_prep_tile"), N.helper("v100_adam_prep_max_tiles")
+    rec = []
+    for ti, k in enumerate(numels):
+        rows, cols = tiled[ti] if tiled is not None else (0, 0)
+        if rows > 0:
+            if rows % tile or cols % tile or rows * cols != k:
+                raise RuntimeError("FusedAdam: a prepared weight must be whole tiles")
+            rec += [(ti, min(side, (cols - c0) // tile), r0 * cols + c0) for r0 in range(0, rows, tile) for c0 in range(0, cols, tile * side)]
+        else:
+            step = SMALL_CHUNK if rows < 0 else ce
+            rec += [(ti, min(step, k - o), o) for o in range(0, k, step)]
+    if tiled is not None:
+        rec.sort(key=lambda r: tiled[r[0]][0] >= 0)
+    rec = np.array(rec, dtype=np.dtype([("tensor", "<i4"), ("count", "<i4"), ("offset", "<i8")]))
     return _to_dev(rec, dev), len(rec)
 
 
```
